# decadenza/SimpleStereo

Measured on AMD Instinct MI355X. Metric: disparity MPixels/s (H*W*nDisp per second), higher is better.
Workload: dtype f32

## Files before the change

simplestereo_amd/csrc/asw_instances.inc:

```
#ifdef SSAMD_PIPE_INSTANCE
SSAMD_PIPE_INSTANCE(true, 0, 0, 0)
SSAMD_PIPE_INSTANCE(false, 0, 0, 0)
SSAMD_PIPE_INSTANCE(false, 120, 316, 208)
SSAMD_PIPE_INSTANCE(false, 88, 348, 272)
SSAMD_PIPE_INSTANCE(false, 216, 284, 80)
SSAMD_PIPE_INSTANCE(true, 120, 316, 208)
SSAMD_PIPE_INSTANCE(true, 88, 348, 272)
SSAMD_PIPE_INSTANCE(true, 216, 284, 80)
#endif
#ifdef SSAMD_PIPE_INSTANCE_CG
SSAMD_PIPE_INSTANCE_CG(false, 120, 316, 208)
SSAMD_PIPE_INSTANCE_CG(false, 88, 348, 272)
SSAMD_PIPE_INSTANCE_CG(false, 216, 284, 80)
#endif
#ifdef SSAMD_WAVE6_INSTANCE
SSAMD_WAVE6_INSTANCE(true, 0, false)
SSAMD_WAVE6_INSTANCE(false, 0, false)
SSAMD_WAVE6_INSTANCE(false, 2, false)
SSAMD_WAVE6_INSTANCE(false, 2, true)
SSAMD_WAVE6_INSTANCE(false, 3, false)
SSAMD_WAVE6_INSTANCE(false, 3, true)
#endif
```

simplestereo_amd/csrc/asw_kernels.hip.h:

```cpp
#pragma once
#include "common.hip.h"

namespace ssamd {

static constexpr int ASW_RX = 8;
static constexpr int ASW_RD = 4;
static constexpr int ASW_WB = 4;
static constexpr int ASW_MAX_THREADS = 768;
__host__ __device__ constexpr int asw_nwr(int rx) { return (rx + ASW_RD - 1 + 3) / 4 * 4; }
static_assert(ASW_RD == 4 && asw_nwr(8) == 12 && asw_nwr(4) == 8, "the main loop is unrolled for 8x4 and 4x4 register tiles");

struct AswGeom {
    int Tx, XG, DG, Dc, nchunks, threads;
    int Rx;
    int nL, nR, nRc, SR, Se, emask;
    int SL, hL, hR;
    int wseg, wlen;
    int JC;
    int e2;
    int e_bytes;
    int pipe;
    int NC, JCmax;
    int dephase;
    int wave_rx;
    int off_wL, off_wR, off_e, off_labL, off_labR, off_bgrL, off_bgrR, off_bestL, off_bestR, off_cen, off_prox;
    int lds_bytes;
    int lds_bytes_evol;
};

struct AswExactQueue {
    u64 *entries;
    uint32_t *ekeys;
    unsigned int *counter;
    unsigned char *flagL, *flagR;
    unsigned char *zeroL, *zeroR;
    unsigned char *zrow;
    unsigned int W;
    unsigned int cap;
    uint32_t tol;
    float sat_abs;
    uint32_t deep;
};

struct AswArgs {
    const PixRec *recL, *recR;
    const float *prox;
    u64 *keyL;
    u64 *keyR;
    int16_t *disp;
    const unsigned char *evol;
    int erow0, erows, evolW;
    float *costs;
    int cost_keys;
    int H, W, win, pad, minD, maxD, row0, rows;
    int ystep;
    int yb0;
    int yskip_at, yskip;
    float kC;
    AswExactQueue xq;
    AswGeom g;
};

struct AswPipeTileId { int win, XG, DG, JC; };
__host__ __device__ constexpr int asw_cx_round_up(int v, int m) { return (v + m - 1) / m * m; }
__host__ __device__ constexpr int asw_cx_max(int a, int b) { return a > b ? a : b; }
__host__ __device__ constexpr AswGeom asw_pipe_geom_constexpr(AswPipeTileId t)
{
    AswGeom g{};
    const int win = t.win, p = win / 2;
    g.Rx = 8; g.JC = t.JC; g.pipe = 1; g.wave_rx = 0; g.e2 = 1; g.nchunks = 1;
    g.NC = (win + t.JC / 2) / t.JC;
    g.JCmax = asw_cx_max(t.JC, win - (g.NC - 1) * t.JC);
    g.XG = t.XG; g.DG = t.DG;
    g.Tx = 8 * t.XG; g.Dc = ASW_RD * t.DG;
    g.threads = asw_cx_round_up(t.XG * t.DG, 64);
    g.dephase = g.threads / 64 >= 12 ? 1 : 0;
    g.nL = g.Tx + 2 * p;
    g.nRc = g.Tx + g.Dc - 1;
    g.nR = g.nRc + 2 * p;
    g.hL = 0; g.hR = 0;
    g.SL = asw_cx_round_up(g.Tx, 4);
    g.SR = asw_cx_round_up(g.nRc + 1, 4);
    g.Se = 16 * ((t.DG + 3) / 4);
    g.emask = 0;
    const int wrows = 2 * g.JCmax;
    int off = 0;
    g.off_wL = off; off = (off + wrows * g.SL * 4 + 15) & ~15;
    g.off_wR = off; off = (off + wrows * g.SR * 4 + 15) & ~15;
    g.e_bytes = (g.nL * g.Se + 15) & ~15;
    g.off_e = off; off = (off + g.e_bytes * 2 + 15) & ~15;
    g.off_labL = off; off = (off + g.nL * 16 * 2 + 15) & ~15;
    g.off_labR = off; off = (off + g.nR * 16 * 2 + 15) & ~15;
    g.off_bestL = off; off = (off + g.Tx * 8 + 15) & ~15;
    g.off_bestR = off; off = (off + (g.nRc + 1) * 8 + 15) & ~15;
    g.off_cen = off; off = (off + (g.Tx + g.nRc) * 16 + 15) & ~15;
    g.off_prox = off; off = (off + win * 4 * 2 + 15) & ~15;
    g.lds_bytes_evol = off;
    g.off_bgrL = off; off = (off + g.nL * 4 * 2 + 15) & ~15;
    g.off_bgrR = off; off = (off + g.nR * 4 * 2 + 15) & ~15;
    g.lds_bytes = off;
    return g;
}
template <int SLC, int SRC, int SEC> struct AswPipeTile { static constexpr AswPipeTileId id{35, 1, 1, 16}; };
template <> struct AswPipeTile<120, 316, 208> { static constexpr AswPipeTileId id{35, 15, 49, 16}; };
template <> struct AswPipeTile<88, 348, 272> { static constexpr AswPipeTileId id{35, 11, 65, 16}; };
template <> struct AswPipeTile<216, 284, 80> { static constexpr AswPipeTileId id{35, 27, 17, 16}; };
inline bool asw_pipe_geom_matches(const AswGeom &a, const AswGeom &b)
{
    return a.pipe == b.pipe && a.Rx == b.Rx && a.JC == b.JC && a.NC == b.NC && a.JCmax == b.JCmax && a.XG == b.XG && a.DG == b.DG && a.Tx == b.Tx &&
           a.Dc == b.Dc && a.threads == b.threads && a.dephase == b.dephase && a.nL == b.nL && a.nRc == b.nRc && a.nR == b.nR && a.SL == b.SL &&
           a.SR == b.SR && a.Se == b.Se && a.e_bytes == b.e_bytes && a.off_wL == b.off_wL && a.off_wR == b.off_wR && a.off_e == b.off_e &&
           a.off_labL == b.off_labL && a.off_labR == b.off_labR && a.off_bestL == b.off_bestL && a.off_bestR == b.off_bestR &&
           a.off_cen == b.off_cen && a.off_prox == b.off_prox && a.off_bgrL == b.off_bgrL && a.off_bgrR == b.off_bgrR &&
           a.lds_bytes == b.lds_bytes && a.lds_bytes_evol == b.lds_bytes_evol && a.e2 == b.e2;
}

typedef float v2f __attribute__((ext_vector_type(2)));

template <typename Args>
__device__ __forceinline__ int asw_out_row(const Args &A, int b)
{
    b += A.yb0;
    return A.row0 + b * A.ystep + (b >= A.yskip_at ? A.yskip : 0);
}

static constexpr float ASW_TAD_CAP = 40.0f;

struct AswRow {
    float e[ASW_RD], c[ASW_RD];
};

__device__ __forceinline__ void asw_row_unpack(AswRow &row, const uint32_t packed)
{
#pragma unroll
    for (int di = 0; di < ASW_RD; ++di) {
        const float e = (float)((packed >> (8 * di)) & 0xffu);
        row.e[di] = e;
        row.c[di] = ASW_TAD_CAP - e;
    }
}

template <int RX, int ROT>
__device__ __forceinline__ void asw_taps(float (&accN)[RX][ASW_RD], float (&accS)[RX][ASW_RD],
                                         const float (&wl)[RX], const float (&wr)[asw_nwr(RX)],
                                         const AswRow (&win)[RX])
{
#pragma unroll
    for (int xi = 0; xi < RX; ++xi) {
        const AswRow &row = win[(ROT + xi) % RX];
#pragma unroll
        for (int di = 0; di < ASW_RD; ++di) {
            const float w = wl[xi] * wr[xi - di + ASW_RD - 1];
            accN[xi][di] = fmaf(w, row.e[di], accN[xi][di]);
            accS[xi][di] = fmaf(w, row.c[di], accS[xi][di]);
        }
    }
}

__device__ __forceinline__ uint32_t asw_cost_key(const float n, const float s, float &cost)
{
    const float t40 = n + s;
    if (n <= s) {
        cost = ASW_TAD_CAP * n / t40;
        return __float_as_uint(cost);
    }
    const float inv = ASW_TAD_CAP * s / t40;
    cost = ASW_TAD_CAP - inv;
    return 0xC0000000u - __float_as_uint(inv);
}

static constexpr unsigned EXACT_SIDE_L = 1u, EXACT_SIDE_R = 2u;
__device__ __forceinline__ uint32_t exact_zkey(int win)
{
    return __float_as_uint((float)(win * win) * 9.4039548065783e-37f);
}
static constexpr unsigned EXACT_HINT_ZERO = 4u;
static constexpr uint32_t EXACT_KEY_HIGH = 0xC0000000u - 0x41A00000u;

__device__ __forceinline__ bool exact_near(uint32_t key, uint32_t kb, uint32_t tol, float sat_abs, uint32_t zkey)
{
    if (key - kb <= tol || key <= zkey) return true;
    if (key >= EXACT_KEY_HIGH) {
        const float inv = __uint_as_float(0xC0000000u - key);
        if (kb >= EXACT_KEY_HIGH) return __uint_as_float(0xC0000000u - kb) - inv <= sat_abs;
        return (40.0f - inv) - __uint_as_float(kb) <= 20.0f * 1.1920929e-7f * (float)tol;
    }
    return false;
}

__device__ __forceinline__ bool exact_near_local(uint32_t key, uint32_t kb, uint32_t tol, float sat_abs, uint32_t zkey)
{
    if (key - kb <= tol || key <= zkey) return true;
    if (key < EXACT_KEY_HIGH || kb < 0x418C0000u) return false;
    if (exact_near(key, kb, tol, sat_abs, zkey)) return true;
    return kb >= EXACT_KEY_HIGH && __uint_as_float(0xC0000000u - key) >= 20.0f - 20.0f * 1.1920929e-7f * (float)tol;
}

__device__ __forceinline__ u64 exact_entry(uint32_t pix, int d, unsigned sides)
{
    return (u64)pix | ((u64)(uint32_t)d << 32) | ((u64)sides << 48);
}

__device__ __forceinline__ void asw_exact_push_wave(const AswExactQueue &q, bool want, uint32_t pix, int d, unsigned sides, uint32_t key = 0xffffffffu)
{
    if (key == 0u) sides |= EXACT_HINT_ZERO;
    const u64 mask = __builtin_amdgcn_ballot_w64(want);
    if (mask == 0) return;
    const int leader = (int)__builtin_ctzll(mask);
    const unsigned lane = __builtin_amdgcn_mbcnt_hi(~0u, __builtin_amdgcn_mbcnt_lo(~0u, 0u));
    unsigned base = 0;
    if ((int)lane == leader) base = atomicAdd(q.counter, (unsigned)__builtin_popcountll(mask));
    base = (unsigned)__builtin_amdgcn_readlane((int)base, leader);
    if (want) {
        const unsigned slot = base + (unsigned)__builtin_popcountll(mask & (((u64)1 << lane) - 1));
        if (slot < q.cap) {
            q.entries[slot] = exact_entry(pix, d, sides);
            if (q.ekeys) q.ekeys[slot] = key;
        }
        if ((sides & EXACT_SIDE_L) && q.flagL) q.flagL[pix] = 1;
        if ((sides & EXACT_SIDE_R) && q.flagR) q.flagR[pix - (uint32_t)d] = 1;
    }
}

template <int RX, int RD> struct AswKeyTile { uint32_t v[RX][RD]; };
template <int RX, int RD>
__device__ __forceinline__ void asw_exact_select(const AswExactQueue &q, bool live, const AswKeyTile<RX, RD> &kt,
                                                 const u64 *bL, const u64 *bR, int xb, int db, uint32_t rowpix, uint32_t zkey)
{
    const uint32_t (&kk)[RX][RD] = kt.v;
    static_assert(RX * RD <= 32, "one bit per candidate of the register tile");
    uint32_t mL = 0, mR = 0;
    if (live) {
        uint32_t zl = 0, zr = 0;
        const uint32_t tol = q.tol, deep = q.deep;
        const float ctol = 20.0f * 1.1920929e-7f * (float)tol, sat_abs = q.sat_abs;
        auto slow = [&](uint32_t key, uint32_t kh) -> uint32_t {
            const float inv = __uint_as_float(0xC0000000u - key);
            const uint32_t khigh = kh >= EXACT_KEY_HIGH ? 1u : 0u;
            const uint32_t b_ = khigh & (__uint_as_float(0xC0000000u - kh) - inv <= sat_abs ? 1u : 0u);
            const uint32_t c_ = (khigh ^ 1u) & ((40.0f - inv) - __uint_as_float(kh) <= ctol ? 1u : 0u);
            const uint32_t band = khigh & (inv >= 20.0f - ctol ? 1u : 0u);
            return (key >= EXACT_KEY_HIGH ? 1u : 0u) & (b_ | c_ | band);
        };
#pragma unroll
        for (int xi = 0; xi < RX; ++xi) {
            const u64 kl = bL[xi];
            const uint32_t kh = (uint32_t)(kl >> 32);
            const uint32_t wd = (uint32_t)kl - (uint32_t)db;
            const uint32_t tk = kh <= zkey ? max(tol, zkey - kh) : tol;
            uint32_t okm = 0;
#pragma unroll
            for (int di = 0; di < RD; ++di) {
                const uint32_t key = kk[xi][di];
                const uint32_t ok = (key < deep ? 1u : 0u) & (key != 0u ? 1u : 0u) & (wd != (uint32_t)di ? 1u : 0u);
                okm |= ok << di;
                mL |= (ok & (key - kh <= tk ? 1u : 0u)) << (xi * RD + di);
                zl |= ((key == 0u ? 1u : 0u) & (wd != (uint32_t)di ? 1u : 0u)) << xi;
            }
            if (kh >= 0x418C0000u && kh != 0xffffffffu) {
#pragma unroll
                for (int di = 0; di < RD; ++di) mL |= (((okm >> di) & 1u) & slow(kk[xi][di], kh)) << (xi * RD + di);
            }
        }
        if (bR) {
#pragma unroll
            for (int k = 0; k < RX + RD - 1; ++k) {
                const u64 kr = bR[k];
                const uint32_t kh = (uint32_t)(kr >> 32);
                const uint32_t wx = (uint32_t)kr - (uint32_t)xb;
                const bool high = kh >= 0x418C0000u && kh != 0xffffffffu;
                const uint32_t tk = kh <= zkey ? max(tol, zkey - kh) : tol;
#pragma unroll
                for (int xi = 0; xi < RX; ++xi) {
                    const int di = xi + RD - 1 - k;
                    if (di >= 0 && di < RD) {
                        const uint32_t key = kk[xi][di];
                        const uint32_t ok = (key < deep ? 1u : 0u) & (key != 0u ? 1u : 0u) & (wx != (uint32_t)xi ? 1u : 0u);
                        uint32_t near = key - kh <= tk ? 1u : 0u;
                        if (high) near |= slow(key, kh);
                        mR |= (ok & near) << (xi * RD + di);
                        zr |= ((key == 0u ? 1u : 0u) & (wx != (uint32_t)xi ? 1u : 0u)) << k;
                    }
                }
            }
        }
        if (zl | zr) {
            q.zrow[rowpix / q.W] = 1;
            for (uint32_t z = zl; z; z &= z - 1) q.zeroL[rowpix + (uint32_t)(xb + __builtin_ctz(z))] = 1;
            for (uint32_t z = zr; z; z &= z - 1) q.zeroR[rowpix + (uint32_t)(xb - db - RD + 1 + __builtin_ctz(z))] = 1;
        }
    }
    const uint32_t m = mL | mR;
    const uint32_t n = (uint32_t)__builtin_popcount(m);
    if (__builtin_amdgcn_ballot_w64(n != 0) == 0) return;
    uint32_t before = 0, total = 0;
#pragma unroll
    for (int bit = 0; bit < 6; ++bit) {
        const u64 pl = __builtin_amdgcn_ballot_w64((n >> bit) & 1u);
        before += __builtin_amdgcn_mbcnt_hi((uint32_t)(pl >> 32), __builtin_amdgcn_mbcnt_lo((uint32_t)pl, 0u)) << bit;
        total += (uint32_t)__builtin_popcountll(pl) << bit;
    }
    const u64 active = __builtin_amdgcn_ballot_w64(true);
    const int leader = (int)__builtin_ctzll(active);
    const unsigned lane = __builtin_amdgcn_mbcnt_hi(~0u, __builtin_amdgcn_mbcnt_lo(~0u, 0u));
    unsigned base = 0;
    if ((int)lane == leader) base = atomicAdd(q.counter, total);
    base = (unsigned)__builtin_amdgcn_readlane((int)base, leader);
    unsigned slot = base + before;
    uint32_t mm = m;
    while (mm) {
        const int b = __builtin_ctz(mm);
        mm &= mm - 1;
        const int xi = b / RD, di = b - xi * RD;
        const unsigned sides = ((mL >> b) & 1u ? EXACT_SIDE_L : 0u) | ((mR >> b) & 1u ? EXACT_SIDE_R : 0u);
        const uint32_t pix = rowpix + (uint32_t)(xb + xi);
        const int d = db + di;
        if (slot < q.cap) {
            uint32_t key = 0;
#pragma unroll
            for (int a = 0; a < RX; ++a)
#pragma unroll
                for (int c2 = 0; c2 < RD; ++c2)
                    if (a * RD + c2 == b) key = kk[a][c2];
            q.entries[slot] = exact_entry(pix, d, sides | (key == 0u ? EXACT_HINT_ZERO : 0u));
            if (q.ekeys) q.ekeys[slot] = key;
        }
        if ((sides & EXACT_SIDE_L) && q.flagL) q.flagL[pix] = 1;
        if ((sides & EXACT_SIDE_R) && q.flagR) q.flagR[pix - (uint32_t)d] = 1;
        ++slot;
    }
}

template <bool RIGHT>
__device__ __forceinline__ void asw_exact_merge(const AswExactQueue &q, bool have, u64 mine, u64 old, uint32_t rowpix, int xcol, uint32_t zkey)
{
    bool want = false;
    uint32_t pix = 0, key = 0;
    int d = 0;
    if (have && old != KEY_NONE) {
        const u64 lo = mine < old ? mine : old, hi = mine < old ? old : mine;
        if ((uint32_t)(hi >> 32) < q.deep && (uint32_t)(hi >> 32) != 0u && exact_near_local((uint32_t)(hi >> 32), (uint32_t)(lo >> 32), q.tol, q.sat_abs, zkey)) {
            want = true;
            key = (uint32_t)(hi >> 32);
            if (RIGHT) { const int xl = (int)(uint32_t)hi; pix = rowpix + (uint32_t)xl; d = xl - xcol; }
            else { pix = rowpix + (uint32_t)xcol; d = (int)(uint32_t)hi; }
        }
    }
    if (have && old != KEY_NONE && (uint32_t)(old >> 32) == 0u && (uint32_t)(mine >> 32) == 0u) {
        (RIGHT ? q.zeroR : q.zeroL)[rowpix + (uint32_t)xcol] = 1;
        q.zrow[rowpix / q.W] = 1;
    }
    asw_exact_push_wave(q, want, pix, d, RIGHT ? EXACT_SIDE_R : EXACT_SIDE_L, key);
}

__device__ __forceinline__ int asw_split_pos(int c, int half)
{
    return ((c >> 2) & 1) * half + ((c >> 3) << 2) + (c & 3);
}

template <int RX>
__device__ __forceinline__ int asw_e_offset(int ul, int slot, int Se, int emask)
{
    return ul * Se + ((slot ^ ((ul / RX) & emask)) << 2);
}

template <bool WITH_COSTS, bool CHUNKED, int RX = ASW_RX>
__global__ __launch_bounds__(ASW_MAX_THREADS, RX == 8 ? 3 : 4) void asw_aggregate_kernel(const AswArgs A)
{
    constexpr int NWR = asw_nwr(RX);
    extern __shared__ __attribute__((aligned(16))) char smem[];
    const AswGeom &g = A.g;
    float *const wL = reinterpret_cast<float *>(smem + g.off_wL);
    float *const wR = reinterpret_cast<float *>(smem + g.off_wR);
    unsigned char *const eT0 = reinterpret_cast<unsigned char *>(smem + g.off_e);
    float4 *const labL = reinterpret_cast<float4 *>(smem + g.off_labL);
    float4 *const labR = reinterpret_cast<float4 *>(smem + g.off_labR);
    uint32_t *const bgrL = reinterpret_cast<uint32_t *>(smem + g.off_bgrL);
    uint32_t *const bgrR = reinterpret_cast<uint32_t *>(smem + g.off_bgrR);
    u64 *const bestL = reinterpret_cast<u64 *>(smem + g.off_bestL);
    u64 *const bestR = reinterpret_cast<u64 *>(smem + g.off_bestR);
    float4 *const cenLab = reinterpret_cast<float4 *>(smem + g.off_cen);
    float *const proxS = reinterpret_cast<float *>(smem + g.off_prox);

    const int tid = threadIdx.x, nthr = blockDim.x;
    const int W = A.W, win = A.win, p = A.pad;
    const int Tx = g.Tx, Dc = g.Dc, nL = g.nL, nR = g.nR, nRc = g.nRc, SR = g.SR, Se = g.Se, emask = g.emask;
    int bx = blockIdx.x;
    if ((gridDim.x & 7) == 0) bx = (bx & 7) * (gridDim.x >> 3) + (bx >> 3);
    const int x0 = bx * Tx;
    const int y = asw_out_row(A, blockIdx.y);
    const int dlo = A.minD + blockIdx.z * Dc;
    const int dhi = dlo + Dc - 1;
    if (min(x0 + Tx - 1, W - 1) - dlo < 0) {
        if (A.disp)
            for (int k = threadIdx.x; k < Tx && x0 + k < W; k += blockDim.x)
                A.disp[(size_t)(y - A.row0) * W + x0 + k] = (int16_t)(x0 + k);
        return;
    }

    const int segL_lo = x0 - p;
    const int xrc_lo = x0 - dhi;
    const int segR_lo = xrc_lo - p;


    float accN[RX][ASW_RD], accS[RX][ASW_RD];
#pragma unroll
    for (int a = 0; a < RX; ++a)
#pragma unroll
        for (int b = 0; b < ASW_RD; ++b) { accN[a][b] = 0.f; accS[a][b] = 0.f; }

    for (int k = tid; k < Tx; k += nthr) bestL[k] = KEY_NONE;
    for (int k = tid; k <= nRc; k += nthr) bestR[k] = KEY_NONE;

    for (int c = tid; c < Tx + nRc; c += nthr) {
        const bool isL = c < Tx;
        const int ccol = isL ? x0 + c : xrc_lo + (c - Tx);
        float4 v = make_float4(0.f, 0.f, 0.f, 0.f);
// ... 338 lines not shown
```

simplestereo_amd/csrc/asw_pipe_kernel.hip.h:

```cpp
#pragma once
#include "asw_kernels.hip.h"
#ifndef SSAMD_KERNEL_TU
#include "lab_kernels.hip.h"
#endif

#ifndef SSAMD_PIPE_SENTINEL
#define SSAMD_PIPE_SENTINEL 1
#endif

namespace ssamd {

#ifndef SSAMD_KERNEL_TU
static constexpr int TADV_COLS = 64;
template <bool BYTES>
__device__ __forceinline__ void asw_tad_tile(const void *__restrict__ srcL, const void *__restrict__ srcR, unsigned char *__restrict__ evol,
                                             int W, int pad, int minD, int Dc, int Se, int erow0, int erows, int evolW, int rd, long long npix_total,
                                             int bx, int by, int bz, char *smem)
{
    uint32_t *const sL = reinterpret_cast<uint32_t *>(smem);
    uint32_t *const sR = sL + TADV_COLS;
    const int r = erow0 + by, z = bz, uc0 = bx * TADV_COLS;
    const int P = Se >> 2, dlo = minD + z * Dc, dhi = dlo + Dc - 1;
    const int u0 = uc0 - pad, xr0 = u0 - dhi;
    auto pixel = [&](const void *src, int col) -> uint32_t {
        const size_t q = (size_t)r * W + col;
        if constexpr (BYTES) {
            typedef uint32_t __attribute__((aligned(1))) u32_unaligned;
            const uint8_t *const b = reinterpret_cast<const uint8_t *>(src) + 3 * q;
            return (long long)q + 1 < npix_total ? (*reinterpret_cast<const u32_unaligned *>(b) & 0xffffffu)
                                                 : ((uint32_t)b[0] | ((uint32_t)b[1] << 8) | ((uint32_t)b[2] << 16));
        } else {
            return reinterpret_cast<const PixRec *>(src)[q].bgrx;
        }
    };
    for (int k = threadIdx.x; k < 2 * TADV_COLS + Dc; k += blockDim.x) {
        const bool isL = k < TADV_COLS;
        const int col = isL ? u0 + k : xr0 + (k - TADV_COLS);
        const uint32_t v = (unsigned)col < (unsigned)W ? pixel(isL ? srcL : srcR, col) : 0x80000000u;
        (isL ? sL : sR)[isL ? k : k - TADV_COLS] = v;
    }
    __syncthreads();
    const int ncols = min(TADV_COLS, evolW - uc0);
    uint32_t *const out = reinterpret_cast<uint32_t *>(evol + (((size_t)z * erows + by) * (size_t)evolW + uc0) * Se);
    auto dword = [&](int c, int slot, uint32_t lp) {
        uint32_t v = 0;
        const int d0 = rd == 6 ? 6 * (slot >> 1) + 4 * (slot & 1) : 4 * slot, nv = rd == 6 && (slot & 1) ? 2 : 4;
        if (!(lp >> 31) && d0 < Dc) {
            const uint32_t *const rp = sR + c + (Dc - 1) - d0;
#pragma unroll
            for (int q = 0; q < 4; ++q) {
                const uint32_t rv = q < nv && d0 + q < Dc ? rp[-q] : 0x80000000u;
                if (!(rv >> 31)) v |= min(__builtin_amdgcn_sad_u8(lp, rv, 0u), 40u) << (8 * q);
            }
        }
        return v;
    };
    if ((P & 3) == 0) {
        const int P4 = P >> 2;
        uint4 *const out4 = reinterpret_cast<uint4 *>(out);
        for (int k = threadIdx.x; k < ncols * P4; k += blockDim.x) {
            const int c = k / P4, s4 = 4 * (k - c * P4);
            const uint32_t lp = sL[c];
            out4[k] = make_uint4(dword(c, s4, lp), dword(c, s4 + 1, lp), dword(c, s4 + 2, lp), dword(c, s4 + 3, lp));
        }
        return;
    }
    for (int k = threadIdx.x; k < ncols * P; k += blockDim.x) {
        const int c = k / P, slot = k - c * P;
        out[k] = dword(c, slot, sL[c]);
    }
}

__global__ __launch_bounds__(256) void asw_tad_volume_kernel(const PixRec *__restrict__ recL, const PixRec *__restrict__ recR,
                                                             unsigned char *__restrict__ evol, int W, int pad, int minD, int Dc,
                                                             int Se, int erow0, int erows, int evolW, int rd = 4)
{
    extern __shared__ __attribute__((aligned(16))) char smem[];
    asw_tad_tile<false>(recL, recR, evol, W, pad, minD, Dc, Se, erow0, erows, evolW, rd, 0, blockIdx.x, blockIdx.y, blockIdx.z, smem);
}

struct AswPrepassArgs {
    const uint8_t *bgrL, *bgrR;
    PixRec *recL, *recR;
    unsigned char *evol;
    long long npix_total;
    int W, pad, minD, Dc, Se, erow0, erows, evolW, rd;
    int lab_blocks, ex, ey;
};
__global__ __launch_bounds__(256) void asw_prepass_kernel(const AswPrepassArgs P)
{
    extern __shared__ __attribute__((aligned(16))) char smem[];
    if ((int)blockIdx.x < P.lab_blocks) {
        SSAMD_LAB_TABLES_IN_LDS(T)
        const long long np = (long long)P.erows * P.W, first = (long long)P.erow0 * P.W;
        const uint8_t *const bl = P.bgrL + 3 * first, *const br = P.bgrR + 3 * first;
        PixRec *const rl = P.recL + first, *const rr = P.recR + first;
        typedef uint32_t __attribute__((aligned(1))) u32_unaligned;
        for (long long q = (long long)blockIdx.x * blockDim.x + threadIdx.x; q < 2 * np; q += (long long)P.lab_blocks * blockDim.x) {
            const bool right = q >= np;
            const long long p = right ? q - np : q;
            const uint8_t *const bgr = right ? br : bl;
            uint32_t B, G, R;
            if (p + 1 < np) {
                const uint32_t v = *reinterpret_cast<const u32_unaligned *>(bgr + 3 * p);
                B = v & 0xff; G = (v >> 8) & 0xff; R = (v >> 16) & 0xff;
            } else {
                B = bgr[3 * p]; G = bgr[3 * p + 1]; R = bgr[3 * p + 2];
            }
            PixRec o;
            bgr_to_lab(B, G, R, o.L, o.a, o.b, T);
            o.bgrx = B | (G << 8) | (R << 16);
            (right ? rr : rl)[p] = o;
        }
        return;
    }
    const int b = (int)blockIdx.x - P.lab_blocks, bx = b % P.ex, by = (b / P.ex) % P.ey, bz = b / (P.ex * P.ey);
    asw_tad_tile<true>(P.bgrL, P.bgrR, P.evol, P.W, P.pad, P.minD, P.Dc, P.Se, P.erow0, P.erows, P.evolW, P.rd, P.npix_total, bx, by, bz, smem);
}

#endif

template <bool WITH_COSTS, int SLC = 0, int SRC = 0, int SEC = 0, bool CG = false>
__global__ __launch_bounds__(ASW_MAX_THREADS, 3) void asw_aggregate_pipe_kernel(const AswArgs A)
{
    constexpr bool STATIC = SLC > 0;
    static_assert(!CG || STATIC, "compile-time geometry belongs to a static tile");
    constexpr int RX = ASW_RX;
    constexpr int NWR = asw_nwr(RX);
    extern __shared__ __attribute__((aligned(16))) char smem[];
    constexpr AswGeom SG = asw_pipe_geom_constexpr(AswPipeTile<SLC, SRC, SEC>::id);
    static_assert(!STATIC || (SG.SL == SLC && SG.SR == SRC && SG.Se == SEC), "the strides name the tile");
    const AswGeom &g = CG ? SG : A.g;
    float *const wL = reinterpret_cast<float *>(smem + g.off_wL);
    float *const wR = reinterpret_cast<float *>(smem + g.off_wR);
    unsigned char *const eT0 = reinterpret_cast<unsigned char *>(smem + g.off_e);
    float4 *const labL = reinterpret_cast<float4 *>(smem + g.off_labL);
    float4 *const labR = reinterpret_cast<float4 *>(smem + g.off_labR);
    uint32_t *const bgrL = reinterpret_cast<uint32_t *>(smem + g.off_bgrL);
    uint32_t *const bgrR = reinterpret_cast<uint32_t *>(smem + g.off_bgrR);
    u64 *const bestL = reinterpret_cast<u64 *>(smem + g.off_bestL);
    u64 *const bestR = reinterpret_cast<u64 *>(smem + g.off_bestR);
    float4 *const cenLab = reinterpret_cast<float4 *>(smem + g.off_cen);
    float *const proxS = reinterpret_cast<float *>(smem + g.off_prox);

    const int tid = threadIdx.x, nthr = blockDim.x;
    const int W = A.W, win = CG ? AswPipeTile<SLC, SRC, SEC>::id.win : A.win, p = CG ? AswPipeTile<SLC, SRC, SEC>::id.win / 2 : A.pad;
    const int Tx = g.Tx, Dc = g.Dc, nL = g.nL, nR = g.nR, nRc = g.nRc, SR = g.SR, Se = g.Se;
    const int JC = g.JC, NC = g.NC;
    int bx = blockIdx.x;
    if ((gridDim.x & 7) == 0) bx = (bx & 7) * (gridDim.x >> 3) + (bx >> 3);
    const int x0 = bx * Tx;
    const int y = asw_out_row(A, blockIdx.y);
    const int dlo = A.minD + blockIdx.z * Dc;
    const int dhi = dlo + Dc - 1;
    if (min(x0 + Tx - 1, W - 1) - dlo < 0) {
        if (A.disp)
            for (int k = threadIdx.x; k < Tx && x0 + k < W; k += blockDim.x)
                A.disp[(size_t)(y - A.row0) * W + x0 + k] = (int16_t)(x0 + k);
        return;
    }
    const int segL_lo = x0 - p, xrc_lo = x0 - dhi, segR_lo = xrc_lo - p;
    const int phase = g.dephase ? __builtin_amdgcn_readfirstlane((int)(threadIdx.x >> 8)) : 1;

    float accN[RX][ASW_RD], accS[RX][ASW_RD];
#pragma unroll
    for (int a = 0; a < RX; ++a)
#pragma unroll
        for (int b = 0; b < ASW_RD; ++b) { accN[a][b] = 0.f; accS[a][b] = 0.f; }

    for (int k = tid; k < Tx; k += nthr) bestL[k] = KEY_NONE;
    for (int k = tid; k <= nRc; k += nthr) bestR[k] = KEY_NONE;
    for (int c = tid; c < Tx + nRc; c += nthr) {
        const bool isL = c < Tx;
        const int ccol = isL ? x0 + c : xrc_lo + (c - Tx);
        float4 v = make_float4(0.f, 0.f, 0.f, 0.f);
        if ((unsigned)ccol < (unsigned)W) {
            const PixRec q = (isL ? A.recL : A.recR)[(size_t)y * W + ccol];
            v = make_float4(q.L, q.a, q.b, 1.f);
        }
        cenLab[c] = v;
    }

    const int i_lo = max(0, p - y), i_hi = min(win, A.H + p - y);

    auto stage_row = [&](int i) {
        int tids = threadIdx.x;
        asm volatile("" : "+v"(tids));
        const int buf = i & 1, r = y - p + i;
        for (int k = tids; k < win; k += nthr) proxS[buf * win + k] = A.prox[i * win + k];
        const PixRec *const rowL = A.recL + (size_t)r * W;
        const PixRec *const rowR = A.recR + (size_t)r * W;
        for (int k = tids; k < nL + nR; k += nthr) {
            const bool isL = k < nL;
            const int idx = isL ? k : k - nL;
            const int col = (isL ? segL_lo : segR_lo) + idx;
            PixRec v;
            v.L = SSAMD_PIPE_SENTINEL ? __builtin_inff() : 0.f;
            v.a = v.b = 0.f;
            v.bgrx = 0u;
            if ((unsigned)col < (unsigned)W) v = (isL ? rowL : rowR)[col];
            (isL ? labL + buf * nL : labR + buf * nR)[idx] = make_float4(v.L, v.a, v.b, 0.f);
            if (!A.evol) (isL ? bgrL + buf * nL : bgrR + buf * nR)[idx] = v.bgrx;
        }
    };
    auto build_e = [&](int i, int t_lo, int t_hi) {
        int tidb = threadIdx.x;
        asm volatile("" : "+v"(tidb));
        unsigned char *const eT = eT0 + (i & 1) * g.e_bytes;
        const uint32_t *const bgrLc = bgrL + (i & 1) * nL, *const bgrRc = bgrR + (i & 1) * nR;
        const int e_q = nthr / nL, e_r = nthr - e_q * nL;
        int t = t_lo + tidb;
        int sp = t / nL, ul = t - sp * nL;
        while (t < t_hi) {
            const uint32_t lp = bgrLc[ul];
            const uint32_t *const rp = bgrRc + (ul + (Dc - 1) - 8 * sp);
            uint32_t lo = 0, hi = 0;
#pragma unroll
            for (int k = 0; k < 4; ++k) {
                lo |= min(__builtin_amdgcn_sad_u8(lp, rp[-k], 0u), 40u) << (8 * k);
                hi |= min(__builtin_amdgcn_sad_u8(lp, rp[-4 - k], 0u), 40u) << (8 * k);
            }
            uint32_t *const dst = reinterpret_cast<uint32_t *>(eT + ul * Se) + 2 * sp;
            dst[0] = lo;
            if (2 * sp + 1 < g.DG) dst[1] = hi;
            t += nthr; ul += e_r; sp += e_q;
            if (ul >= nL) { ul -= nL; ++sp; }
        }
    };
    auto load_e = [&](int i) {
        int tidd = threadIdx.x;
        asm volatile("" : "+v"(tidd));
        const int r = y - p + i;
        const unsigned char *const src = A.evol + (((size_t)blockIdx.z * A.erows + (r - A.erow0)) * (size_t)A.evolW + x0) * Se;
        unsigned char *const dst = eT0 + (i & 1) * g.e_bytes;
        const int bytes = nL * Se, lane16 = (tidd & 63) * 16;
        for (int k = __builtin_amdgcn_readfirstlane(tidd >> 6) * 1024; k < bytes; k += (nthr >> 6) * 1024)
            if (k + lane16 < bytes)
                __builtin_amdgcn_global_load_lds((const void *)(src + k + lane16),
                                                 (__attribute__((address_space(3))) void *)(dst + k), 16, 0, 0);
    };
    auto build_weights = [&](int i, int jb, int je, int rb) {
        int tidw = threadIdx.x;
        asm volatile("" : "+v"(tidw));
        const float4 *const labLc = labL + (i & 1) * nL, *const labRc = labR + (i & 1) * nR;
        const float *const prow = proxS + (i & 1) * win;
        const int ncen = Tx + nRc;
        const int full = ncen / nthr * nthr, rest = ncen - full;
        int slen = je - jb, nseg = 1;
        if (rest > 0 && full > 0) {
            slen = max(ASW_WB, (je - jb + nthr / rest - 1) / (nthr / rest));
            slen = (slen + ASW_WB - 1) / ASW_WB * ASW_WB;
            nseg = (je - jb + slen - 1) / slen;
        }
        const int ntasks = full + rest * nseg;
        for (int t = tidw; t < ntasks; t += nthr) {
            int c = t, jb_t = jb, je_t = je;
            if (t >= full && nseg > 1) {
                const int q = t - full, sgm = q / rest;
                c = full + q - sgm * rest;
                jb_t = jb + sgm * slen;
                je_t = min(je, jb_t + slen);
            }
            const bool isL = c < Tx;
            const int cc = isL ? c : c - Tx;
            const float4 cen = cenLab[c];
            const float4 *const seg = (isL ? labLc : labRc) + cc;
            const int stride = isL ? g.SL : SR;
            float *const wout = (isL ? wL : wR) + cc + (rb - jb) * stride;
            const int col0 = (isL ? x0 : xrc_lo) + cc - p;
            const uint32_t cmask = cen.w != 0.f ? 0xffffffffu : 0u;
            int j = jb_t;
            const float4 *sp = seg + j;
            const float *pp = prow + j;
            float *wp = wout + j * stride;
            int col = col0 + j;
            const int stride4 = ASW_WB * stride;
            for (; j + ASW_WB <= je_t; j += ASW_WB, sp += ASW_WB, pp += ASW_WB, wp += stride4, col += ASW_WB) {
                float4 tp[ASW_WB];
                float pr[ASW_WB], wv[ASW_WB];
#pragma unroll
                for (int u = 0; u < ASW_WB; ++u) { tp[u] = sp[u]; pr[u] = pp[u]; }
#pragma unroll
                for (int u = 0; u < ASW_WB; ++u) {
                    asm volatile("" ::"v"(tp[u].w));
                    const float dL = tp[u].x - cen.x, da = tp[u].y - cen.y, db = tp[u].z - cen.z;
                    wv[u] = fmaf(db, db, fmaf(da, da, dL * dL));
                }
#pragma unroll
                for (int u = 0; u < ASW_WB; ++u) wv[u] = __builtin_amdgcn_sqrtf(wv[u]);
#pragma unroll
                for (int u = 0; u < ASW_WB; ++u) wv[u] = asw_weight_finish(wv[u], A.kC, pr[u]);
#pragma unroll
                for (int u = 0; u < ASW_WB; ++u) {
                    if constexpr (SSAMD_PIPE_SENTINEL) {
                        wp[u * stride] = wv[u];
                    } else {
                        const uint32_t m = (unsigned)(col + u) < (unsigned)W ? cmask : 0u;
                        wp[u * stride] = __uint_as_float(__float_as_uint(wv[u]) & m);
                    }
                }
            }
            if (j < je_t) {
                float4 tp[ASW_WB];
                float pr[ASW_WB], wv[ASW_WB];
#pragma unroll
                for (int u = 0; u < ASW_WB; ++u) {
                    const int jj = min(j + u, je_t - 1);
                    tp[u] = seg[jj];
                    pr[u] = prow[jj];
                }
#pragma unroll
                for (int u = 0; u < ASW_WB; ++u) {
                    asm volatile("" ::"v"(tp[u].w));
                    const float dL = tp[u].x - cen.x, da = tp[u].y - cen.y, db = tp[u].z - cen.z;
                    wv[u] = fmaf(db, db, fmaf(da, da, dL * dL));
                }
#pragma unroll
                for (int u = 0; u < ASW_WB; ++u) wv[u] = __builtin_amdgcn_sqrtf(wv[u]);
#pragma unroll
                for (int u = 0; u < ASW_WB; ++u) wv[u] = asw_weight_finish(wv[u], A.kC, pr[u]);
#pragma unroll
                for (int u = 0; u < ASW_WB; ++u) {
                    const int jj = min(j + u, je_t - 1);
                    if constexpr (SSAMD_PIPE_SENTINEL) {
                        wout[jj * stride] = wv[u];
                    } else {
                        const uint32_t m = (unsigned)(col0 + jj) < (unsigned)W ? cmask : 0u;
                        wout[jj * stride] = __uint_as_float(__float_as_uint(wv[u]) & m);
                    }
                }
            }
        }
    };
    auto chunk_end = [&](int c) { return c == NC - 1 ? win : (c + 1) * JC; };
    const int nE = nL * ((g.DG + 1) >> 1);
    auto build_next = [&](int i, int c, int cb) {
        const bool more_rows = i + 1 < i_hi;
#ifdef SSAMD_PIPE_BUILD_PRIO
        __builtin_amdgcn_s_setprio(SSAMD_PIPE_BUILD_PRIO);
#endif
#ifndef SSAMD_ABLATE_STAGE
        if (c == 0 && more_rows) stage_row(i + 1);
#endif
        if (c == 0 && more_rows && A.evol) load_e(i + 1);
#ifndef SSAMD_ABLATE_WEIGHTS
        if (c + 1 < NC) build_weights(i, (c + 1) * JC, chunk_end(c + 1), (cb ^ 1) * g.JCmax);
        else if (more_rows) build_weights(i + 1, 0, chunk_end(0), (cb ^ 1) * g.JCmax);
#endif
#ifndef SSAMD_ABLATE_E
        if (c >= 1 && more_rows && !A.evol) build_e(i + 1, (int)((long long)nE * (c - 1) / (NC - 1)), (int)((long long)nE * c / (NC - 1)));
#endif
#ifdef SSAMD_PIPE_BUILD_PRIO
        __builtin_amdgcn_s_setprio(0);
#endif
    };

    stage_row(i_lo);
    if (A.evol) load_e(i_lo);
    __syncthreads();
    if (!A.evol) build_e(i_lo, 0, nE);
    build_weights(i_lo, 0, chunk_end(0), 0);

    const int DGe = max(1, min(g.DG, (min(min(x0 + Tx, W) - 1, x0 + Tx - 1) - dlo) / ASW_RD + 1));
    const int nact = g.XG * DGe;
    int pk_xd;
    bool run;
    {
        const int tidm = threadIdx.x;
        int xg, dg;
#ifdef SSAMD_PIPE_PLAIN_LANES
        xg = tidm / DGe; dg = tidm - xg * DGe;
#else
        const int F = DGe >> 4, Lo = DGe & 15, nfull = g.XG * F;
        const int grp16 = tidm >> 4, r16 = tidm & 15;
        if (grp16 < nfull) {
            xg = grp16 / F;
            int gi = grp16 - xg * F;
            if (xg & 1) gi = F - 1 - gi;
            dg = 16 * gi + r16;
        } else {
            const int q = tidm - 16 * nfull;
            xg = Lo ? q / Lo : g.XG;
            dg = 16 * F + (Lo ? q - xg * Lo : 0);
        }
#endif
        pk_xd = xg | (dg << 16);
        const bool tile_live = tidm < nact && x0 + RX * xg < W && dlo + ASW_RD * dg <= A.maxD &&
                               x0 + RX * xg + RX - 1 - (dlo + ASW_RD * dg) >= 0;
        run = __builtin_amdgcn_ballot_w64(tile_live) != 0 && tidm < nact;
    }

    int cb = 0;
#pragma nounroll
    for (int i = i_lo; i < i_hi; ++i) {
        const unsigned char *const eT = eT0 + (i & 1) * g.e_bytes;
        AswRow ew[RX];

#pragma nounroll
        for (int c = 0; c < NC; ++c) {
#ifndef SSAMD_ABLATE_BARRIER
            __syncthreads();
#endif
            const int jc = c * JC, jend = chunk_end(c);
            const int rb = cb * g.JCmax;
            if (phase == 0) build_next(i, c, cb);
#ifndef SSAMD_ABLATE_AGG
            if (run) {
                const int xg = pk_xd & 0xffff, dg = pk_xd >> 16;
                const unsigned char *erow = eT + (RX * xg + (jc == 0 ? 0 : RX - 1 + jc)) * Se + 4 * dg;
                if (jc == 0) {
#pragma unroll
                    for (int n = 0; n < RX - 1; ++n) {
                        asw_row_unpack(ew[n], *reinterpret_cast<const uint32_t *>(erow));
                        erow += Se;
                    }
                }
                const float *wlp = wL + rb * g.SL + 8 * xg;
                const float *wrp = wR + rb * SR + (RX * xg - ASW_RD * dg + Dc - ASW_RD);
                for (int j0 = jc; j0 < jend; j0 += RX) {
#define SSAMD_PSTEP(JJ)                                                                             \
    if (j0 + (JJ) < jend) {                                                                         \
        const uint32_t epk = *reinterpret_cast<const uint32_t *>(erow + (STATIC ? (JJ) * SEC : 0)); \
        if constexpr (!STATIC) erow += Se;                                                          \
        float wl[RX], wr[NWR];                                                                      \
        {                                                                                           \
            const float *const wl_ = wlp + (STATIC ? (JJ) * SLC : 0);                              \
            const float *const wr_ = wrp + (STATIC ? (JJ) * SRC : 0);                              \
            const float4 v0 = *reinterpret_cast<const float4 *>(wl_);                              \
            wl[0] = v0.x; wl[1] = v0.y; wl[2] = v0.z; wl[3] = v0.w;                                 \
            const float4 v1 = *reinterpret_cast<const float4 *>(wl_ + 4);                          \
            wl[4] = v1.x; wl[5] = v1.y; wl[6] = v1.z; wl[7] = v1.w;                                 \
            const float4 r0 = *reinterpret_cast<const float4 *>(wr_);                              \
            const float4 r1 = *reinterpret_cast<const float4 *>(wr_ + 4);                          \
            const float4 r2 = *reinterpret_cast<const float4 *>(wr_ + 8);                          \
            asm volatile("" ::"v"(r2.w));       \
            wr[0] = r0.x; wr[1] = r0.y; wr[2] = r0.z; wr[3] = r0.w;                                 \
            wr[4] = r1.x; wr[5] = r1.y; wr[6] = r1.z; wr[7] = r1.w;                                 \
            wr[8] = r2.x; wr[9] = r2.y; wr[10] = r2.z; wr[11] = r2.w;                               \
        }                                                                                           \
        if constexpr (!STATIC) { wlp += g.SL; wrp += SR; }                                         \
               \
        _Pragma("unroll") for (int xi = 0; xi < RX; ++xi) {                                         \
            if (xi == RX - 1) asw_row_unpack(ew[((JJ) + RX - 1) % RX], epk);                        \
            const AswRow &row_ = ew[((JJ) + xi) % RX];                                              \
            _Pragma("unroll") for (int di = 0; di < ASW_RD; ++di) {                                 \
                const float w_ = wl[xi] * wr[xi - di + ASW_RD - 1];                                 \
                accN[xi][di] = fmaf(w_, row_.e[di], accN[xi][di]);                                  \
                accS[xi][di] = fmaf(w_, row_.c[di], accS[xi][di]);                                  \
            }                                                                                       \
        }                                                                                           \
    }
                    SSAMD_PSTEP(0) SSAMD_PSTEP(1) SSAMD_PSTEP(2) SSAMD_PSTEP(3)
                    SSAMD_PSTEP(4) SSAMD_PSTEP(5) SSAMD_PSTEP(6) SSAMD_PSTEP(7)
#undef SSAMD_PSTEP
                    if constexpr (STATIC) { erow += RX * SEC; wlp += RX * SLC; wrp += RX * SRC; }
                }
            }
#endif
            if (phase != 0) build_next(i, c, cb);
            cb ^= 1;
        }
    }

    int tidf = threadIdx.x;
    asm volatile("" : "+v"(tidf));
    AswKeyTile<RX, ASW_RD> kt;
    if (tidf < nact) {
        const int xg = pk_xd & 0xffff, dg = pk_xd >> 16;
        u64 diag[RX + ASW_RD - 1];
#pragma unroll
        for (int k = 0; k < RX + ASW_RD - 1; ++k) diag[k] = KEY_NONE;
#pragma unroll
        for (int xi = 0; xi < RX; ++xi) {
            const int x = x0 + RX * xg + xi;
            u64 bl = KEY_NONE;
#pragma unroll
            for (int di = 0; di < ASW_RD; ++di) {
                const int d = dlo + ASW_RD * dg + di;
                const bool valid = (x < W) && (d <= A.maxD) && (x - d >= 0);
                kt.v[xi][di] = 0xffffffffu;
                if (valid) {
                    float c;
                    const u64 hi = (u64)asw_cost_key(accN[xi][di], accS[xi][di], c) << 32;
                    kt.v[xi][di] = (uint32_t)(hi >> 32);
                    bl = min(bl, hi | (u64)(uint32_t)d);
                    diag[xi - di + ASW_RD - 1] = min(diag[xi - di + ASW_RD - 1], hi | (u64)(uint32_t)x);
                    if (WITH_COSTS)
                        A.costs[((size_t)(y - A.row0) * W + x) * (A.maxD - A.minD + 1) + (d - A.minD)] = A.cost_keys ? __uint_as_float((uint32_t)(hi >> 32)) : c;
                }
            }
            if (bl != KEY_NONE) atomicMin(&bestL[RX * xg + xi], bl);
        }
        if (A.keyR) {
            const int base = RX * xg - ASW_RD * dg + Dc - ASW_RD;
#pragma unroll
            for (int k = 0; k < RX + ASW_RD - 1; ++k)
                if (diag[k] != KEY_NONE) atomicMin(&bestR[base + k], diag[k]);
        }
    }
    __syncthreads();
    const size_t orow = (size_t)(y - A.row0) * W;
    const bool xq = !WITH_COSTS && A.xq.entries != nullptr;
    if (xq) {
        const int xg = pk_xd & 0xffff, dg = pk_xd >> 16;
        asw_exact_select<RX, ASW_RD>(A.xq, tidf < nact, kt, bestL + RX * xg, A.keyR ? bestR + (RX * xg - ASW_RD * dg + Dc - ASW_RD) : nullptr,
                                     x0 + RX * xg, dlo + ASW_RD * dg, (uint32_t)orow, exact_zkey(win));
    }
    if (A.disp) {
        for (int k = tid; k < Tx; k += nthr) {
            const int x = x0 + k;
            if (x < W) A.disp[orow + x] = bestL[k] == KEY_NONE ? (int16_t)x : (int16_t)(uint32_t)bestL[k];
        }
        return;
    }
    if (xq) {
        for (int k0 = 0; k0 < Tx; k0 += nthr) {
            const int k = k0 + tid, x = x0 + k;
            const bool have = k < Tx && x < W && bestL[k < Tx ? k : 0] != KEY_NONE;
            const u64 mine = have ? bestL[k] : KEY_NONE;
            const u64 old = have ? atomicMin(&A.keyL[orow + x], mine) : KEY_NONE;
            asw_exact_merge<false>(A.xq, have, mine, old, (uint32_t)orow, x, exact_zkey(win));
        }
        if (A.keyR)
            for (int k0 = 0; k0 < nRc; k0 += nthr) {
                const int k = k0 + tid, xr = xrc_lo + k;
                const bool have = k < nRc && (unsigned)xr < (unsigned)W && bestR[k < nRc ? k : 0] != KEY_NONE;
                const u64 mine = have ? bestR[k] : KEY_NONE;
                const u64 old = have ? atomicMin(&A.keyR[orow + xr], mine) : KEY_NONE;
                asw_exact_merge<true>(A.xq, have, mine, old, (uint32_t)orow, xr, exact_zkey(win));
            }
        return;
    }
    for (int k = tid; k < Tx; k += nthr) {
        const int x = x0 + k;
        if (x < W && bestL[k] != KEY_NONE) atomicMin(&A.keyL[orow + x], bestL[k]);
    }
    if (A.keyR) {
        for (int k = tid; k < nRc; k += nthr) {
            const int xr = xrc_lo + k;
            if ((unsigned)xr < (unsigned)W && bestR[k] != KEY_NONE) atomicMin(&A.keyR[orow + xr], bestR[k]);
        }
    }
}

}
```

simplestereo_amd/csrc/asw_pipe_tu.hip:

```cpp
#define SSAMD_KERNEL_TU 1
#include <hip/hip_runtime.h>
#include "asw_pipe_kernel.hip.h"

namespace ssamd {
#define SSAMD_PIPE_INSTANCE(C, SL, SR, SE) template __global__ void asw_aggregate_pipe_kernel<C, SL, SR, SE>(const AswArgs);
#define SSAMD_PIPE_INSTANCE_CG(C, SL, SR, SE) template __global__ void asw_aggregate_pipe_kernel<C, SL, SR, SE, true>(const AswArgs);
#include "asw_instances.inc"
#undef SSAMD_PIPE_INSTANCE_CG
#undef SSAMD_PIPE_INSTANCE
}
```

simplestereo_amd/csrc/ssamd_api.hip:

```cpp
#include <hip/hip_runtime.h>

#include <algorithm>
#include <array>
#include <atomic>
#include <list>
#include <map>
#include <thread>
#include <cmath>
#include <cstdarg>
#include <cstdio>
#include <cstdlib>
#include <cstring>
#include <mutex>
#include <string>
#include <vector>

#include "../../include/ssamd.h"
#include "asw_kernels.hip.h"
#include "asw_pipe_kernel.hip.h"
#include "asw_wave_kernel.hip.h"
#include "asw_wave6_kernel.hip.h"
#include "asw_alt_kernels.hip.h"
#ifndef SSAMD_SINGLE_TU
namespace ssamd {
#define SSAMD_PIPE_INSTANCE(C, SL, SR, SE) extern template __global__ void asw_aggregate_pipe_kernel<C, SL, SR, SE>(const AswArgs);
#define SSAMD_PIPE_INSTANCE_CG(C, SL, SR, SE) extern template __global__ void asw_aggregate_pipe_kernel<C, SL, SR, SE, true>(const AswArgs);
#define SSAMD_WAVE6_INSTANCE(C, K, CREG) extern template __global__ void asw_aggregate_wave6_kernel<C, K, CREG>(const AswWaveArgs);
#include "asw_instances.inc"
#undef SSAMD_PIPE_INSTANCE
#undef SSAMD_PIPE_INSTANCE_CG
#undef SSAMD_WAVE6_INSTANCE
}
#endif
#include "gsw_kernels.hip.h"
#include "lab_kernels.hip.h"
#include "asw_exact_kernels.hip.h"
#include "rig_kernels.hip.h"
#include "unwrap_kernels.hip.h"

using namespace ssamd;

namespace {

thread_local std::string g_err;
std::mutex g_geom_mutex;

int fail(int code, const char *fmt, ...)
{
    char buf[512];
    va_list ap;
    va_start(ap, fmt);
    vsnprintf(buf, sizeof(buf), fmt, ap);
    va_end(ap);
    g_err = buf;
    return code;
}

struct Tuning {
    std::string asw_geom, gsw_geom;
    int asw_pipe = -1;
    int asw_dephase = -1;
    int asw_evol = 1;
    int asw_wave = -1;
    int wave_rx = 0;
    int wave_wg = 0;
    int wave_unroll = 1;
    int wave_merge = 1;
    int asw_static = 1;
    int evol_max_mb = 0;
    int wave_rd = 0;
    bool no_e2 = false, xor_only = false, multi_allow_repeat = false;
    int alt_queue_cap = 0;
    int autotune_env = -2;
    int evol_fail = 0;
    int lds_relax = 1;
    int wave_creg = 1;
    int asw_tail = -1;
    int prepass_fuse = 1;
    int exact_tol = 128;
    int exact_cap = 0;
    int exact_rawcap = 0;
    int unwrap_rows = 0;
};
std::mutex g_tune_mutex;
std::atomic<unsigned> g_tune_version{1};

bool tuning_assign(Tuning &t, const std::string &name, const char *v)
{
    auto num = [&](int unset) { return v ? atoi(v) : unset; };
    if (name == "SSAMD_ASW_GEOM") t.asw_geom = v ? v : "";
    else if (name == "SSAMD_GSW_GEOM") t.gsw_geom = v ? v : "";
    else if (name == "SSAMD_ASW_PIPE") t.asw_pipe = num(-1);
    else if (name == "SSAMD_ASW_DEPHASE") t.asw_dephase = num(-1);
    else if (name == "SSAMD_ASW_EVOL") t.asw_evol = num(1);
    else if (name == "SSAMD_ASW_WAVE") t.asw_wave = v ? (atoi(v) != 0 ? 1 : 0) : -1;
    else if (name == "SSAMD_ASW_WAVE_RX") t.wave_rx = num(0);
    else if (name == "SSAMD_ASW_WAVE_WG") t.wave_wg = v ? std::max(1, std::min(4, atoi(v))) : 0;
    else if (name == "SSAMD_ASW_WAVE_UNROLL") t.wave_unroll = num(1);
    else if (name == "SSAMD_ASW_WAVE_MERGE") t.wave_merge = num(1);
    else if (name == "SSAMD_ASW_STATIC") t.asw_static = num(1);
    else if (name == "SSAMD_ASW_EVOL_MAX_MB") t.evol_max_mb = v ? std::max(0, atoi(v)) : 0;
    else if (name == "SSAMD_ASW_WAVE_RD") t.wave_rd = num(0);
    else if (name == "SSAMD_ASW_NO_E2") t.no_e2 = v != nullptr;
    else if (name == "SSAMD_ASW_XOR_ONLY") t.xor_only = v != nullptr;
    else if (name == "SSAMD_MULTI_ALLOW_REPEAT") t.multi_allow_repeat = v != nullptr;
    else if (name == "SSAMD_ALT_QUEUE_CAP") t.alt_queue_cap = v ? std::max(1, atoi(v)) : 0;
    else if (name == "SSAMD_AUTOTUNE") t.autotune_env = v ? (atoi(v) > 0 ? 1 : (atoi(v) < 0 ? -1 : 0)) : -2;
    else if (name == "SSAMD_ASW_EVOL_FAIL") t.evol_fail = num(0);
    else if (name == "SSAMD_ASW_TAIL") t.asw_tail = num(-1);
    else if (name == "SSAMD_ASW_WAVE_CREG") t.wave_creg = num(1);
    else if (name == "SSAMD_ASW_LDS_RELAX") t.lds_relax = num(1);
    else if (name == "SSAMD_ASW_PREPASS_FUSE") t.prepass_fuse = num(1);
    else if (name == "SSAMD_EXACT_TOL") t.exact_tol = v ? std::max(0, atoi(v)) : 128;
    else if (name == "SSAMD_EXACT_CAP") t.exact_cap = v ? std::max(1, atoi(v)) : 0;
    else if (name == "SSAMD_EXACT_RAWCAP") t.exact_rawcap = v ? std::max(1, atoi(v)) : 0;
    else if (name == "SSAMD_UNWRAP_ROWS") t.unwrap_rows = v ? std::max(0, std::min(UNWRAP_MAX_ROWS, atoi(v))) : 0;
    else return false;
    return true;
}

const char *const kTuningNames[] = {"SSAMD_ASW_GEOM", "SSAMD_GSW_GEOM", "SSAMD_ASW_PIPE", "SSAMD_ASW_DEPHASE", "SSAMD_ASW_EVOL",
                                    "SSAMD_ASW_WAVE", "SSAMD_ASW_WAVE_RX", "SSAMD_ASW_WAVE_WG", "SSAMD_ASW_WAVE_UNROLL",
                                    "SSAMD_ASW_WAVE_MERGE", "SSAMD_ASW_STATIC", "SSAMD_ASW_EVOL_MAX_MB", "SSAMD_ASW_WAVE_RD", "SSAMD_ASW_NO_E2", "SSAMD_ASW_XOR_ONLY", "SSAMD_MULTI_ALLOW_REPEAT",
                                    "SSAMD_ALT_QUEUE_CAP", "SSAMD_AUTOTUNE", "SSAMD_ASW_EVOL_FAIL", "SSAMD_ASW_TAIL", "SSAMD_ASW_WAVE_CREG", "SSAMD_ASW_LDS_RELAX",
                                    "SSAMD_EXACT_TOL", "SSAMD_EXACT_CAP", "SSAMD_EXACT_RAWCAP", "SSAMD_ASW_PREPASS_FUSE", "SSAMD_UNWRAP_ROWS"};

std::map<std::string, std::string> g_tuning_env;
Tuning tuning_from_env()
{
    Tuning t;
    for (const char *n : kTuningNames)
        if (const char *v = getenv(n)) {
            g_tuning_env[n] = v;
            (void)tuning_assign(t, n, v);
        }
    return t;
}
Tuning g_tuning = tuning_from_env();

const Tuning &tune()
{
    thread_local Tuning snap;
    thread_local unsigned seen = 0;
    const unsigned v = g_tune_version.load(std::memory_order_acquire);
    if (v != seen) {
        std::lock_guard<std::mutex> lk(g_tune_mutex);
        snap = g_tuning;
        seen = v;
    }
    return snap;
}

#define HIP_TRY(expr)                                                                              \
    do {                                                                                           \
        hipError_t e_ = (expr);                                                                    \
        if (e_ != hipSuccess)                                                                      \
            return fail(e_ == hipErrorOutOfMemory ? SSAMD_ENOMEM : SSAMD_EHIP, "%s failed: %s",    \
                        #expr, hipGetErrorString(e_));                                             \
    } while (0)

struct DevBuf {
    void *ptr = nullptr;
    size_t cap = 0;
    int reserve(size_t bytes)
    {
        if (bytes <= cap) return SSAMD_OK;
        if (ptr) { (void)hipFree(ptr); ptr = nullptr; cap = 0; }
        size_t want = bytes + bytes / 8 + 256;
        hipError_t e = hipMalloc(&ptr, want);
        if (e != hipSuccess) {
            ptr = nullptr;
            (void)hipGetLastError();
            return fail(SSAMD_ENOMEM, "hipMalloc(%zu) failed: %s", want, hipGetErrorString(e));
        }
        cap = want;
        return SSAMD_OK;
    }
    void release()
    {
        if (ptr) (void)hipFree(ptr);
        ptr = nullptr; cap = 0;
    }
};

struct Profile {
    bool on = false;
    struct Pair { hipEvent_t a, b; int slot; };
    std::vector<Pair> pending;
    std::vector<hipEvent_t> pool;
    double ms[SSAMD_K_COUNT] = {0};
    long long n[SSAMD_K_COUNT] = {0};
    hipEvent_t get()
    {
        if (!pool.empty()) { hipEvent_t e = pool.back(); pool.pop_back(); return e; }
        hipEvent_t e = nullptr;
        (void)hipEventCreate(&e);
        return e;
    }
    void drain()
    {
        for (auto &p : pending) {
            float t = 0.f;
            if (hipEventSynchronize(p.b) == hipSuccess && hipEventElapsedTime(&t, p.a, p.b) == hipSuccess) {
                ms[p.slot] += t;
                n[p.slot] += 1;
            }
            pool.push_back(p.a);
            pool.push_back(p.b);
        }
        pending.clear();
    }
};

struct TableEntry {
    int k0 = 0; double k1 = 0;
    DevBuf dev;
    std::vector<float> host;
    std::vector<double> host64;
};
struct TableCache {
    std::list<TableEntry> entries;
    size_t max_entries;
    explicit TableCache(size_t n) : max_entries(n) {}
    TableEntry *find(int k0, double k1)
    {
        for (auto it = entries.begin(); it != entries.end(); ++it)
            if (it->k0 == k0 && it->k1 == k1) {
                entries.splice(entries.begin(), entries, it);
                return &entries.front();
            }
        return nullptr;
    }
};

struct Ctx {
    std::mutex mu;
    int dev = -1;
    int cus = 256;
    bool lut_ready = false;
    hipStream_t stream = nullptr;
    DevBuf imgL, imgR, recL, recR, keyL, keyR, disp, costs, lab, altq, evol, altdisp;
    DevBuf xlabL, xlabR, xflags, xqueue, xcost, xslots, xctr, xraw, xwtab;
    DevBuf uwIn, uwOut;
    unsigned int xcap = 0, xrawcap = 0;
    TableCache proxTabs{8}, gswTabs{4}, proxTabs64{8};
    std::map<const void *, int> max_dyn_lds;
    hipEvent_t scratch_free = nullptr;
    int evol_small_calls = 0;
    long long evol_fallbacks = 0;
    long long tail_splits = 0;
    long long exact_calls = 0;
    long long static_tile_mismatch = 0;
    Profile prof;
};

Ctx g_ctx[16];

struct DeviceGuard {
    int saved = -1;
    DeviceGuard() { if (hipGetDevice(&saved) != hipSuccess) saved = -1; }
    ~DeviceGuard() { if (saved >= 0) (void)hipSetDevice(saved); }
    DeviceGuard(const DeviceGuard &) = delete;
    DeviceGuard &operator=(const DeviceGuard &) = delete;
};

int grant_dyn_lds(Ctx &c, const void *kernel, int bytes);

struct Timed {
    Ctx &c; hipStream_t s; int slot; hipEvent_t a = nullptr, b = nullptr;
    Timed(Ctx &c_, hipStream_t s_, int slot_) : c(c_), s(s_), slot(slot_)
    {
        if (c.prof.on) { a = c.prof.get(); b = c.prof.get(); (void)hipEventRecord(a, s); }
    }
    ~Timed()
    {
        if (a) { (void)hipEventRecord(b, s); c.prof.pending.push_back({a, b, slot}); }
    }
};

struct CtxLock {
    DeviceGuard guard;
    std::unique_lock<std::mutex> lk;
    Ctx *c = nullptr;
    Ctx *operator->() { return c; }
    Ctx &operator*() { return *c; }
};

int get_ctx(int device, CtxLock &out)
{
    int n = 0;
    if (hipGetDeviceCount(&n) != hipSuccess || n <= 0)
        return fail(SSAMD_ENODEVICE, "no HIP device visible: libssamd has no CPU fallback");
    if (device < 0) device = out.guard.saved >= 0 ? out.guard.saved : 0;
    if (device >= n || device >= 16) return fail(SSAMD_EINVAL, "device ordinal %d out of range (%d visible)", device, n);
    HIP_TRY(hipSetDevice(device));
    Ctx &c = g_ctx[device];
    out.lk = std::unique_lock<std::mutex>(c.mu);
    out.c = &c;
    if (c.dev < 0) {
        c.dev = device;
        int cus = 0;
        if (hipDeviceGetAttribute(&cus, hipDeviceAttributeMultiprocessorCount, device) == hipSuccess && cus > 0) c.cus = cus;
        else (void)hipGetLastError();
        HIP_TRY(hipStreamCreateWithFlags(&c.stream, hipStreamNonBlocking));
        HIP_TRY(hipEventCreateWithFlags(&c.scratch_free, hipEventDisableTiming));
    }
    if (!c.lut_ready) {
        float lut[256];
        for (int v = 0; v < 256; ++v) {
            float x = v / 255.0;
            if (x > 0.04045) x = glibc_powf_pos((float)((x + 0.055) / 1.055), (float)2.4);
            else x /= 12.92;
            x *= 100;
            lut[v] = x;
        }
        HIP_TRY(hipMemcpyToSymbol(HIP_SYMBOL(c_lin100), lut, sizeof(lut)));
        c.lut_ready = true;
    }
    return SSAMD_OK;
}

int grant_dyn_lds(Ctx &c, const void *kernel, int bytes)
{
    int &granted = c.max_dyn_lds[kernel];
    if (bytes <= granted || bytes <= 48 * 1024) return SSAMD_OK;
    HIP_TRY(hipFuncSetAttribute(kernel, hipFuncAttributeMaxDynamicSharedMemorySize, bytes));
    granted = bytes;
    return SSAMD_OK;
}

struct ScratchOrder {
    Ctx &c; hipStream_t s;
    ScratchOrder(Ctx &c_, hipStream_t s_) : c(c_), s(s_) { (void)hipStreamWaitEvent(s, c.scratch_free, 0); }
    ~ScratchOrder() { (void)hipEventRecord(c.scratch_free, s); }
};

int check_common(int H, int W, int win, int minD, int maxD, int row0, int rows)
{
    if (H <= 0 || W <= 0) return fail(SSAMD_EINVAL, "Wrong image dimensions!");
    if (!(win > 0 && win % 2 == 1)) return fail(SSAMD_EINVAL, "winSize must be a positive odd number!");
    if (minD < 0) return fail(SSAMD_EINVAL, "minDisparity must be >= 0 (negative values are undefined behaviour in the reference)");
    if (W > 32767 || maxD > 32767) return fail(SSAMD_ELIMIT, "width / maxDisparity exceed the int16 disparity range");
    if (row0 < 0 || rows < 0 || row0 + rows > H) return fail(SSAMD_EINVAL, "output row range [%d,%d) outside the image (height %d)", row0, row0 + rows, H);
    if (win > 255) return fail(SSAMD_ELIMIT, "winSize %d > 255 not supported", win);
    if (rows > 65535) return fail(SSAMD_ELIMIT, "more than 65535 output rows per call: split the image into row strips");
    return SSAMD_OK;
}

inline int round_up(int v, int m) { return (v + m - 1) / m * m; }

thread_local bool t_pipe_full_lds = false;

bool asw_layout_e(AswGeom &g, int win, int XG, int DG, size_t limit, int JC, int Rx, bool e2, bool odd_pitch = false,
                  bool pipe = false)
{
    g.Rx = Rx;
    g.JC = JC >= win ? win : JC;
    g.pipe = 0; g.NC = 1; g.JCmax = g.JC; g.dephase = 0; g.wave_rx = 0;
    if (pipe) {
        if (Rx != 8 || JC % Rx || !e2) return false;
        g.NC = (win + JC / 2) / JC;
        if (g.NC < 2 || (g.NC - 1) * JC >= win) return false;
        g.pipe = 1;
        g.dephase = tune().asw_dephase >= 0 ? tune().asw_dephase : (round_up(XG * DG, 64) / 64 >= 12 ? 1 : 0);
        g.JCmax = std::max(JC, win - (g.NC - 1) * JC);
    }
    const int wrows = g.pipe ? 2 * g.JCmax : (g.JC < win ? 2 * g.JC : win);
    const int wcols = g.JC;

    const int p = win / 2;
    g.XG = XG; g.DG = DG;
    g.Tx = Rx * XG; g.Dc = ASW_RD * DG;
    g.threads = round_up(XG * DG, 64);
    g.nL = g.Tx + 2 * p;
    g.nRc = g.Tx + g.Dc - 1;
    g.nR = g.nRc + 2 * p;
    g.hL = ((g.Tx + 7) / 8) * 4 + 4;
    g.SL = 2 * g.hL;
    g.hR = ((g.nRc + 4 + 7) / 8) * 4 + 4;
    g.SR = 2 * g.hR;
    int P = 8;
    while (P < DG && P < 32) P <<= 1;
    if (P < DG) P = round_up(DG, 32);
    g.Se = 4 * P;
    g.emask = std::min(P, 32) - 1;
    if (odd_pitch) {
        g.Se = 4 * (DG | 1);
        g.emask = 0;
    }
    if (g.pipe) {
        g.hL = g.hR = 0;
        g.SL = round_up(g.Tx, 4);
        g.SR = round_up(g.nRc + 1, 4);
        g.Se = 16 * ((DG + 3) / 4);
        g.emask = 0;
    }
    {
        const int ncen = g.Tx + g.nRc;
        int best_cost = 1 << 30;
        for (int ns = 1; ns <= wcols && ns <= 8; ++ns) {
            const int len = (wcols + ns - 1) / ns, rounds = (ncen * ns + g.threads - 1) / g.threads;
            const int cost = rounds * (round_up(len, ASW_WB) + 2);
            if (cost < best_cost) { best_cost = cost; g.wseg = ns; g.wlen = len; }
        }
    }
    size_t off = 0;
    auto take = [&](size_t bytes) { size_t o = off; off = (off + bytes + 15) & ~(size_t)15; return (int)o; };
    g.off_wL = take((size_t)wrows * g.SL * 4);
    g.off_wR = take((size_t)wrows * g.SR * 4);
    g.e_bytes = (int)(((size_t)g.nL * g.Se + 15) & ~(size_t)15);
    g.e2 = (e2 && g.JC < win && (win + g.JC - 1) / g.JC >= 2) ? 1 : 0;
    if (g.pipe && !g.e2) return false;
    g.off_e = take((size_t)g.e_bytes * (g.e2 ? 2 : 1));
    g.off_labL = take((size_t)g.nL * 16 * 2);
    g.off_labR = take((size_t)g.nR * 16 * 2);
    if (!g.pipe) {
        g.off_bgrL = take((size_t)g.nL * 4 * 2);
        g.off_bgrR = take((size_t)g.nR * 4 * 2);
    }
    g.off_bestL = take((size_t)g.Tx * 8);
    g.off_bestR = take((size_t)(g.nRc + 1) * 8);
    g.off_cen = take((size_t)(g.Tx + g.nRc) * 16);
    g.off_prox = take((size_t)win * 4 * 2);
    g.lds_bytes_evol = (int)off;
    if (g.pipe) {
        g.off_bgrL = take((size_t)g.nL * 4 * 2);
        g.off_bgrR = take((size_t)g.nR * 4 * 2);
    }
    g.lds_bytes = (int)off;
    if (g.pipe && tune().asw_evol != 0 && tune().lds_relax != 0 && !t_pipe_full_lds) return (size_t)g.lds_bytes_evol <= limit;
    return off <= limit;
}

bool asw_layout(AswGeom &g, int win, int XG, int DG, size_t limit, int JC = 1 << 20, int Rx = ASW_RX, bool odd_pitch = false)
{
    if (!tune().no_e2 && asw_layout_e(g, win, XG, DG, limit, JC, Rx, true, odd_pitch) && g.e2) return true;
    return asw_layout_e(g, win, XG, DG, limit, JC, Rx, false, odd_pitch);
}

double asw_e_read_passes(const AswGeom &g)
{
    const int P = g.Se / 4, T = g.XG * g.DG;
    long long tot = 0, cnt = 0;
    for (int n = 0; n < g.Rx; ++n)
        for (int base = 0; base < T; base += 32) {
            int hits[64] = {0}, worst = 0;
            for (int l = 0; l < 32 && base + l < T; ++l) {
                const int tid = base + l, xg = tid % g.XG, dg = tid / g.XG, ul = g.Rx * xg + n;
                worst = std::max(worst, ++hits[(ul * P + (dg ^ ((ul / g.Rx) & g.emask))) & 63]);
            }
            tot += worst; ++cnt;
        }
    return cnt ? (double)tot / cnt : 1.0;
}

void asw_pick_e_scheme(AswGeom &g, int win)
{
    if (tune().xor_only) return;
    AswGeom alt;
    if (!asw_layout(alt, win, g.XG, g.DG, 160 * 1024, g.JC >= win ? (1 << 20) : g.JC, g.Rx, true)) return;
    const bool take = alt.e2 != g.e2 ? alt.e2 > g.e2 : asw_e_read_passes(alt) <= asw_e_read_passes(g) + 1e-9;
    if (take) {
        alt.nchunks = g.nchunks;
        g = alt;
    }
}

void asw_try_pipe(AswGeom &g, int win)
{
    const int want = tune().asw_pipe;
    if (want == 0 || g.Rx != 8) return;
    for (int JC : {16, 8}) {
        if (want > 0 && JC != want) continue;
        if (want < 0 && JC == 8 && round_up(g.XG * g.DG, 64) / 64 < 12) continue;
        AswGeom alt;
        if (!asw_layout_e(alt, win, g.XG, g.DG, 160 * 1024, JC, 8, true, false, true)) continue;
        alt.nchunks = g.nchunks;
        g = alt;
        return;
    }
}

static constexpr int ASW_WAVE_MAX_DG = 16;
bool asw_wave_layout_one(AswWaveGeom &g, int win, int DG, int rx, int nxg, bool merged, int rd = ASW_RD, bool creg = false)
{
    g.RX = rx;
    g.RD = rd;
    g.creg = 0;
    const int p = win / 2;
    g.DG = DG;
    g.NXG = nxg;
    g.Txw = rx * g.NXG;
    g.Dc = rd * g.DG;
    g.lanes = g.NXG * g.DG;
    g.nLw = g.Txw + 2 * p;
    g.nRcw = g.Txw + g.Dc - 1;
    g.nRw = g.nRcw + 2 * p;
    g.merged = merged ? 1 : 0;
    if (merged) {
        g.K = (g.Txw + g.nRcw + 63) / 64;
        g.SLw = g.Txw;
        g.SRw = round_up(g.Txw + g.nRcw + 1, 64) - g.Txw;
    } else {
        g.K = (g.Txw + 63) / 64 + (g.nRcw + 63) / 64;
        g.SLw = round_up(g.Txw, 64);
        g.SRw = round_up(g.nRcw + 1, 64);
    }
    g.Se = rd == 6 ? 8 * ((g.DG + 1) | 1) : 4 * (g.DG | 1);
    g.waves = tune().wave_wg ? tune().wave_wg : 1;
    size_t off = 0;
    auto take = [&](size_t bytes) { size_t o = off; off = (off + bytes + 15) & ~(size_t)15; return (int)o; };
    g.off_w = take((size_t)(g.SLw + g.SRw) * 4 * 2);
    g.creg = creg && merged && rx == 4 && g.K >= 2 && (rd == 6 ? g.K <= 3 : g.K <= 4) ? 1 : 0;
    g.off_cen = take(g.creg ? 0 : (size_t)(g.Txw + g.nRcw) * 16);
    g.off_pixL = take((size_t)g.nLw * 16);
    g.off_pixR = take((size_t)g.nRw * 16);
    g.off_e = take(std::max((size_t)g.nLw * g.Se, (size_t)(129 + 2 * p) * 16) + (rd == 6 ? 0 : (size_t)rx * g.Se));
    g.off_bestL = g.off_pixL;
    g.off_bestR = g.off_pixL + (int)(((size_t)g.Txw * 8 + 15) & ~(size_t)15);
    if ((size_t)g.off_bestR + (size_t)(g.nRcw + 1) * 8 > off) off = (size_t)g.off_bestR + (size_t)(g.nRcw + 1) * 8;
    g.wave_lds = (int)((off + 15) & ~(size_t)15);
    return g.off_pixR == g.off_pixL + g.nLw * 16 && (size_t)g.wave_lds * g.waves <= 160 * 1024;
}

bool asw_wave_layout(AswWaveGeom &g, int win, int nD, int rx, bool creg = false)
{
    const bool never6 = (rx & 16) != 0;
    rx &= 15;
    creg = creg && tune().wave_creg != 0;
    const int DG = (nD + ASW_RD - 1) / ASW_RD;
    if (DG < 1 || DG > ASW_WAVE_MAX_DG) return false;
    const int nxg_max = 64 / DG;
    if (tune().wave_merge == 0) return asw_wave_layout_one(g, win, DG, rx, nxg_max, false);
    const double c_round = 17.0, c_taps = rx == 8 ? 110.0 : 59.0;
    double best = 1e30;
    bool found = false;
    for (int nxg = nxg_max; nxg >= std::max(1, nxg_max - 4); --nxg)
        for (int merged = 0; merged <= 1; ++merged) {
            AswWaveGeom c;
            if (merged && nxg != nxg_max && tune().wave_merge == 2) continue;
            if (!asw_wave_layout_one(c, win, DG, rx, nxg, merged != 0, ASW_RD, creg)) continue;
            if (merged && c.K > 4) continue;
            if (!merged && nxg != nxg_max) continue;
            const double cost = (c.K * c_round + c_taps) / (double)c.Txw;
            if (cost < best - 1e-9) { best = cost; g = c; found = true; }
        }
    if (found && rx == 4 && !never6 && tune().wave_rd != 4 && tune().wave_merge != 0) {
        const int DG6 = (nD + 5) / 6;
        if (DG6 >= 1 && DG6 <= 10) {
            const int nxg6 = 64 / DG6;
            for (int nxg = nxg6; nxg >= std::max(1, nxg6 - 4); --nxg) {
                AswWaveGeom c;
                if (!asw_wave_layout_one(c, win, DG6, 4, nxg, true, 6, creg) || c.K > 4) continue;
                const double cost = (c.K * c_round + 87.0) / (double)c.Txw;
                if (cost < 0.95 * best) { best = cost / 0.95; g = c; }
            }
        }
    }
    return found;
}

static constexpr int ASW_WAVE_MAX_ND = 64;
int asw_wave_pick(int win, int nD)
{
    if (tune().asw_wave == 0 || tune().asw_evol == 0) return 0;
    if (nD < 1 || nD > ASW_WAVE_MAX_ND || win > 63) return 0;
    AswWaveGeom wg;
    if (const int rx = tune().wave_rx) {
        return (rx == 8 || rx == 4) && asw_wave_layout(wg, win, nD, rx) ? rx : 0;
    }
    const int first = nD <= 20 ? 4 : 8, second = 12 - first;
    if (asw_wave_layout(wg, win, nD, first)) return first;
    return asw_wave_layout(wg, win, nD, second) ? second : 0;
}

int asw_search_geometry(AswGeom &best, int W, int rows, int win, int nD, std::vector<AswGeom> *shortlist = nullptr);

std::map<std::array<int, 4>, AswGeom> g_asw_geom_cache;
std::map<std::array<int, 4>, bool> g_asw_geom_tuned;
std::atomic<int> g_autotune{g_tuning.autotune_env != -2 ? g_tuning.autotune_env : -1};
constexpr double ASW_AUTOTUNE_SMALL_TAPS = 6.0e10;

bool asw_geometry_forced()
{
    const Tuning &t = tune();
    return !t.asw_geom.empty() || t.asw_wave >= 0 || t.wave_rx != 0 || t.wave_merge != 1 || t.asw_pipe >= 0 || t.asw_dephase >= 0 ||
           t.asw_evol != 1 || t.wave_wg != 0 || t.no_e2 || t.xor_only || t.asw_static != 1 || t.evol_max_mb != 0 || t.wave_rd != 0 ||
           t.wave_creg != 1 || t.lds_relax != 1;
}

int asw_choose_geometry(AswGeom &best, int W, int rows, int win, int nD)
{
    if (asw_geometry_forced()) return asw_search_geometry(best, W, rows, win, nD);
    std::lock_guard<std::mutex> glk(g_geom_mutex);
    const std::array<int, 4> key{W, rows, win, nD};
    auto it = g_asw_geom_cache.find(key);
    if (it != g_asw_geom_cache.end()) { best = it->second; return SSAMD_OK; }
    const int rc = asw_search_geometry(best, W, rows, win, nD);
    if (rc == SSAMD_OK) {
        if (g_asw_geom_cache.size() > 256) { g_asw_geom_cache.clear(); g_asw_geom_tuned.clear(); }
        g_asw_geom_cache[key] = best;
    }
    return rc;
}

int asw_search_geometry(AswGeom &best, int W, int rows, int win, int nD, std::vector<AswGeom> *shortlist)
{
    std::map<std::array<int, 4>, std::pair<double, AswGeom>> classes;
    if (!tune().asw_geom.empty()) {
        int XG = 0, DG = 0, JCe = 1 << 20, Rx = ASW_RX;
        if (sscanf(tune().asw_geom.c_str(), "%d,%d,%d,%d", &XG, &DG, &JCe, &Rx) >= 2 && XG > 0 && DG > 0 && XG * DG <= ASW_MAX_THREADS &&
            (Rx == 8 || Rx == 4)) {
            if (JCe <= 0 || JCe % Rx) JCe = 1 << 20;
            if (!asw_layout(best, win, XG, DG, 160 * 1024, JCe, Rx)) return fail(SSAMD_ELIMIT, "SSAMD_ASW_GEOM does not fit LDS");
            best.nchunks = (nD + best.Dc - 1) / best.Dc;
            asw_pick_e_scheme(best, win);
            asw_try_pipe(best, win);
            return SSAMD_OK;
        }
    }
    const double c_tap = 10.9, c_w = 70.0, c_e = 60.0, c_stage = 40.0;
    double best_score = -1.0;
    bool found = false;
    for (int nch = 1; nch <= nD; ++nch) {
        const int per = (nD + nch - 1) / nch;
        const int DG = round_up(per, ASW_RD) / ASW_RD;
        if (DG > 128) continue;
        if ((nD + DG * ASW_RD - 1) / (DG * ASW_RD) != nch) continue;
        for (int Rx : {8, 4}) {
        if (Rx == 4 && nD > 56) continue;
        const int max_wps = Rx == 8 ? 3 : 4;
        const int xg_cap = std::min(ASW_MAX_THREADS / DG, (W + Rx - 1) / Rx);
        const int pipe_env = tune().asw_pipe;
        for (int XG = xg_cap; XG >= 1; --XG)
        for (int cand = 0; cand < 6; ++cand) {
            static const int jcs[6] = {1 << 20, 16, 8, 4, 16, 8};
            const int JC = jcs[cand];
            const bool piped = cand >= 4;
            AswGeom g;
            if (piped) {
                if (Rx != 8 || pipe_env == 0 || (pipe_env > 0 && pipe_env != JC)) continue;
                if (pipe_env < 0 && JC == 8 && round_up(XG * DG, 64) / 64 < 12) continue;
                if (!asw_layout_e(g, win, XG, DG, 160 * 1024, JC, 8, true, false, true)) continue;
            } else {
                if (JC < (1 << 20) && (JC >= win || JC % Rx)) continue;
                if (!asw_layout(g, win, XG, DG, 160 * 1024, JC, Rx)) continue;
            }
            g.nchunks = nch;
            const int waves = g.threads / 64, per_simd = (waves + 3) / 4;
            const int k = std::min(max_wps / per_simd, (160 * 1024) / (piped && tune().asw_evol != 0 ? g.lds_bytes_evol : g.lds_bytes));
            if (k < 1) continue;
            const double M = (double)win * Rx * ASW_RD * (Rx == 8 ? (piped ? 0.93 * c_tap : c_tap) : c_tap * 1.15);
            const int ncen = g.Tx + g.nRc;
            const int njc = piped ? g.NC : (win + g.JC - 1) / g.JC;
            double B;
            if (piped)
                B = (double)ncen * win / g.threads * 28.0 + njc * 350.0 + c_stage;
            else
                B = (double)njc * ((ncen * g.wseg + g.threads - 1) / g.threads) * (round_up(g.wlen, ASW_WB) + 2) * c_w +
                    (njc > 1 ? njc * 400.0 : 0.0) +
                    (double)((g.nL * (g.Dc / 4) + g.threads - 1) / g.threads) * c_e +
                    (double)((g.nL + g.nR + g.threads - 1) / g.threads) * c_stage;
            const double d_util = (double)nD / ((double)nch * g.Dc);
            const int xt = (W + g.Tx - 1) / g.Tx;
            const double x_util = (double)W / ((double)xt * g.Tx);
            const double nwg = (double)xt * std::max(rows, 1) * nch, slots = 256.0 * k;
            const double tail = nwg / (std::ceil(nwg / slots) * slots);
            const double overlap = k > 1 ? 1.05 : 1.0;
            const int wps = k * per_simd;
            const double occ = wps >= 3 ? 1.0 : (wps == 2 ? 0.85 : 0.6);
            const double useful = (double)win * Rx * ASW_RD * c_tap;
            const double score = (double)XG * DG / per_simd * occ * (useful / (M + B)) * d_util * x_util * tail * overlap;
            if (score > best_score) { best_score = score; best = g; found = true; }
            if (shortlist) {
                auto &slot = classes[{piped ? 80 : Rx, std::min(g.JC, 64), nch, waves}];
                if (score > slot.first) slot = {score, g};
            }
        }
        }
        if (DG <= 2) break;
    }
    if (found && !best.pipe && best.Rx == 8 && best.JC >= win && best.DG >= 33 && win > 16) {
        AswGeom g;
        if (asw_layout(g, win, best.XG, best.DG, 160 * 1024, 16, 8)) {
            g.nchunks = best.nchunks;
            best = g;
        }
    }
    if (found && !best.pipe) asw_pick_e_scheme(best, win);
    const int wave_rx = found ? asw_wave_pick(win, nD) : 0;
    if (wave_rx) best.wave_rx = wave_rx;
    if (shortlist && found) {
        std::vector<std::pair<double, AswGeom>> v;
        for (auto &kv : classes) v.push_back(kv.second);
        std::sort(v.begin(), v.end(), [](const auto &a, const auto &b) { return a.first > b.first; });
        shortlist->clear();
        if (wave_rx) {
            shortlist->push_back(best);
            AswWaveGeom wg;
            if (!tune().wave_rx && asw_wave_layout(wg, win, nD, 12 - wave_rx)) {
                AswGeom other = best;
                other.wave_rx = 12 - wave_rx;
                shortlist->push_back(other);
            }
            if (wave_rx == 4 && asw_wave_layout(wg, win, nD, 4) && wg.RD == 6) {
                AswGeom other = best;
                other.wave_rx = 4 | 16;
                shortlist->push_back(other);
            }
        }
        for (size_t i = 0; i < v.size() && i < (wave_rx ? 3u : 12u) && v[i].first > 0.6 * best_score; ++i) {
            if (!v[i].second.pipe) asw_pick_e_scheme(v[i].second, win);
            v[i].second.wave_rx = 0;
            shortlist->push_back(v[i].second);
        }
    }
    return found ? SSAMD_OK : fail(SSAMD_ELIMIT, "no ASW launch geometry fits LDS for winSize=%d nD=%d", win, nD);
}

int get_prox(Ctx &c, int win, double gammaP, hipStream_t s, const float **out)
{
    if (TableEntry *e = c.proxTabs.find(win, gammaP)) { *out = (const float *)e->dev.ptr; return SSAMD_OK; }
    if (c.proxTabs.entries.size() >= c.proxTabs.max_entries) {
        HIP_TRY(hipDeviceSynchronize());
        (void)hipFree(c.proxTabs.entries.back().dev.ptr);
        c.proxTabs.entries.pop_back();
    }
    c.proxTabs.entries.emplace_front();
    TableEntry &e = c.proxTabs.entries.front();
    e.k0 = win; e.k1 = gammaP;
    const int p = win / 2;
    e.host.resize((size_t)win * win);
    for (int i = 0; i < win; ++i)
        for (int j = 0; j < win; ++j) {
            const double di = i - p, dj = j - p;
#if SSAMD_W_FOLD
            e.host[(size_t)i * win + j] = (float)(-std::sqrt(di * di + dj * dj) / gammaP * 1.4426950408889634);
#else
            e.host[(size_t)i * win + j] = (float)glibc_exp(-std::sqrt(di * di + dj * dj) / gammaP);
#endif
        }
    int rc = e.dev.reserve(e.host.size() * 4);
    if (rc) { c.proxTabs.entries.pop_front(); return rc; }
    hipError_t he = hipMemcpyAsync(e.dev.ptr, e.host.data(), e.host.size() * 4, hipMemcpyHostToDevice, s);
    if (he != hipSuccess) {
        (void)hipFree(e.dev.ptr);
        c.proxTabs.entries.pop_front();
        return fail(SSAMD_EHIP, "hipMemcpyAsync(proximity table) failed: %s", hipGetErrorString(he));
    }
    *out = (const float *)e.dev.ptr;
    return SSAMD_OK;
}

int get_prox64(Ctx &c, int win, double gammaP, hipStream_t s, const double **out)
{
    if (TableEntry *e = c.proxTabs64.find(win, gammaP)) { *out = (const double *)e->dev.ptr; return SSAMD_OK; }
    if (c.proxTabs64.entries.size() >= c.proxTabs64.max_entries) {
        HIP_TRY(hipDeviceSynchronize());
        (void)hipFree(c.proxTabs64.entries.back().dev.ptr);
        c.proxTabs64.entries.pop_back();
    }
    c.proxTabs64.entries.emplace_front();
    TableEntry &e = c.proxTabs64.entries.front();
    e.k0 = win; e.k1 = gammaP;
    const int p = win / 2;
    e.host64.resize((size_t)win * win);
    for (int i = 0; i < win; ++i)
        for (int j = 0; j < win; ++j)
            {
                const double di = i - p, dj = j - p;
                e.host64[(size_t)i * win + j] = glibc_exp(-std::sqrt(di * di + dj * dj) / gammaP);
            }
    int rc = e.dev.reserve(e.host64.size() * 8);
    if (rc) { c.proxTabs64.entries.pop_front(); return rc; }
    hipError_t he = hipMemcpyAsync(e.dev.ptr, e.host64.data(), e.host64.size() * 8, hipMemcpyHostToDevice, s);
    if (he != hipSuccess) {
        (void)hipFree(e.dev.ptr);
        c.proxTabs64.entries.pop_front();
        return fail(SSAMD_EHIP, "hipMemcpyAsync(fp64 proximity table) failed: %s", hipGetErrorString(he));
    }
    *out = (const double *)e.dev.ptr;
    return SSAMD_OK;
}

int asw_exact_prepare(Ctx &c, int W, int rows, int win, int nD, double gammaC, bool consistent, bool direct, hipStream_t s,
                      AswExactQueue &q, AswExactQueue &raw, AswExactQueue &kernel_q)
{
    const size_t nout = (size_t)rows * W;
    if (nout >= ((size_t)1 << 32)) return fail(SSAMD_ELIMIT, "exact mode: more than 2^32 output pixels per call");
    const size_t all_cands = 2 * (nout * (size_t)nD + nout);
    size_t cap = std::min<size_t>(std::max<size_t>(4 * nout, std::min<size_t>(all_cands, (size_t)1 << 23)), (size_t)1 << 26);
    if (tune().exact_cap) cap = (size_t)tune().exact_cap;
    size_t rawcap = direct ? 0 : std::min<size_t>(std::max<size_t>(2 * nout, std::min<size_t>(all_cands, (size_t)1 << 23)), (size_t)1 << 26);
    if (!direct && tune().exact_cap) rawcap = std::max<size_t>(rawcap, cap);
    if (!direct && tune().exact_rawcap) rawcap = (size_t)tune().exact_rawcap;
    int rc;
    if ((rc = c.xqueue.reserve(cap * 8)) || (rc = c.xcost.reserve(cap * 8)) || (rc = c.xflags.reserve(64 + 4 * nout + (size_t)rows)) ||
        (rc = c.xslots.reserve(nout * 32)) || (rawcap && (rc = c.xraw.reserve(rawcap * 12))))
        return rc;
    c.xcap = (unsigned int)cap;
    c.xrawcap = (unsigned int)rawcap;
    HIP_TRY(hipMemsetAsync(c.xflags.ptr, 0, 64 + 4 * nout + (size_t)rows, s));
    q.entries = (u64 *)c.xqueue.ptr;
    q.ekeys = nullptr;
    q.counter = (unsigned int *)c.xflags.ptr;
    q.flagL = (unsigned char *)c.xflags.ptr + 64;
    q.flagR = consistent ? q.flagL + nout : nullptr;
    q.zeroL = q.flagL + 2 * nout;
    q.zeroR = consistent ? q.flagL + 3 * nout : nullptr;
    q.zrow = q.flagL + 4 * nout;
    q.W = (unsigned int)W;
    q.cap = (unsigned int)cap;
    q.tol = (uint32_t)std::min(1.0e6, (double)tune().exact_tol * std::max(1.0, 5.0 / gammaC) * std::max(1.0, win / 35.0));
    q.sat_abs = (float)(1.5 * 2.0 * 2.0 * ((double)win * win + 3.0) * 1.1102230246251565e-16 * 40.0);
    q.deep = 0xffffffffu;
    raw = AswExactQueue{};
    if (!direct) {
        raw = q;
        union { float f; uint32_t u; } sa; sa.f = q.sat_abs;
        raw.deep = 0xC0000000u - sa.u;
        raw.entries = (u64 *)c.xraw.ptr;
        raw.ekeys = (uint32_t *)((u64 *)c.xraw.ptr + rawcap);
        raw.counter = q.counter + 4;
        raw.flagL = raw.flagR = nullptr;
        raw.cap = (unsigned int)rawcap;
    }
    kernel_q = direct ? q : raw;
    return SSAMD_OK;
}

int asw_exact_pass(Ctx &c, const AswExactQueue &q, const AswExactQueue &raw, int H, int W, int row0, int rows, int win, int maxD, int minD, double gammaC, double gammaP,
                   bool consistent, bool direct, int16_t *d_disp, hipStream_t s)
{
    const int p = win / 2;
    const size_t nout = (size_t)rows * W, npix = (size_t)H * W;
    int rc;
    const double *d_prox = nullptr;
    if ((rc = get_prox64(c, win, gammaP, s, &d_prox))) return rc;
    if ((rc = c.xlabL.reserve(npix * 24)) || (rc = c.xlabR.reserve(npix * 24))) return rc;
    AswExactArgs x;
    x.recL = (const PixRec *)c.recL.ptr; x.recR = (const PixRec *)c.recR.ptr;
    x.labL = (const double *)c.xlabL.ptr; x.labR = (const double *)c.xlabR.ptr;
    x.prox = d_prox;
    x.keyL = direct ? nullptr : (u64 *)c.keyL.ptr; x.keyR = consistent ? (u64 *)c.keyR.ptr : nullptr;
    x.disp = d_disp;
    x.q = q;
    x.raw = raw;
    x.ecost = (double *)c.xcost.ptr;
    x.costL = (u64 *)c.xslots.ptr; x.costR = x.costL + nout;
    x.idxL = (uint32_t *)(x.costR + nout); x.idxR = x.idxL + nout;
    x.wslotL = x.idxR + nout; x.wslotR = x.wslotL + nout;
    {
        const size_t per = (size_t)win * win * 8;
        size_t wcap = std::min<size_t>(65536, ((size_t)64 << 20) / per);
        if (nout >= ((size_t)1 << 31)) wcap = 0;
        if (wcap && (rc = c.xwtab.reserve(wcap * 8 + wcap * per))) return rc;
        x.wcap = (unsigned int)wcap;
        x.wpix = (uint32_t *)c.xwtab.ptr;
        x.wtab = (double *)((char *)c.xwtab.ptr + wcap * 8);
    }
    x.H = H; x.W = W; x.win = win; x.pad = p; x.minD = minD; x.maxD = maxD; x.row0 = row0; x.rows = rows;
    x.gammaC = gammaC;
    Timed t(c, s, SSAMD_K_ASW_EXACT);
    {
        const int r0 = std::max(0, row0 - p), r1 = std::min(H, row0 + rows + p);
        const long long np2 = (long long)(r1 - r0) * W;
        const int blocks = (int)std::min<long long>((2 * np2 + 255) / 256, 256 * 8);
        hipLaunchKernelGGL(bgr2lab_f64_pair_kernel, dim3(blocks), dim3(256), 0, s, x.recL + (size_t)r0 * W, x.recR + (size_t)r0 * W,
                           (double *)c.xlabL.ptr + 3 * (size_t)r0 * W, (double *)c.xlabR.ptr + 3 * (size_t)r0 * W, np2);
    }
    const int pb = (int)std::min<long long>(((long long)nout + 255) / 256, 256 * 8);
    if (raw.entries) {
        hipLaunchKernelGGL(asw_exact_filter_kernel, dim3(256 * 8), dim3(256), 0, s, x);
        hipLaunchKernelGGL(asw_exact_escalate_kernel, dim3(pb), dim3(256), 0, s, x);
    }
    {
        const int zwin = std::min(win, EXACT_ZWIN_MAX - 1);
        const size_t zlds = (size_t)2 * zwin * (EXACT_ZSEG + 2 * (zwin / 2)) * 4;
        if ((rc = grant_dyn_lds(c, (const void *)asw_exact_zero_kernel, (int)zlds))) return rc;
        const long long segs = (long long)rows * ((W + EXACT_ZSEG - 1) / EXACT_ZSEG);
        hipLaunchKernelGGL(asw_exact_zero_kernel, dim3((unsigned)std::min<long long>(segs, 256 * 64)), dim3(256), zlds, s, x);
    }
    hipLaunchKernelGGL(asw_exact_winners_kernel, dim3(pb), dim3(256), 0, s, x);
    if (x.wcap) hipLaunchKernelGGL(asw_exact_wtab_kernel, dim3(256 * 4), dim3(256), 0, s, x);
    hipLaunchKernelGGL(asw_exact_eval_kernel, dim3((unsigned)(c.cus * 5)), dim3(64 * EXACT_WAVES), 0, s, x);
    hipLaunchKernelGGL(asw_exact_resolve_kernel, dim3(256 * 4), dim3(256), 0, s, x);
    hipLaunchKernelGGL(asw_exact_patch_kernel, dim3(pb), dim3(256), 0, s, x);
    HIP_TRY(hipGetLastError());
    ++c.exact_calls;
    return SSAMD_OK;
}

int launch_finalize(Ctx &c, int slot, bool lrcheck, int rows, int W, int16_t *d_disp, hipStream_t s,
                    int16_t *d_raw_right = nullptr)
{
    if (rows <= 0) return SSAMD_OK;
    Timed t(c, s, slot);
    if (d_raw_right) {
        const long long n = (long long)rows * W;
        const int blocks = (int)std::min<long long>((n + 255) / 256, 256 * 8);
        hipLaunchKernelGGL(wta_decode_kernel, dim3(blocks), dim3(256), 0, s, (const u64 *)c.keyL.ptr, d_disp, rows, W, 0);
        hipLaunchKernelGGL(wta_decode_kernel, dim3(blocks), dim3(256), 0, s, (const u64 *)c.keyR.ptr, d_raw_right, rows, W, 1);
    } else if (lrcheck) {
        const size_t lds = (((size_t)W * 2 + 15) & ~(size_t)15) + W;
        int rc = grant_dyn_lds(c, (const void *)lr_check_fill_kernel, (int)lds);
        if (rc) return rc;
        hipLaunchKernelGGL(lr_check_fill_kernel, dim3(rows), dim3(256), lds, s, (const u64 *)c.keyL.ptr,
                           (const u64 *)c.keyR.ptr, d_disp, rows, W);
    } else {
        const long long n = (long long)rows * W;
        const int blocks = (int)std::min<long long>((n + 255) / 256, 256 * 8);
        hipLaunchKernelGGL(wta_decode_kernel, dim3(blocks), dim3(256), 0, s, (const u64 *)c.keyL.ptr, d_disp, rows, W, 0);
    }
    HIP_TRY(hipGetLastError());
    return SSAMD_OK;
}

int asw_device_impl(Ctx &c, const uint8_t *dL, const uint8_t *dR, int H, int W, int row0, int rows, int win,
                    int maxD, int minD, double gammaC, double gammaP, int consistent, int16_t *d_disp,
                    float *d_costs, hipStream_t s, bool alternate = false, int16_t *d_raw_right = nullptr, const RemapSrc *rm = nullptr,
                    bool exact = false, int skip_at = 0, int skip = 0)
{
    int rc = check_common(H, W, win, minD, maxD, row0, rows);
    if (rc) return rc;
    if (skip < 0 || skip_at < 0 || skip_at + skip > rows) return fail(SSAMD_EINVAL, "bad row gap [%d,%d) in a range of %d rows", skip_at, skip_at + skip, rows);
    if (skip > 0 && (alternate || d_costs || d_raw_right)) return fail(SSAMD_EINVAL, "two row ranges: plain, consistent and exact matching only");
    if (skip == rows) return SSAMD_OK;
    if (!(gammaC > 0) || !(gammaP > 0)) return fail(SSAMD_EINVAL, "gammaC and gammaP must be positive");
    if (exact && (alternate || d_costs)) return fail(SSAMD_EINVAL, "the exact (fp64 tie-break) mode has no alternate-rows form and no cost dump");
    if (maxD < minD) exact = false;
    if (alternate && d_costs) return fail(SSAMD_EINVAL, "the alternate-rows mode has no cost dump");
    if (rows == 0) return SSAMD_OK;
    ScratchOrder order(c, s);
    const int p = win / 2, nD = maxD - minD + 1;
    const size_t npix = (size_t)H * W, nout = (size_t)rows * W;

    AswArgs a{};
    AswExactQueue xq_final{}, xq_raw{};
    const int grows = alternate ? (rows + 1) / 2 : rows - skip;
    if (nD >= 1 && (rc = asw_choose_geometry(a.g, W, grows, win, nD))) return rc;
    const std::array<int, 4> shape{W, grows, win, nD};
    std::vector<AswGeom> trial;
    const double call_taps = (double)W * grows * nD * win * win;
    const int tune_mode = g_autotune.load();
    const bool tune_now = (tune_mode > 0 || (tune_mode < 0 && call_taps <= ASW_AUTOTUNE_SMALL_TAPS));
    bool tuned_already;
    { std::lock_guard<std::mutex> glk(g_geom_mutex); tuned_already = g_asw_geom_tuned.count(shape) != 0; }
    if (tune_now && nD >= 1 && !asw_geometry_forced() && !tuned_already) {
        AswGeom tmp;
        if (asw_search_geometry(tmp, W, grows, win, nD, &trial) != SSAMD_OK || trial.size() < 2) trial.clear();
    }
    const size_t evol_cap_max = tune().evol_max_mb ? std::min((size_t)24 << 30, (size_t)tune().evol_max_mb << 20) : (size_t)24 << 30;
    size_t evol_limit_cached = 0;
    bool evol_limit_known = false;
    auto evol_fits = [&](size_t bytes) {
        if (bytes > evol_cap_max) return false;
        if (bytes <= c.evol.cap) return true;
        if (!evol_limit_known) {
            size_t free_b = 0, total_b = 0;
            evol_limit_cached = evol_cap_max;
            if (hipMemGetInfo(&free_b, &total_b) == hipSuccess) evol_limit_cached = std::min(evol_cap_max, c.evol.cap + free_b / 2);
            else (void)hipGetLastError();
            evol_limit_known = true;
        }
        return bytes <= evol_limit_cached;
    };
    auto wave_volume_fits = [&](const AswGeom &g) {
        AswWaveGeom wg;
        if (!g.wave_rx || !asw_wave_layout(wg, win, nD, g.wave_rx)) return !g.wave_rx;
        const int xt = (W + wg.Txw - 1) / wg.Txw, erows = std::min(H, row0 + rows + win / 2) - std::max(0, row0 - win / 2);
        return evol_fits((size_t)erows * (size_t)round_up(xt * wg.Txw + 2 * (win / 2), 4) * (size_t)wg.Se + 4096);
    };
    if (nD >= 1 && a.g.wave_rx && !wave_volume_fits(a.g)) ++c.evol_fallbacks;
    if (nD >= 1 && !wave_volume_fits(a.g)) a.g.wave_rx = 0;
    trial.erase(std::remove_if(trial.begin(), trial.end(), [&](const AswGeom &g) { return !wave_volume_fits(g); }), trial.end());
    if (trial.size() < 2) trial.clear();
    auto is_direct = [&](const AswGeom &g) { return nD >= 1 && (g.nchunks == 1 || g.wave_rx) && !consistent; };
    bool need_keys = !is_direct(a.g) || alternate;
    for (const AswGeom &g : trial) need_keys = need_keys || !is_direct(g);
    if (need_keys) {
        if ((rc = c.keyL.reserve(nout * 8))) return rc;
        HIP_TRY(hipMemsetAsync(c.keyL.ptr, 0xFF, nout * 8, s));
    }
    if (consistent) {
        if ((rc = c.keyR.reserve(nout * 8))) return rc;
        HIP_TRY(hipMemsetAsync(c.keyR.ptr, 0xFF, nout * 8, s));
    }

    if (nD >= 1) {
        if ((rc = c.recL.reserve(npix * sizeof(PixRec)))) return rc;
        if ((rc = c.recR.reserve(npix * sizeof(PixRec)))) return rc;
        const float *d_prox = nullptr;
        if ((rc = get_prox(c, win, gammaP, s, &d_prox))) return rc;
        const int r0 = std::max(0, row0 - p), r1 = std::min(H, row0 + rows + p);
        const long long np2 = (long long)(r1 - r0) * W;
        const int lab_blocks = (int)std::min<long long>((2 * np2 + 255) / 256, 256 * 8);
        auto launch_lab = [&]() -> int {
            Timed t(c, s, SSAMD_K_LAB);
            if (rm)
                hipLaunchKernelGGL(remap_lab_records_pair_kernel, dim3(lab_blocks), dim3(256), 0, s, *rm, (PixRec *)c.recL.ptr, (PixRec *)c.recR.ptr,
                                   (long long)r0 * W, np2);
            else
                hipLaunchKernelGGL(bgr2lab_records_pair_kernel, dim3(lab_blocks), dim3(256), 0, s, dL + (size_t)r0 * W * 3, dR + (size_t)r0 * W * 3,
                                   (PixRec *)c.recL.ptr + (size_t)r0 * W, (PixRec *)c.recR.ptr + (size_t)r0 * W, np2);
            HIP_TRY(hipGetLastError());
            return SSAMD_OK;
        };
        bool lab_pending = trial.empty() && !rm && tune().prepass_fuse != 0;
        if (!lab_pending && (rc = launch_lab())) return rc;

        a.recL = (const PixRec *)c.recL.ptr; a.recR = (const PixRec *)c.recR.ptr;
        a.prox = d_prox;
        a.keyR = consistent ? (u64 *)c.keyR.ptr : nullptr;
        a.costs = d_costs;
        a.cost_keys = 0;
        a.xq = AswExactQueue{};
        a.H = H; a.W = W; a.win = win; a.pad = p; a.minD = minD; a.maxD = maxD; a.row0 = row0; a.rows = rows;
        a.kC = (float)(-1.4426950408889634 / gammaC);
        a.ystep = alternate ? 2 : 1;
        a.yskip_at = skip > 0 ? skip_at : 0x7fffffff; a.yskip = skip;
        a.evol = nullptr; a.erow0 = r0; a.erows = r1 - r0; a.evolW = 0;
        AswWaveArgs wa;
        auto prepare_evol = [&](const AswGeom &g) -> int {
            a.evol = nullptr;
            int chunks = g.nchunks, Tx = g.Tx, Dc = g.Dc, Se = g.Se;
            if (g.wave_rx) {
                if (!asw_wave_layout(wa.g, win, nD, g.wave_rx, !d_costs && tune().wave_unroll != 0))
                    return fail(SSAMD_ELIMIT, "wave kernel geometry does not fit LDS");
                chunks = 1; Tx = wa.g.Txw; Dc = wa.g.Dc; Se = wa.g.Se;
            } else if (!g.pipe || tune().asw_evol == 0) {
                return SSAMD_OK;
            }
            const int xt = (W + Tx - 1) / Tx;
            const int evolW = round_up(xt * Tx + 2 * p + (g.wave_rx ? 0 : Tx / 2 + 8), 4);
            const size_t bytes = (size_t)chunks * (size_t)(r1 - r0) * (size_t)evolW * (size_t)Se;
            if (c.evol.cap > ((size_t)256 << 20) && (bytes + 4096) * 4 < c.evol.cap) {
                if (trial.empty() && ++c.evol_small_calls >= 8) {
                    (void)hipStreamSynchronize(s);
                    c.evol.release();
                    c.evol_small_calls = 0;
                }
            } else {
                c.evol_small_calls = 0;
            }
            int erc = SSAMD_ENOMEM;
            if (tune().evol_fail) {
                void *none = nullptr;
                size_t free_b = 0, total_b = (size_t)512 << 30;
                (void)hipMemGetInfo(&free_b, &total_b);
                if (hipMalloc(&none, 2 * total_b) == hipSuccess) (void)hipFree(none);
            } else if (evol_fits(bytes + 4096)) {
                erc = c.evol.reserve(bytes + 4096);
            }
            if (erc) {
                (void)hipGetLastError();
                if (g.wave_rx) return fail(erc == SSAMD_ENOMEM ? SSAMD_ENOMEM : erc, "TAD volume of %zu bytes does not fit the device memory left", bytes);
                ++c.evol_fallbacks;
                g_err.clear();
                return SSAMD_OK;
            }
            a.evol = (const unsigned char *)c.evol.ptr;
            a.evolW = evolW;
            Timed t(c, s, SSAMD_K_LAB);
            const dim3 egrid((unsigned)((evolW + TADV_COLS - 1) / TADV_COLS), (unsigned)(r1 - r0), (unsigned)chunks);
            const size_t elds = (size_t)(2 * TADV_COLS + Dc) * 4;
            const long long tiles = (long long)egrid.x * egrid.y * egrid.z;
            if (lab_pending && tiles + lab_blocks < (1ll << 31)) {
                AswPrepassArgs pa;
                pa.bgrL = dL; pa.bgrR = dR; pa.recL = (PixRec *)c.recL.ptr; pa.recR = (PixRec *)c.recR.ptr;
                pa.evol = (unsigned char *)c.evol.ptr; pa.npix_total = (long long)H * W;
                pa.W = W; pa.pad = p; pa.minD = minD; pa.Dc = Dc; pa.Se = Se; pa.erow0 = r0; pa.erows = r1 - r0; pa.evolW = evolW;
                pa.rd = g.wave_rx ? wa.g.RD : 4;
                pa.lab_blocks = lab_blocks; pa.ex = (int)egrid.x; pa.ey = (int)egrid.y;
                if (int grc = grant_dyn_lds(c, (const void *)asw_prepass_kernel, (int)elds)) return grc;
                hipLaunchKernelGGL(asw_prepass_kernel, dim3((unsigned)(tiles + lab_blocks)), dim3(256), elds, s, pa);
                HIP_TRY(hipGetLastError());
                lab_pending = false;
                return SSAMD_OK;
            }
            if (lab_pending) {
                lab_pending = false;
                if (int lrc = launch_lab()) return lrc;
            }
            if (int grc = grant_dyn_lds(c, (const void *)asw_tad_volume_kernel, (int)elds)) return grc;
            hipLaunchKernelGGL(asw_tad_volume_kernel, egrid, dim3(256), elds, s, (const PixRec *)c.recL.ptr, (const PixRec *)c.recR.ptr,
                               (unsigned char *)c.evol.ptr, W, p, minD, Dc, Se, r0, r1 - r0, evolW, g.wave_rx ? wa.g.RD : 4);
            HIP_TRY(hipGetLastError());
            return SSAMD_OK;
        };
        auto launch = [&](const AswGeom &g) -> int {
            a.g = g;
            a.keyL = is_direct(g) ? nullptr : (u64 *)c.keyL.ptr;
            a.disp = is_direct(g) ? d_disp : nullptr;
            if (g.wave_rx) {
                wa.recL = a.recL; wa.recR = a.recR; wa.prox = a.prox;
                wa.keyL = a.keyL; wa.keyR = a.keyR; wa.disp = a.disp; wa.costs = a.costs; wa.cost_keys = a.cost_keys; wa.xq = a.xq;
                wa.evol = a.evol; wa.erow0 = a.erow0; wa.erows = a.erows; wa.evolW = a.evolW;
                wa.H = H; wa.W = W; wa.win = win; wa.pad = p; wa.minD = minD; wa.maxD = maxD; wa.row0 = row0; wa.rows = rows;
                wa.ystep = a.ystep; wa.kC = a.kC; wa.yb0 = 0; wa.yskip_at = a.yskip_at; wa.yskip = a.yskip;
                auto wk = wa.g.RX == 8 ? (d_costs ? asw_aggregate_wave_kernel<true, 8> : asw_aggregate_wave_kernel<false, 8>)
                                       : (d_costs ? asw_aggregate_wave_kernel<true, 4> : asw_aggregate_wave_kernel<false, 4>);
                const int kl = (wa.g.Txw + 63) / 64, kr = (wa.g.nRcw + 63) / 64;
                const bool unrolled = tune().wave_unroll != 0;
                if (wa.g.RD == 6) {
                    wk = d_costs ? asw_aggregate_wave6_kernel<true, 0> : asw_aggregate_wave6_kernel<false, 0>;
                    if (unrolled && !d_costs && wa.g.K == 3) wk = wa.g.creg ? asw_aggregate_wave6_kernel<false, 3, true> : asw_aggregate_wave6_kernel<false, 3>;
                    else if (unrolled && !d_costs && wa.g.K == 2) wk = wa.g.creg ? asw_aggregate_wave6_kernel<false, 2, true> : asw_aggregate_wave6_kernel<false, 2>;
                } else if (unrolled && !d_costs && wa.g.merged) {
                    const int key = wa.g.RX * 10 + wa.g.K;
                    if (key == 42) wk = wa.g.creg ? asw_aggregate_wave_kernel<false, 4, 0, 0, 2, true> : asw_aggregate_wave_kernel<false, 4, 0, 0, 2>;
                    else if (key == 43) wk = wa.g.creg ? asw_aggregate_wave_kernel<false, 4, 0, 0, 3, true> : asw_aggregate_wave_kernel<false, 4, 0, 0, 3>;
                    else if (key == 44) wk = wa.g.creg ? asw_aggregate_wave_kernel<false, 4, 0, 0, 4, true> : asw_aggregate_wave_kernel<false, 4, 0, 0, 4>;
                    else if (key == 82) wk = asw_aggregate_wave_kernel<false, 8, 0, 0, 2>;
                    else if (key == 83) wk = asw_aggregate_wave_kernel<false, 8, 0, 0, 3>;
                    else if (key == 84) wk = asw_aggregate_wave_kernel<false, 8, 0, 0, 4>;
                } else if (unrolled && !d_costs) {
                    const int key = wa.g.RX * 100 + kl * 10 + kr;
                    if (key == 822) wk = asw_aggregate_wave_kernel<false, 8, 2, 2>;
                    else if (key == 812) wk = asw_aggregate_wave_kernel<false, 8, 1, 2>;
                    else if (key == 412) wk = asw_aggregate_wave_kernel<false, 4, 1, 2>;
                    else if (key == 422) wk = asw_aggregate_wave_kernel<false, 4, 2, 2>;
                    else if (key == 423) wk = asw_aggregate_wave_kernel<false, 4, 2, 3>;
                }
                const int lds = wa.g.wave_lds * wa.g.waves, xt = (W + wa.g.Txw - 1) / wa.g.Txw;
                if (int grc = grant_dyn_lds(c, (const void *)wk, lds)) return grc;
                hipLaunchKernelGGL(wk, dim3((xt + wa.g.waves - 1) / wa.g.waves, grows, 1), dim3(64 * wa.g.waves), lds, s, wa);
                HIP_TRY(hipGetLastError());
                return SSAMD_OK;
            }
            const dim3 grid((W + g.Tx - 1) / g.Tx, grows, g.nchunks), block(g.threads);
            const bool chunked = g.JC < win;
            if (g.pipe) {
                auto pk = d_costs ? asw_aggregate_pipe_kernel<true> : asw_aggregate_pipe_kernel<false>;
                if (tune().asw_static != 0) {
                    if (g.SL == 120 && g.SR == 316 && g.Se == 208) pk = d_costs ? asw_aggregate_pipe_kernel<true, 120, 316, 208> : asw_aggregate_pipe_kernel<false, 120, 316, 208>;
                    else if (g.SL == 88 && g.SR == 348 && g.Se == 272) pk = d_costs ? asw_aggregate_pipe_kernel<true, 88, 348, 272> : asw_aggregate_pipe_kernel<false, 88, 348, 272>;
                    else if (g.SL == 216 && g.SR == 284 && g.Se == 80) pk = d_costs ? asw_aggregate_pipe_kernel<true, 216, 284, 80> : asw_aggregate_pipe_kernel<false, 216, 284, 80>;
                }
                if (tune().asw_static == 2 && !d_costs) {
                    auto is_tile = [&](AswPipeTileId id) { return win == id.win && asw_pipe_geom_matches(g, asw_pipe_geom_constexpr(id)); };
                    if (is_tile(AswPipeTile<120, 316, 208>::id)) pk = asw_aggregate_pipe_kernel<false, 120, 316, 208, true>;
                    else if (is_tile(AswPipeTile<88, 348, 272>::id)) pk = asw_aggregate_pipe_kernel<false, 88, 348, 272, true>;
                    else if (is_tile(AswPipeTile<216, 284, 80>::id)) pk = asw_aggregate_pipe_kernel<false, 216, 284, 80, true>;
                    else ++c.static_tile_mismatch;
                }
                const int pipe_lds = a.evol ? g.lds_bytes_evol : g.lds_bytes;
                if (pipe_lds > 160 * 1024) return fail(SSAMD_ELIMIT, "this tile needs the TAD volume (LDS %d bytes without it)", pipe_lds);
                if (int grc = grant_dyn_lds(c, (const void *)pk, pipe_lds)) return grc;
                int rows_main = grows;
                AswGeom tail_g;
                if (!alternate && tune().asw_tail != 0 && g.XG >= 4) {
                    const int per_simd = (g.threads / 64 + 3) / 4;
                    const long long resident = std::max(1, std::min(3 / std::max(1, per_simd), (160 * 1024) / std::max(1, pipe_lds)));
                    const long long per_row = (long long)grid.x * g.nchunks, n = per_row * grows, slots = (long long)c.cus * resident;
                    const long long full = n / slots, rem = n - full * slots;
                    if (full >= 1 && rem > 0 && 2 * rem <= slots && (full < 32 || tune().asw_tail > 0)) {
                        const int rm = (int)(full * slots / per_row);
                        if (rm >= 1 && rm < grows &&
                            asw_layout_e(tail_g, win, (g.XG + 1) / 2, g.DG, 160 * 1024, g.JC, 8, true, false, true) && tail_g.pipe &&
                            tail_g.Se == g.Se && tail_g.Dc == g.Dc &&
                            (a.evol == nullptr || round_up(((W + tail_g.Tx - 1) / tail_g.Tx) * tail_g.Tx + 2 * p, 4) <= a.evolW)) {
                            tail_g.nchunks = g.nchunks;
                            rows_main = rm;
                        }
                    }
                }
                hipLaunchKernelGGL(pk, dim3(grid.x, rows_main, grid.z), block, pipe_lds, s, a);
                HIP_TRY(hipGetLastError());
                if (rows_main < grows) {
                    ++c.tail_splits;
                    AswArgs t = a;
                    t.g = tail_g;
                    t.yb0 = rows_main;
                    auto tk = d_costs ? asw_aggregate_pipe_kernel<true> : asw_aggregate_pipe_kernel<false>;
                    const int tail_lds = a.evol ? tail_g.lds_bytes_evol : tail_g.lds_bytes;
                    if (int grc = grant_dyn_lds(c, (const void *)tk, tail_lds)) return grc;
                    hipLaunchKernelGGL(tk, dim3((W + tail_g.Tx - 1) / tail_g.Tx, grows - rows_main, tail_g.nchunks), dim3(tail_g.threads),
                                       tail_lds, s, t);
                    HIP_TRY(hipGetLastError());
                }
                return SSAMD_OK;
            }
            auto kern = chunked ? (d_costs ? asw_aggregate_kernel<true, true> : asw_aggregate_kernel<false, true>)
                                : (d_costs ? asw_aggregate_kernel<true, false> : asw_aggregate_kernel<false, false>);
            if (g.Rx == 4)
                kern = chunked ? (d_costs ? asw_aggregate_kernel<true, true, 4> : asw_aggregate_kernel<false, true, 4>)
                               : (d_costs ? asw_aggregate_kernel<true, false, 4> : asw_aggregate_kernel<false, false, 4>);
            if (int grc = grant_dyn_lds(c, (const void *)kern, g.lds_bytes)) return grc;
            hipLaunchKernelGGL(kern, grid, block, g.lds_bytes, s, a);
            HIP_TRY(hipGetLastError());
            return SSAMD_OK;
        };
        if (!trial.empty()) {
            hipEvent_t e0 = nullptr, e1 = nullptr;
            HIP_TRY(hipEventCreate(&e0));
            HIP_TRY(hipEventCreate(&e1));
            std::vector<float> cand_ms(trial.size(), 3.0e38f);
            bool all_prepared = true;
            const bool want_evol = tune().asw_evol != 0;
            for (const AswGeom &g : trial) {
                if (prepare_evol(g) != SSAMD_OK) { all_prepared = false; continue; }
                if (g.pipe && !g.wave_rx && want_evol && !a.evol) all_prepared = false;
                if (launch(g) != SSAMD_OK) all_prepared = false;
            }
            for (int round = 0; round < 4; ++round)
                for (size_t ci = 0; ci < trial.size(); ++ci) {
                    float ms = 3.0e38f;
                    if (hipEventRecord(e0, s) == hipSuccess && prepare_evol(trial[ci]) == SSAMD_OK && launch(trial[ci]) == SSAMD_OK &&
                        hipEventRecord(e1, s) == hipSuccess && hipEventSynchronize(e1) == hipSuccess)
                        (void)hipEventElapsedTime(&ms, e0, e1);
                    else
                        all_prepared = false;
                    if (trial[ci].pipe && !trial[ci].wave_rx && want_evol && !a.evol) all_prepared = false;
                    if (round > 0) cand_ms[ci] = std::min(cand_ms[ci], ms);
                }
            AswGeom fastest = a.g;
            float best_ms = 3.0e38f;
            for (size_t ci = 0; ci < trial.size(); ++ci)
                if (cand_ms[ci] < best_ms * (ci == 0 ? 1.0f : 0.985f)) { best_ms = cand_ms[ci]; fastest = trial[ci]; }
            (void)hipEventDestroy(e0);
            (void)hipEventDestroy(e1);
            if (all_prepared) {
                std::lock_guard<std::mutex> glk(g_geom_mutex);
                g_asw_geom_cache[shape] = fastest;
                g_asw_geom_tuned[shape] = true;
            } else {
                g_err.clear();
            }
            a.g = fastest;
        }
        {
            AswGeom final_geom = a.g;
            rc = prepare_evol(final_geom);
            if (rc == SSAMD_ENOMEM && final_geom.wave_rx) {
                ++c.evol_fallbacks;
                g_err.clear();
                final_geom.wave_rx = 0;
                a.g = final_geom;
                if (!is_direct(final_geom) && !need_keys) {
                    if ((rc = c.keyL.reserve(nout * 8))) return rc;
                    HIP_TRY(hipMemsetAsync(c.keyL.ptr, 0xFF, nout * 8, s));
                    need_keys = true;
                }
                rc = prepare_evol(final_geom);
            }
            if (rc) return rc;
            if (final_geom.pipe && !final_geom.wave_rx && !a.evol && final_geom.lds_bytes > 160 * 1024) {
                t_pipe_full_lds = true;
                AswGeom g2;
                const int r2 = asw_search_geometry(g2, W, grows, win, nD);
                t_pipe_full_lds = false;
                if (r2) return r2;
                g2.wave_rx = 0;
                if (!is_direct(g2) && !need_keys) {
                    if ((rc = c.keyL.reserve(nout * 8))) return rc;
                    HIP_TRY(hipMemsetAsync(c.keyL.ptr, 0xFF, nout * 8, s));
                }
                final_geom = g2;
                if ((rc = prepare_evol(final_geom))) return rc;
            }
            if (lab_pending) {
                lab_pending = false;
                if ((rc = launch_lab())) return rc;
            }
            if (exact) {
                if (!trial.empty()) {
                    if (need_keys) HIP_TRY(hipMemsetAsync(c.keyL.ptr, 0xFF, nout * 8, s));
                    if (consistent) HIP_TRY(hipMemsetAsync(c.keyR.ptr, 0xFF, nout * 8, s));
                }
                if ((rc = asw_exact_prepare(c, W, rows, win, nD, gammaC, consistent != 0, is_direct(final_geom), s, xq_final, xq_raw, a.xq))) return rc;
            }
            Timed t(c, s, SSAMD_K_ASW_AGG);
            if ((rc = launch(final_geom))) return rc;
        }
    }
    const bool direct = is_direct(a.g);
    if (exact && nD >= 1 &&
        (rc = asw_exact_pass(c, xq_final, xq_raw, H, W, row0, rows, win, maxD, minD, gammaC, gammaP, consistent != 0, direct, d_disp, s)))
        return rc;
    if (!direct && skip > 0) {
        const auto band = [&](int b0, int nb) -> int {
            if (nb <= 0) return SSAMD_OK;
            const size_t off = (size_t)b0 * W;
            Timed t(c, s, SSAMD_K_ASW_FIN);
            if (consistent) {
                const size_t lds = (((size_t)W * 2 + 15) & ~(size_t)15) + W;
                if (int grc = grant_dyn_lds(c, (const void *)lr_check_fill_kernel, (int)lds)) return grc;
                hipLaunchKernelGGL(lr_check_fill_kernel, dim3(nb), dim3(256), lds, s, (const u64 *)c.keyL.ptr + off, (const u64 *)c.keyR.ptr + off,
                                   d_disp + off, nb, W);
            } else {
                const long long n = (long long)nb * W;
                hipLaunchKernelGGL(wta_decode_kernel, dim3((int)std::min<long long>((n + 255) / 256, 256 * 8)), dim3(256), 0, s,
                                   (const u64 *)c.keyL.ptr + off, d_disp + off, nb, W, 0);
            }
            HIP_TRY(hipGetLastError());
            return SSAMD_OK;
        };
        if ((rc = band(0, skip_at)) || (rc = band(skip_at + skip, rows - skip_at - skip))) return rc;
    } else if (!direct && (rc = launch_finalize(c, SSAMD_K_ASW_FIN, consistent != 0, rows, W, d_disp, s, d_raw_right))) return rc;
    if (alternate && rows > 1) {
        AswAltArgs f;
        const size_t nodd = (size_t)(rows / 2) * W;
        if ((double)nodd * ((nD + 7) / 8 + 1) >= 4.0e9)
            return fail(SSAMD_ELIMIT, "alternate-rows mode: image x disparity range too large for the 32-bit job counter");
        f.cap = (unsigned int)std::min<size_t>(std::max<size_t>(nodd, 1 << 16), 1u << 28);
        if (tune().alt_queue_cap)
            f.cap = (unsigned int)tune().alt_queue_cap;
        if ((rc = c.altq.reserve((size_t)f.cap * 8 + 16))) return rc;
        f.ctr = (unsigned int *)c.altq.ptr; f.queue = (u64 *)((char *)c.altq.ptr + 16);
        HIP_TRY(hipMemsetAsync(f.ctr, 0, 16, s));
        f.recL = (const PixRec *)c.recL.ptr; f.recR = (const PixRec *)c.recR.ptr; f.prox = a.prox;
        f.disp = d_disp; f.key = (u64 *)c.keyL.ptr;
        f.H = H; f.W = W; f.win = win; f.pad = p; f.minD = minD; f.maxD = maxD; f.row0 = row0; f.rows = rows;
        f.kC = (float)(-1.4426950408889634 / gammaC);
        const dim3 pix_grid((W + 255) / 256, rows / 2);
        Timed t(c, s, SSAMD_K_ASW_ALT);
        hipLaunchKernelGGL(asw_alt_scan_kernel, pix_grid, dim3(256), 0, s, f);
        hipLaunchKernelGGL(asw_alt_jobs_kernel, dim3(256 * 8), dim3(256), 0, s, f);
        hipLaunchKernelGGL(asw_alt_decode_kernel, pix_grid, dim3(256), 0, s, f);
        HIP_TRY(hipGetLastError());
    }
    return SSAMD_OK;
}


int asw_alternate_rows(Ctx &c, const uint8_t *dL, const uint8_t *dR, int H, int W, int row0, int rows, int row_parity, int win,
                       int maxD, int minD, double gammaC, double gammaP, int consistent, int16_t *d_disp, hipStream_t s)
{
    int rc = check_common(H, W, win, minD, maxD, row0, rows);
    if (rc) return rc;
    if (rows == 0) return SSAMD_OK;
    const bool top_odd = ((row0 + row_parity) & 1) != 0, bottom_odd = ((row0 + rows - 1 + row_parity) & 1) != 0;
    if (top_odd && row0 == 0)
        return fail(SSAMD_EINVAL, "alternate rows: the first output row is an odd row of the image, the sub-image must start at least one row above it");
    const int e0 = top_odd ? row0 - 1 : row0, e1 = bottom_odd ? std::min(H, row0 + rows + 1) : row0 + rows;
    if (e0 == row0 && e1 == row0 + rows)
        return asw_device_impl(c, dL, dR, H, W, row0, rows, win, maxD, minD, gammaC, gammaP, consistent, d_disp, nullptr, s, true);
    ScratchOrder order(c, s);
    if ((rc = c.altdisp.reserve((size_t)(e1 - e0) * W * 2))) return rc;
    rc = asw_device_impl(c, dL, dR, H, W, e0, e1 - e0, win, maxD, minD, gammaC, gammaP, consistent, (int16_t *)c.altdisp.ptr, nullptr, s, true);
    if (rc) return rc;
    HIP_TRY(hipMemcpyAsync(d_disp, (const int16_t *)c.altdisp.ptr + (size_t)(row0 - e0) * W, (size_t)rows * W * 2, hipMemcpyDeviceToDevice, s));
    return SSAMD_OK;
}

bool gsw_layout(GswGeom &g, int win, int XG, int DG, int Ty, size_t limit, int Hy = 1)
{
    const int p = win / 2;
    g.XG = XG; g.DG = DG; g.Ty = Ty; g.Rd = Ty == 2 ? 4 : 8; g.Hy = Hy;
    g.Tx = GSW_RX * XG; g.Dc = g.Rd * DG;
    g.threads = round_up(XG * DG, 64);
    g.nL = g.Tx + 2 * p;
    g.nT = g.nL + g.Dc - 1;
    int P = 1;
    while (8 * P < g.Dc) P <<= 1;
    g.Se = 8 * P;
    g.Ses = 3;
    while ((1 << g.Ses) < g.Se) ++g.Ses;
    g.emask = std::min(P, 32) - 1;
    size_t off = 0;
    auto take = [&](size_t bytes) { size_t o = off; off = (off + bytes + 15) & ~(size_t)15; return (int)o; };
    g.off_w = take((size_t)Ty * Hy * win * g.Tx * 4);
    const int nL4 = round_up(g.nL, 4);
    g.off_e = take((size_t)nL4 * g.Se * 4);
    g.off_ref = take((size_t)nL4 * 16 * 2);
    g.off_tgt = take((size_t)(g.nT + nL4 - g.nL) * 16 * 2);
    g.off_best = take((size_t)Ty * Hy * g.Tx * 8);
    g.off_cen = take((size_t)Ty * Hy * g.Tx * 4);
    g.lds_bytes = (int)off;
    return off <= limit && g.threads * Hy <= GSW_MAX_THREADS;
}

int gsw_search_geometry(GswGeom &best, int W, int rows, int win, int nD);

std::map<std::array<int, 4>, GswGeom> g_gsw_geom_cache;
std::map<std::array<int, 4>, bool> g_gsw_geom_tuned;

int gsw_choose_geometry(GswGeom &best, int W, int rows, int win, int nD)
{
    if (!tune().gsw_geom.empty()) return gsw_search_geometry(best, W, rows, win, nD);
    std::lock_guard<std::mutex> glk(g_geom_mutex);
    const std::array<int, 4> key{W, rows, win, nD};
    auto it = g_gsw_geom_cache.find(key);
    if (it != g_gsw_geom_cache.end()) { best = it->second; return SSAMD_OK; }
    const int rc = gsw_search_geometry(best, W, rows, win, nD);
    if (rc == SSAMD_OK) {
        if (g_gsw_geom_cache.size() > 256) { g_gsw_geom_cache.clear(); g_gsw_geom_tuned.clear(); }
        g_gsw_geom_cache[key] = best;
    }
    return rc;
}

void gsw_candidates(std::vector<GswGeom> &out, const GswGeom &model, int W, int rows, int win, int nD)
{
    out.clear();
    out.push_back(model);
    const int Ty = 2, Rd = 4;
    if (rows < 2) return;
    for (int nch = model.nchunks; nch <= model.nchunks + 1 && nch <= nD; ++nch) {
        const int per = (nD + nch - 1) / nch, DG = round_up(per, Rd) / Rd;
        if (DG > 64 || (nD + DG * Rd - 1) / (DG * Rd) != nch) continue;
        for (int Hy : {1, 2, 4}) {
            if (Ty * Hy > std::max(rows, 2)) break;
            for (int T : {32, 64, 128, 192, 256, 384, 512}) {
                if (T * Hy > GSW_MAX_THREADS) break;
                for (int trim = 0; trim < 2; ++trim) {
                    const int XG = std::min((T / DG) * (6 - trim) / 6, (W + GSW_RX - 1) / GSW_RX);
                    if (XG < 2) continue;
                    GswGeom g;
                    if (!gsw_layout(g, win, XG, DG, Ty, 160 * 1024, Hy)) continue;
                    g.nchunks = nch;
                    bool dup = false;
                    for (const GswGeom &o : out) dup = dup || (o.XG == g.XG && o.DG == g.DG && o.Ty == g.Ty && o.Hy == g.Hy && o.nchunks == g.nchunks);
                    if (!dup && out.size() < 36) out.push_back(g);
                }
            }
        }
    }
}

int gsw_search_geometry(GswGeom &best, int W, int rows, int win, int nD)
{
    if (!tune().gsw_geom.empty()) {
        const char *const env = tune().gsw_geom.c_str();
        int XG = 0, DG = 0, Ty = 1, Hy = 1;
        if (sscanf(env, "%d,%d,%d,%d", &XG, &DG, &Ty, &Hy) >= 2 && XG >= 1 && DG >= 1 && (Ty == 1 || Ty == 2) && Hy >= 1 && Hy <= 8 &&
            XG * DG <= GSW_MAX_THREADS && gsw_layout(best, win, XG, DG, Ty, 160 * 1024, Hy)) {
            best.nchunks = (nD + best.Dc - 1) / best.Dc;
            return SSAMD_OK;
        }
        return fail(SSAMD_EINVAL, "SSAMD_GSW_GEOM=%s is not a usable geometry", env);
    }
    const double c_tap = 5.3, c_w = 60.0, c_e = 70.0;
    double best_score = -1.0;
    bool found = false;
    for (int Ty = 1; Ty <= 2; ++Ty) {
        if (Ty > std::max(rows, 1)) break;
        const int Rd = Ty == 2 ? 4 : 8;
        for (int nch = 1; nch <= nD; ++nch) {
            const int per = (nD + nch - 1) / nch;
            const int DG = round_up(per, Rd) / Rd;
            if (DG > 64) continue;
            if ((nD + DG * Rd - 1) / (DG * Rd) != nch) continue;
            const int xg_cap = std::min(GSW_MAX_THREADS / DG, (W + GSW_RX - 1) / GSW_RX);
            for (int Hy = 1; Hy <= 1; Hy *= 2)
            for (int XG = xg_cap; XG >= 1; --XG) {
                GswGeom g;
                if (!gsw_layout(g, win, XG, DG, Ty, 160 * 1024, Hy)) continue;
                g.nchunks = nch;
                const int tot = g.threads * Hy, TyS = Ty * Hy;
                const int waves = tot / 64, per_simd = (waves + 3) / 4;
                const int k = std::min({4 / per_simd, (160 * 1024) / g.lds_bytes, 8});
                if (k < 1) continue;
                const double M = (double)win * GSW_RX * Rd * c_tap;
                const double Bw = (double)((g.Tx * win + tot - 1) / tot) * c_w;
                const double Be = (double)((g.nL * g.Dc + tot - 1) / tot) * c_e;
                const double strip = (double)(win + TyS - 1) * Be + (double)TyS * win * Bw + (double)Ty * win * M;
                const double eff = (double)Ty * win * M / strip;
                const double d_util = (double)nD / ((double)nch * g.Dc);
                const int xt = (W + g.Tx - 1) / g.Tx, yt = (std::max(rows, 1) + TyS - 1) / TyS;
                const double x_util = (double)W / ((double)xt * g.Tx);
                const double y_util = (double)std::max(rows, 1) / ((double)yt * TyS);
                const double nwg = (double)xt * yt * nch, slots = 256.0 * k;
                const double tail = nwg / (std::ceil(nwg / slots) * slots);
                const double score = (double)k * XG * DG * Hy * eff * d_util * x_util * y_util * tail;
                if (score > best_score) { best_score = score; best = g; found = true; }
            }
            if (DG <= 1) break;
        }
    }
    return found ? SSAMD_OK : fail(SSAMD_ELIMIT, "no GSW launch geometry fits LDS for winSize=%d nD=%d", win, nD);
}

int get_gsw_table(Ctx &c, int gamma, hipStream_t s, const float **out)
{
    if (TableEntry *e = c.gswTabs.find(gamma, 0.0)) { *out = (const float *)e->dev.ptr; return SSAMD_OK; }
    if (c.gswTabs.entries.size() >= c.gswTabs.max_entries) {
// ... 12 lines not shown
    int rc = e.dev.reserve(e.host.size() * 4);
    if (rc) { c.gswTabs.entries.pop_front(); return rc; }
    hipError_t he = hipMemcpyAsync(e.dev.ptr, e.host.data(), e.host.size() * 4, hipMemcpyHostToDevice, s);
    if (he != hipSuccess) {
        (void)hipFree(e.dev.ptr);
        c.gswTabs.entries.pop_front();
        return fail(SSAMD_EHIP, "hipMemcpyAsync(GSW weight table) failed: %s", hipGetErrorString(he));
    }
    *out = (const float *)e.dev.ptr;
    return SSAMD_OK;
}

int gsw_device_impl(Ctx &c, const uint8_t *dL, const uint8_t *dR, int H, int W, int row0, int rows, int win, int maxD,
                    int minD, int gamma, float fMax, int iterations, int16_t *d_disp, hipStream_t s, const RemapSrc *rm = nullptr)
{
    int rc = check_common(H, W, win, minD, maxD, row0, rows);
    if (rc) return rc;
    if (gamma == 0) return fail(SSAMD_EINVAL, "gamma must be non-zero");
    if (rows == 0) return SSAMD_OK;
    ScratchOrder order(c, s);
    const int p = win / 2, nD = maxD - minD + 1;
    const size_t npix = (size_t)H * W, nout = (size_t)rows * W;
    if ((rc = c.keyL.reserve(nout * 8)) || (rc = c.keyR.reserve(nout * 8))) return rc;
    HIP_TRY(hipMemsetAsync(c.keyL.ptr, 0xFF, nout * 8, s));
    HIP_TRY(hipMemsetAsync(c.keyR.ptr, 0xFF, nout * 8, s));
    if (nD >= 1) {
        if ((rc = c.recL.reserve(npix * 4)) || (rc = c.recR.reserve(npix * 4))) return rc;
        const float *d_tab = nullptr;
        if ((rc = get_gsw_table(c, gamma, s, &d_tab))) return rc;
        const int r0 = std::max(0, row0 - p), r1 = std::min(H, row0 + rows + p);
        const long long np = (long long)(r1 - r0) * W;
        const int blocks = (int)std::min<long long>((np + 255) / 256, 256 * 8);
        {
            Timed t(c, s, SSAMD_K_LAB);
            if (rm) {
                hipLaunchKernelGGL(remap_pack_pair_kernel, dim3(blocks), dim3(256), 0, s, *rm, (uint32_t *)c.recL.ptr, (uint32_t *)c.recR.ptr,
                                   (long long)r0 * W, np);
            } else {
                hipLaunchKernelGGL(bgr_pack_kernel, dim3(blocks), dim3(256), 0, s, dL + (size_t)r0 * W * 3,
                                   (uint32_t *)c.recL.ptr + (size_t)r0 * W, np);
                hipLaunchKernelGGL(bgr_pack_kernel, dim3(blocks), dim3(256), 0, s, dR + (size_t)r0 * W * 3,
                                   (uint32_t *)c.recR.ptr + (size_t)r0 * W, np);
            }
            HIP_TRY(hipGetLastError());
        }
        GswArgs a;
        if ((rc = gsw_choose_geometry(a.g, W, rows, win, nD))) return rc;
        a.tab = d_tab;
        a.H = H; a.W = W; a.win = win; a.pad = p; a.minD = minD; a.maxD = maxD; a.row0 = row0; a.rows = rows;
        a.iterations = iterations; a.fMax = fMax;
        auto launch = [&](const GswGeom &g) -> int {
            a.g = g;
            const int TyS = g.Ty * g.Hy;
            const dim3 grid((W + g.Tx - 1) / g.Tx, (rows + TyS - 1) / TyS, g.nchunks), block(g.threads * g.Hy);
            auto kernel = g.Ty == 2 ? gsw_aggregate_kernel<2, 4> : gsw_aggregate_kernel<1, 8>;
            if (int grc = grant_dyn_lds(c, (const void *)kernel, g.lds_bytes)) return grc;
            for (int pass = 0; pass < 2; ++pass) {
                a.right = pass;
                a.ref = (const uint32_t *)(pass ? c.recR.ptr : c.recL.ptr);
                a.tgt = (const uint32_t *)(pass ? c.recL.ptr : c.recR.ptr);
                a.key = (u64 *)(pass ? c.keyR.ptr : c.keyL.ptr);
                hipLaunchKernelGGL(kernel, grid, block, g.lds_bytes, s, a);
                HIP_TRY(hipGetLastError());
            }
            return SSAMD_OK;
        };
        {
            const std::array<int, 4> shape{W, rows, win, nD};
            const double call_taps = 2.0 * (double)W * rows * nD * win * win;
            const int tune_mode = g_autotune.load();
            bool tuned_already;
            { std::lock_guard<std::mutex> glk(g_geom_mutex); tuned_already = g_gsw_geom_tuned.count(shape) != 0; }
            if ((tune_mode > 0 || (tune_mode < 0 && call_taps <= ASW_AUTOTUNE_SMALL_TAPS)) && tune().gsw_geom.empty() && !tuned_already) {
                std::vector<GswGeom> trial;
                gsw_candidates(trial, a.g, W, rows, win, nD);
                if (trial.size() >= 2) {
                    hipEvent_t e0 = nullptr, e1 = nullptr;
                    HIP_TRY(hipEventCreate(&e0));
                    if (hipEventCreate(&e1) != hipSuccess) {
                        (void)hipEventDestroy(e0);
                        return fail(SSAMD_EHIP, "hipEventCreate failed");
                    }
                    std::vector<float> cand_ms(trial.size(), 3.0e38f), warm_ms(trial.size(), 3.0e38f);
                    std::vector<char> alive(trial.size(), 1);
                    for (int round = 0; round < 3; ++round) {
                        for (size_t ci = 0; ci < trial.size(); ++ci) {
                            if (!alive[ci]) continue;
                            float ms = 3.0e38f;
                            if (hipEventRecord(e0, s) == hipSuccess && launch(trial[ci]) == SSAMD_OK && hipEventRecord(e1, s) == hipSuccess &&
                                hipEventSynchronize(e1) == hipSuccess)
                                (void)hipEventElapsedTime(&ms, e0, e1);
                            if (round > 0) cand_ms[ci] = std::min(cand_ms[ci], ms);
                            else warm_ms[ci] = ms;
                        }
                        if (round == 0) {
                            const float wbest = *std::min_element(warm_ms.begin(), warm_ms.end());
                            for (size_t ci = 1; ci < trial.size(); ++ci) alive[ci] = warm_ms[ci] <= 2.0f * wbest;
                        }
                    }
                    (void)hipGetLastError();
                    g_err.clear();
                    GswGeom fastest = trial[0];
                    float best_ms = 3.0e38f;
                    for (size_t ci = 0; ci < trial.size(); ++ci)
                        if (cand_ms[ci] < best_ms * (ci == 0 ? 1.0f : 0.985f)) { best_ms = cand_ms[ci]; fastest = trial[ci]; }
                    (void)hipEventDestroy(e0);
                    (void)hipEventDestroy(e1);
                    std::lock_guard<std::mutex> glk(g_geom_mutex);
                    g_gsw_geom_cache[shape] = fastest;
                    g_gsw_geom_tuned[shape] = true;
                    a.g = fastest;
                }
            }
        }
        {
            const GswGeom final_geom = a.g;
            Timed t(c, s, SSAMD_K_GSW_AGG);
            if ((rc = launch(final_geom))) return rc;
        }
    }
    return launch_finalize(c, SSAMD_K_GSW_FIN, true, rows, W, d_disp, s);
}

}

namespace {

struct HostJob {
    const uint8_t *img1, *img2;
    int H, W, win, maxD, minD;
    int o0, o1;
    int16_t *disparity;
    double gammaC, gammaP; int consistent; float *costs; bool alternate;
    bool exact;
    int16_t *raw_right;
    int gamma; float fMax; int iterations;
};

int asw_host_rows(const HostJob &j, int device)
{
    CtxLock c;
    int rc = get_ctx(device, c);
    if (rc) return rc;
    if ((rc = check_common(j.H, j.W, j.win, j.minD, j.maxD, j.o0, j.o1 - j.o0))) return rc;
    const int p = j.win / 2 + (j.alternate ? 1 : 0);
    const int in0 = std::max(0, j.o0 - p), in1 = std::min(j.H, j.o1 + p), rows = j.o1 - j.o0;
    const size_t nb = (size_t)(in1 - in0) * j.W * 3, nout = (size_t)rows * j.W;
    if ((rc = c->imgL.reserve(nb)) || (rc = c->imgR.reserve(nb)) || (rc = c->disp.reserve(nout * 2))) return rc;
    const size_t ncost = j.costs ? nout * (size_t)std::max(1, j.maxD - j.minD + 1) : 0;
    if (j.costs && (rc = c->costs.reserve(ncost * 4))) return rc;
    if (j.raw_right && (rc = c->lab.reserve(nout * 2))) return rc;
    hipStream_t s = c->stream;
    HIP_TRY(hipMemcpyAsync(c->imgL.ptr, j.img1 + (size_t)in0 * j.W * 3, nb, hipMemcpyHostToDevice, s));
    HIP_TRY(hipMemcpyAsync(c->imgR.ptr, j.img2 + (size_t)in0 * j.W * 3, nb, hipMemcpyHostToDevice, s));
    if (j.costs) HIP_TRY(hipMemsetAsync(c->costs.ptr, 0xFF, ncost * 4, s));
    if (j.alternate)
        rc = asw_alternate_rows(*c, (const uint8_t *)c->imgL.ptr, (const uint8_t *)c->imgR.ptr, in1 - in0, j.W, j.o0 - in0, rows, in0 & 1,
                                j.win, j.maxD, j.minD, j.gammaC, j.gammaP, j.consistent, (int16_t *)c->disp.ptr, s);
    else
        rc = asw_device_impl(*c, (const uint8_t *)c->imgL.ptr, (const uint8_t *)c->imgR.ptr, in1 - in0, j.W, j.o0 - in0, rows,
                             j.win, j.maxD, j.minD, j.gammaC, j.gammaP, j.consistent, (int16_t *)c->disp.ptr,
                             j.costs ? (float *)c->costs.ptr : nullptr, s, false,
                             j.raw_right ? (int16_t *)c->lab.ptr : nullptr, nullptr, j.exact);
    if (rc) return rc;
    if (j.raw_right)
        HIP_TRY(hipMemcpyAsync(j.raw_right + (size_t)j.o0 * j.W, c->lab.ptr, nout * 2, hipMemcpyDeviceToHost, s));
    if (j.disparity)
        HIP_TRY(hipMemcpyAsync(j.disparity + (size_t)j.o0 * j.W, c->disp.ptr, nout * 2, hipMemcpyDeviceToHost, s));
    if (j.costs) HIP_TRY(hipMemcpyAsync(j.costs, c->costs.ptr, ncost * 4, hipMemcpyDeviceToHost, s));
    HIP_TRY(hipStreamSynchronize(s));
    return SSAMD_OK;
}

int gsw_host_rows(const HostJob &j, int device)
{
    CtxLock c;
    int rc = get_ctx(device, c);
    if (rc) return rc;
    if ((rc = check_common(j.H, j.W, j.win, j.minD, j.maxD, j.o0, j.o1 - j.o0))) return rc;
    const int p = j.win / 2, in0 = std::max(0, j.o0 - p), in1 = std::min(j.H, j.o1 + p), rows = j.o1 - j.o0;
    const size_t nb = (size_t)(in1 - in0) * j.W * 3, nout = (size_t)rows * j.W;
    if ((rc = c->imgL.reserve(nb)) || (rc = c->imgR.reserve(nb)) || (rc = c->disp.reserve(nout * 2))) return rc;
    hipStream_t s = c->stream;
    HIP_TRY(hipMemcpyAsync(c->imgL.ptr, j.img1 + (size_t)in0 * j.W * 3, nb, hipMemcpyHostToDevice, s));
    HIP_TRY(hipMemcpyAsync(c->imgR.ptr, j.img2 + (size_t)in0 * j.W * 3, nb, hipMemcpyHostToDevice, s));
    rc = gsw_device_impl(*c, (const uint8_t *)c->imgL.ptr, (const uint8_t *)c->imgR.ptr, in1 - in0, j.W, j.o0 - in0, rows,
                         j.win, j.maxD, j.minD, j.gamma, j.fMax, j.iterations, (int16_t *)c->disp.ptr, s);
    if (rc) return rc;
    HIP_TRY(hipMemcpyAsync(j.disparity + (size_t)j.o0 * j.W, c->disp.ptr, nout * 2, hipMemcpyDeviceToHost, s));
    HIP_TRY(hipStreamSynchronize(s));
    return SSAMD_OK;
}

int run_strips(const HostJob &job, const int *devices, int n_devices, int (*fn)(const HostJob &, int))
{
    if (!devices || n_devices < 1) return fail(SSAMD_EINVAL, "devices must name at least one GPU");
    if (n_devices > 16) return fail(SSAMD_EINVAL, "at most 16 devices");
    for (int a = 0; a < n_devices; ++a) {
        if (devices[a] < 0) return fail(SSAMD_EINVAL, "devices[%d] = %d: explicit non-negative ordinals only", a, devices[a]);
        for (int b = 0; b < a && !tune().multi_allow_repeat; ++b)
            if (devices[a] == devices[b]) return fail(SSAMD_EINVAL, "device %d listed twice", devices[a]);
    }
    int rc = check_common(job.H, job.W, job.win, job.minD, job.maxD, 0, job.H);
    if (rc) return rc;
    const int base = job.H / n_devices, extra = job.H % n_devices;
    std::vector<int> codes(n_devices, SSAMD_OK);
    std::vector<std::string> msgs(n_devices);
    std::vector<std::thread> th;
    for (int k = 0; k < n_devices; ++k) {
        HostJob j = job;
        j.o0 = k * base + std::min(k, extra);
        j.o1 = j.o0 + base + (k < extra ? 1 : 0);
        if (j.o1 <= j.o0) continue;
        const int dev = devices[k];
        try {
            th.emplace_back([j, dev, k, fn, &codes, &msgs]() {
                codes[k] = fn(j, dev);
                if (codes[k]) msgs[k] = g_err;
            });
        } catch (const std::exception &e) {
            codes[k] = SSAMD_ENOMEM;
            msgs[k] = std::string("could not start a host thread: ") + e.what();
            break;
        }
    }
    for (auto &t : th) t.join();
    for (int k = 0; k < n_devices; ++k)
        if (codes[k]) return fail(codes[k], "strip %d on device %d: %s", k, devices[k], msgs[k].c_str());
    return SSAMD_OK;
}

HostJob asw_job(const uint8_t *img1, const uint8_t *img2, int H, int W, int win, int maxD, int minD, double gammaC,
                double gammaP, int consistent, int16_t *disparity, float *costs, bool alternate)
{
    HostJob j{};
    j.img1 = img1; j.img2 = img2; j.H = H; j.W = W; j.win = win; j.maxD = maxD; j.minD = minD; j.o0 = 0; j.o1 = H;
    j.disparity = disparity; j.gammaC = gammaC; j.gammaP = gammaP; j.consistent = consistent; j.costs = costs;
    j.alternate = alternate;
    return j;
}

HostJob gsw_job(const uint8_t *img1, const uint8_t *img2, int H, int W, int win, int maxD, int minD, int gamma, float fMax,
                int iterations, int16_t *disparity)
{
    HostJob j{};
    j.img1 = img1; j.img2 = img2; j.H = H; j.W = W; j.win = win; j.maxD = maxD; j.minD = minD; j.o0 = 0; j.o1 = H;
    j.disparity = disparity; j.gamma = gamma; j.fMax = fMax; j.iterations = iterations;
    return j;
}

}

extern "C" {

int ssamd_abi_version(void) { return SSAMD_ABI_VERSION; }
const char *ssamd_last_error(void) { return g_err.c_str(); }

int ssamd_device_count(void)
{
    int n = 0;
    if (hipGetDeviceCount(&n) != hipSuccess) return 0;
    return n;
}

const char *ssamd_kernel_name(int slot)
{
    static const char *names[SSAMD_K_COUNT] = {"asw pre-pass (asw_prepass_kernel: Lab records + TAD volume; or bgr2lab_records_pair_kernel, asw_tad_volume_kernel)", "asw aggregation kernel (asw_aggregate_pipe / _wave / asw_aggregate_kernel)",
                                               "asw finalize (wta_decode / lr_check_fill)",
                                               "gsw_aggregate_kernel", "gsw finalize (lr_check_fill)", "remap_bgr_kernel", "reproject_kernel",
                                               "asw_alt_fill_kernel", "asw fp64 tie-break pass (bgr2lab_f64_pair + asw_exact_winners / _eval / _resolve / _patch kernels)",
                                               "iir_unwrap_kernel"};
    return (slot >= 0 && slot < SSAMD_K_COUNT) ? names[slot] : "";
}

int ssamd_set_option(const char *name, const char *value)
{
    if (!name) return fail(SSAMD_EINVAL, "option name is NULL");
    std::lock_guard<std::mutex> lk(g_tune_mutex);
    if (value) {
        if (!tuning_assign(g_tuning, name, value)) return fail(SSAMD_EINVAL, "unknown option %s", name);
    } else {
        const auto it = g_tuning_env.find(name);
        if (!tuning_assign(g_tuning, name, it == g_tuning_env.end() ? nullptr : it->second.c_str()))
            return fail(SSAMD_EINVAL, "unknown option %s", name);
    }
    if (std::string(name) == "SSAMD_AUTOTUNE")
        g_autotune.store(g_tuning.autotune_env != -2 ? g_tuning.autotune_env : -1);
    g_tune_version.fetch_add(1, std::memory_order_release);
    return SSAMD_OK;
}

int ssamd_counter(int device, const char *name, long long *value)
{
    if (!name || !value) return fail(SSAMD_EINVAL, "name / value is NULL");
    CtxLock c;
    int rc = get_ctx(device, c);
    if (rc) return rc;
    const std::string n(name);
    if (n == "evol_fallbacks") *value = c->evol_fallbacks;
    else if (n == "evol_bytes") *value = (long long)c->evol.cap;
    else if (n == "tail_splits") *value = c->tail_splits;
    else if (n == "exact_calls") *value = c->exact_calls;
    else if (n == "static_tile_mismatch") *value = c->static_tile_mismatch;
    else if (n == "exact_entries" || n == "exact_flagged_left" || n == "exact_flagged_right" || n == "exact_overflow" || n == "exact_raw_entries") {
        unsigned int ctr[5] = {0, 0, 0, 0, 0};
        if (c->xflags.ptr && c->exact_calls > 0) {
            HIP_TRY(hipDeviceSynchronize());
            HIP_TRY(hipMemcpy(ctr, c->xflags.ptr, sizeof(ctr), hipMemcpyDeviceToHost));
        }
        *value = n == "exact_entries" ? ctr[0] : n == "exact_flagged_left" ? ctr[1] : n == "exact_flagged_right" ? ctr[2] :
                 n == "exact_raw_entries" ? ctr[4] : ((ctr[0] > c->xcap || (c->xrawcap && ctr[4] > c->xrawcap)) ? 1 : 0);
    }
    else return fail(SSAMD_EINVAL, "unknown counter %s", name);
    return SSAMD_OK;
}

int ssamd_autotune(int on)
{
    return g_autotune.exchange(on > 0 ? 1 : (on < 0 ? -1 : 0));
}

int ssamd_asw_geometry(int width, int rows, int winSize, int maxDisparity, int minDisparity, int *out)
{
    if (!out) return fail(SSAMD_EINVAL, "out is NULL");
    int rc = check_common(1 << 14, width, winSize, minDisparity, maxDisparity, 0, 0);
    if (rc) return rc;
    const int nD = maxDisparity - minDisparity + 1;
    if (nD < 1) return fail(SSAMD_EINVAL, "empty disparity range");
    AswGeom g;
    if ((rc = asw_choose_geometry(g, width, rows, winSize, nD))) return rc;
    out[0] = g.Tx; out[1] = g.Dc; out[2] = g.nchunks; out[3] = g.threads; out[4] = g.lds_bytes;
    out[5] = (width + g.Tx - 1) / g.Tx; out[6] = rows; out[7] = g.nchunks;
    AswWaveGeom wg;
    if (g.wave_rx && asw_wave_layout(wg, winSize, nD, g.wave_rx, tune().wave_unroll != 0)) {
        out[0] = wg.Txw * wg.waves; out[1] = wg.Dc; out[2] = 1; out[3] = 64 * wg.waves; out[4] = wg.wave_lds * wg.waves;
        out[5] = (width + out[0] - 1) / out[0]; out[7] = 1;
    }
    return SSAMD_OK;
}

int ssamd_asw_kernel_form(int width, int rows, int winSize, int maxDisparity, int minDisparity, int *out)
{
    if (!out) return fail(SSAMD_EINVAL, "out is NULL");
    int rc = check_common(1 << 14, width, winSize, minDisparity, maxDisparity, 0, 0);
    if (rc) return rc;
    const int nD = maxDisparity - minDisparity + 1;
    if (nD < 1) return fail(SSAMD_EINVAL, "empty disparity range");
    AswGeom g;
    if ((rc = asw_choose_geometry(g, width, rows, winSize, nD))) return rc;
    out[0] = g.pipe; out[1] = g.Rx; out[2] = g.JC >= winSize ? 0 : g.JC; out[3] = g.pipe ? g.dephase : 0;
    out[4] = g.wave_rx & 15;
    if (g.wave_rx) { out[0] = 0; out[1] = g.wave_rx & 15; out[2] = 0; out[3] = 0; }
    return SSAMD_OK;
}

int ssamd_gsw_geometry(int width, int rows, int winSize, int maxDisparity, int minDisparity, int *out)
{
    if (!out) return fail(SSAMD_EINVAL, "out is NULL");
    int rc = check_common(1 << 14, width, winSize, minDisparity, maxDisparity, 0, 0);
    if (rc) return rc;
    const int nD = maxDisparity - minDisparity + 1;
    if (nD < 1) return fail(SSAMD_EINVAL, "empty disparity range");
    GswGeom g;
    if ((rc = gsw_choose_geometry(g, width, rows, winSize, nD))) return rc;
    out[0] = g.Tx; out[1] = g.Dc; out[2] = g.nchunks; out[3] = g.threads * g.Hy; out[4] = g.lds_bytes;
    out[5] = (width + g.Tx - 1) / g.Tx; out[6] = (rows + g.Ty * g.Hy - 1) / (g.Ty * g.Hy); out[7] = g.nchunks; out[8] = g.Ty * g.Hy;
    return SSAMD_OK;
}

int ssamd_asw_device(const uint8_t *d_img1, const uint8_t *d_img2, int height, int width, int out_row0, int out_rows,
                     int winSize, int maxDisparity, int minDisparity, double gammaC, double gammaP, int consistent,
                     int16_t *d_disparity, void *stream)
{
    if (!d_img1 || !d_img2 || !d_disparity) return fail(SSAMD_EINVAL, "NULL buffer");
    CtxLock c;
    int rc = get_ctx(-1, c);
    if (rc) return rc;
    return asw_device_impl(*c, d_img1, d_img2, height, width, out_row0, out_rows, winSize, maxDisparity, minDisparity,
                           gammaC, gammaP, consistent, d_disparity, nullptr, (hipStream_t)stream);
}

int ssamd_asw_device_rows2(const uint8_t *d_img1, const uint8_t *d_img2, int height, int width, int out_row0, int out_rows,
                           int skip_row0, int skip_rows, int winSize, int maxDisparity, int minDisparity, double gammaC, double gammaP,
                           int consistent, int16_t *d_disparity, void *stream)
{
    if (!d_img1 || !d_img2 || !d_disparity) return fail(SSAMD_EINVAL, "NULL buffer");
    CtxLock c;
    int rc = get_ctx(-1, c);
    if (rc) return rc;
    if (skip_rows < 0 || (skip_rows > 0 && (skip_row0 < out_row0 || skip_row0 + skip_rows > out_row0 + out_rows)))
        return fail(SSAMD_EINVAL, "the skipped rows [%d,%d) must lie inside the output rows [%d,%d)", skip_row0, skip_row0 + skip_rows,
                    out_row0, out_row0 + out_rows);
    return asw_device_impl(*c, d_img1, d_img2, height, width, out_row0, out_rows, winSize, maxDisparity, minDisparity, gammaC, gammaP,
                           consistent, d_disparity, nullptr, (hipStream_t)stream, false, nullptr, nullptr, false,
                           skip_rows > 0 ? skip_row0 - out_row0 : 0, skip_rows);
}

int ssamd_asw_exact_device(const uint8_t *d_img1, const uint8_t *d_img2, int height, int width, int out_row0, int out_rows,
                           int winSize, int maxDisparity, int minDisparity, double gammaC, double gammaP, int consistent,
                           int16_t *d_disparity, void *stream)
{
    if (!d_img1 || !d_img2 || !d_disparity) return fail(SSAMD_EINVAL, "NULL buffer");
    CtxLock c;
    int rc = get_ctx(-1, c);
    if (rc) return rc;
    return asw_device_impl(*c, d_img1, d_img2, height, width, out_row0, out_rows, winSize, maxDisparity, minDisparity,
                           gammaC, gammaP, consistent, d_disparity, nullptr, (hipStream_t)stream, false, nullptr, nullptr, true);
}

int ssamd_asw_exact_device_rows2(const uint8_t *d_img1, const uint8_t *d_img2, int height, int width, int out_row0, int out_rows,
                                 int skip_row0, int skip_rows, int winSize, int maxDisparity, int minDisparity, double gammaC, double gammaP,
                                 int consistent, int16_t *d_disparity, void *stream)
{
    if (!d_img1 || !d_img2 || !d_disparity) return fail(SSAMD_EINVAL, "NULL buffer");
    CtxLock c;
    int rc = get_ctx(-1, c);
    if (rc) return rc;
    if (skip_rows < 0 || (skip_rows > 0 && (skip_row0 < out_row0 || skip_row0 + skip_rows > out_row0 + out_rows)))
        return fail(SSAMD_EINVAL, "the skipped rows [%d,%d) must lie inside the output rows [%d,%d)", skip_row0, skip_row0 + skip_rows,
                    out_row0, out_row0 + out_rows);
    return asw_device_impl(*c, d_img1, d_img2, height, width, out_row0, out_rows, winSize, maxDisparity, minDisparity, gammaC, gammaP,
                           consistent, d_disparity, nullptr, (hipStream_t)stream, false, nullptr, nullptr, true,
                           skip_rows > 0 ? skip_row0 - out_row0 : 0, skip_rows);
}

int ssamd_asw_exact_rectified_device(const uint8_t *d_raw1, const uint8_t *d_raw2, int src_height, int src_width,
                                     const float *d_mapx1, const float *d_mapy1, const float *d_mapx2, const float *d_mapy2,
                                     int height, int width, int interpolation, int winSize, int maxDisparity, int minDisparity,
                                     double gammaC, double gammaP, int consistent, int16_t *d_disparity, void *stream)
{
    if (!d_raw1 || !d_raw2 || !d_mapx1 || !d_mapy1 || !d_mapx2 || !d_mapy2 || !d_disparity) return fail(SSAMD_EINVAL, "NULL buffer");
    if (src_height <= 0 || src_width <= 0) return fail(SSAMD_EINVAL, "Wrong image dimensions!");
    if (interpolation != 0 && interpolation != 1) return fail(SSAMD_EINVAL, "only INTER_NEAREST (0) and INTER_LINEAR (1) are supported");
    CtxLock c;
    int rc = get_ctx(-1, c);
    if (rc) return rc;
    RemapSrc rm;
    rm.src1 = d_raw1; rm.src2 = d_raw2; rm.mapx1 = d_mapx1; rm.mapy1 = d_mapy1; rm.mapx2 = d_mapx2; rm.mapy2 = d_mapy2;
    rm.Hs = src_height; rm.Ws = src_width; rm.nearest = interpolation == 0 ? 1 : 0;
    return asw_device_impl(*c, nullptr, nullptr, height, width, 0, height, winSize, maxDisparity, minDisparity, gammaC, gammaP, consistent,
                           d_disparity, nullptr, (hipStream_t)stream, false, nullptr, &rm, true);
}

int ssamd_asw_exact(const uint8_t *img1, const uint8_t *img2, int height, int width, int winSize, int maxDisparity,
                    int minDisparity, double gammaC, double gammaP, int consistent, int16_t *disparity, int device)
{
    if (!img1 || !img2 || !disparity) return fail(SSAMD_EINVAL, "NULL buffer");
    HostJob j = asw_job(img1, img2, height, width, winSize, maxDisparity, minDisparity, gammaC, gammaP, consistent, disparity, nullptr, false);
    j.exact = true;
    return asw_host_rows(j, device);
}

int ssamd_asw_rectified_device(const uint8_t *d_raw1, const uint8_t *d_raw2, int src_height, int src_width,
                               const float *d_mapx1, const float *d_mapy1, const float *d_mapx2, const float *d_mapy2,
                               int height, int width, int interpolation, int winSize, int maxDisparity, int minDisparity,
                               double gammaC, double gammaP, int consistent, int16_t *d_disparity, void *stream)
{
    if (!d_raw1 || !d_raw2 || !d_mapx1 || !d_mapy1 || !d_mapx2 || !d_mapy2 || !d_disparity) return fail(SSAMD_EINVAL, "NULL buffer");
    if (src_height <= 0 || src_width <= 0) return fail(SSAMD_EINVAL, "Wrong image dimensions!");
    if (interpolation != 0 && interpolation != 1) return fail(SSAMD_EINVAL, "only INTER_NEAREST (0) and INTER_LINEAR (1) are supported");
    CtxLock c;
    int rc = get_ctx(-1, c);
    if (rc) return rc;
    RemapSrc rm;
    rm.src1 = d_raw1; rm.src2 = d_raw2; rm.mapx1 = d_mapx1; rm.mapy1 = d_mapy1; rm.mapx2 = d_mapx2; rm.mapy2 = d_mapy2;
    rm.Hs = src_height; rm.Ws = src_width; rm.nearest = interpolation == 0 ? 1 : 0;
    return asw_device_impl(*c, nullptr, nullptr, height, width, 0, height, winSize, maxDisparity, minDisparity, gammaC, gammaP, consistent,
                           d_disparity, nullptr, (hipStream_t)stream, false, nullptr, &rm);
}

int ssamd_asw(const uint8_t *img1, const uint8_t *img2, int height, int width, int winSize, int maxDisparity,
              int minDisparity, double gammaC, double gammaP, int consistent, int16_t *disparity, int device)
{
    if (!img1 || !img2 || !disparity) return fail(SSAMD_EINVAL, "NULL buffer");
    return asw_host_rows(asw_job(img1, img2, height, width, winSize, maxDisparity, minDisparity, gammaC, gammaP, consistent,
                                 disparity, nullptr, false), device);
}

int ssamd_asw_multi(const uint8_t *img1, const uint8_t *img2, int height, int width, int winSize, int maxDisparity,
                    int minDisparity, double gammaC, double gammaP, int consistent, int16_t *disparity,
                    const int *devices, int n_devices)
{
    if (!img1 || !img2 || !disparity) return fail(SSAMD_EINVAL, "NULL buffer");
    return run_strips(asw_job(img1, img2, height, width, winSize, maxDisparity, minDisparity, gammaC, gammaP, consistent,
                              disparity, nullptr, false), devices, n_devices, asw_host_rows);
}

int ssamd_asw_exact_multi(const uint8_t *img1, const uint8_t *img2, int height, int width, int winSize, int maxDisparity,
                          int minDisparity, double gammaC, double gammaP, int consistent, int16_t *disparity,
                          const int *devices, int n_devices)
{
    if (!img1 || !img2 || !disparity) return fail(SSAMD_EINVAL, "NULL buffer");
    HostJob j = asw_job(img1, img2, height, width, winSize, maxDisparity, minDisparity, gammaC, gammaP, consistent, disparity, nullptr, false);
    j.exact = true;
    return run_strips(j, devices, n_devices, asw_host_rows);
}

int ssamd_asw_alternate(const uint8_t *img1, const uint8_t *img2, int height, int width, int winSize, int maxDisparity,
                        int minDisparity, double gammaC, double gammaP, int consistent, int16_t *disparity, int device)
{
    if (!img1 || !img2 || !disparity) return fail(SSAMD_EINVAL, "NULL buffer");
    return asw_host_rows(asw_job(img1, img2, height, width, winSize, maxDisparity, minDisparity, gammaC, gammaP, consistent,
                                 disparity, nullptr, true), device);
}

int ssamd_asw_alternate_device(const uint8_t *d_img1, const uint8_t *d_img2, int height, int width, int winSize,
                               int maxDisparity, int minDisparity, double gammaC, double gammaP, int consistent,
                               int16_t *d_disparity, void *stream)
{
    if (!d_img1 || !d_img2 || !d_disparity) return fail(SSAMD_EINVAL, "NULL buffer");
    CtxLock c;
    int rc = get_ctx(-1, c);
    if (rc) return rc;
    return asw_device_impl(*c, d_img1, d_img2, height, width, 0, height, winSize, maxDisparity, minDisparity, gammaC,
                           gammaP, consistent, d_disparity, nullptr, (hipStream_t)stream, true);
}

int ssamd_asw_alternate_rows_device(const uint8_t *d_img1, const uint8_t *d_img2, int height, int width, int out_row0, int out_rows,
                                    int row_parity, int winSize, int maxDisparity, int minDisparity, double gammaC, double gammaP,
                                    int consistent, int16_t *d_disparity, void *stream)
{
    if (!d_img1 || !d_img2 || !d_disparity) return fail(SSAMD_EINVAL, "NULL buffer");
    if (row_parity != 0 && row_parity != 1) return fail(SSAMD_EINVAL, "row_parity must be 0 or 1");
    CtxLock c;
    int rc = get_ctx(-1, c);
    if (rc) return rc;
    return asw_alternate_rows(*c, d_img1, d_img2, height, width, out_row0, out_rows, row_parity, winSize, maxDisparity, minDisparity,
                              gammaC, gammaP, consistent, d_disparity, (hipStream_t)stream);
}

int ssamd_asw_alternate_multi(const uint8_t *img1, const uint8_t *img2, int height, int width, int winSize, int maxDisparity,
                              int minDisparity, double gammaC, double gammaP, int consistent, int16_t *disparity,
                              const int *devices, int n_devices)
{
    if (!img1 || !img2 || !disparity) return fail(SSAMD_EINVAL, "NULL buffer");
    return run_strips(asw_job(img1, img2, height, width, winSize, maxDisparity, minDisparity, gammaC, gammaP, consistent,
                              disparity, nullptr, true), devices, n_devices, asw_host_rows);
}

int ssamd_asw_costs(const uint8_t *img1, const uint8_t *img2, int height, int width, int winSize, int maxDisparity,
                    int minDisparity, double gammaC, double gammaP, float *costs, int device)
{
    if (!img1 || !img2 || !costs) return fail(SSAMD_EINVAL, "NULL buffer");
    if (maxDisparity < minDisparity) return fail(SSAMD_EINVAL, "empty disparity range");
    return asw_host_rows(asw_job(img1, img2, height, width, winSize, maxDisparity, minDisparity, gammaC, gammaP, 0, nullptr,
                                 costs, false), device);
}

int ssamd_asw_argmins(const uint8_t *img1, const uint8_t *img2, int height, int width, int winSize, int maxDisparity,
                      int minDisparity, double gammaC, double gammaP, int16_t *left_disparity, int16_t *right_match,
                      int device)
{
    if (!img1 || !img2 || !left_disparity || !right_match) return fail(SSAMD_EINVAL, "NULL buffer");
    if (maxDisparity < minDisparity) return fail(SSAMD_EINVAL, "empty disparity range");
    HostJob j = asw_job(img1, img2, height, width, winSize, maxDisparity, minDisparity, gammaC, gammaP, 1, left_disparity,
                        nullptr, false);
    j.raw_right = right_match;
    return asw_host_rows(j, device);
}

int ssamd_bgr2lab(const uint8_t *img, int height, int width, float *lab, int device)
{
    if (!img || !lab || height <= 0 || width <= 0) return fail(SSAMD_EINVAL, "bad argument");
    CtxLock c;
    int rc = get_ctx(device, c);
    if (rc) return rc;
    const size_t npix = (size_t)height * width;
    if ((rc = c->imgL.reserve(npix * 3)) || (rc = c->lab.reserve(npix * 12))) return rc;
    hipStream_t s = c->stream;
    ScratchOrder order(*c, s);
    HIP_TRY(hipMemcpyAsync(c->imgL.ptr, img, npix * 3, hipMemcpyHostToDevice, s));
    const int blocks = (int)std::min<size_t>((npix + 255) / 256, 256 * 8);
    hipLaunchKernelGGL(bgr2lab_f32_kernel, dim3(blocks), dim3(256), 0, s, (const uint8_t *)c->imgL.ptr,
                       (float *)c->lab.ptr, (long long)npix);
    HIP_TRY(hipGetLastError());
    HIP_TRY(hipMemcpyAsync(lab, c->lab.ptr, npix * 12, hipMemcpyDeviceToHost, s));
    HIP_TRY(hipStreamSynchronize(s));
    return SSAMD_OK;
}

int ssamd_debug_exact_costs(const uint8_t *img1, const uint8_t *img2, int height, int width, int winSize, double gammaC, double gammaP,
                            int n, const int *yxd, double *costs, double *lab1, double *lab2)
{
    if (!img1 || !img2 || !yxd || !costs || n < 0) return fail(SSAMD_EINVAL, "NULL buffer");
    int rc = check_common(height, width, winSize, 0, 0, 0, height);
    if (rc) return rc;
    CtxLock c;
    if ((rc = get_ctx(-1, c))) return rc;
    const size_t npix = (size_t)height * width;
    hipStream_t s = c->stream;
    ScratchOrder order(*c, s);
    if ((rc = c->imgL.reserve(npix * 3)) || (rc = c->imgR.reserve(npix * 3)) || (rc = c->recL.reserve(npix * sizeof(PixRec))) ||
        (rc = c->recR.reserve(npix * sizeof(PixRec))) || (rc = c->xlabL.reserve(npix * 24)) || (rc = c->xlabR.reserve(npix * 24)) ||
        (rc = c->xqueue.reserve((size_t)std::max(n, 1) * 8)) || (rc = c->xcost.reserve((size_t)std::max(n, 1) * 8)) || (rc = c->xctr.reserve(64)))
        return rc;
    HIP_TRY(hipMemcpyAsync(c->imgL.ptr, img1, npix * 3, hipMemcpyHostToDevice, s));
    HIP_TRY(hipMemcpyAsync(c->imgR.ptr, img2, npix * 3, hipMemcpyHostToDevice, s));
    const int blocks = (int)std::min<long long>((2 * (long long)npix + 255) / 256, 256 * 8);
    hipLaunchKernelGGL(bgr2lab_records_pair_kernel, dim3(blocks), dim3(256), 0, s, (const uint8_t *)c->imgL.ptr, (const uint8_t *)c->imgR.ptr,
                       (PixRec *)c->recL.ptr, (PixRec *)c->recR.ptr, (long long)npix);
    hipLaunchKernelGGL(bgr2lab_f64_pair_kernel, dim3(blocks), dim3(256), 0, s, (const PixRec *)c->recL.ptr, (const PixRec *)c->recR.ptr,
                       (double *)c->xlabL.ptr, (double *)c->xlabR.ptr, (long long)npix);
    std::vector<u64> ent((size_t)n);
    for (int k = 0; k < n; ++k) {
        const int y = yxd[3 * k], x = yxd[3 * k + 1], d = yxd[3 * k + 2];
        if (y < 0 || y >= height || x < 0 || x >= width || d < 0 || x - d < 0) return fail(SSAMD_EINVAL, "candidate %d outside the image", k);
        ent[k] = (u64)((uint32_t)y * (uint32_t)width + (uint32_t)x) | ((u64)(uint32_t)d << 32);
    }
    const unsigned int ctr[16] = {(unsigned int)n};
    HIP_TRY(hipMemcpyAsync(c->xqueue.ptr, ent.data(), (size_t)n * 8, hipMemcpyHostToDevice, s));
    HIP_TRY(hipMemcpyAsync(c->xctr.ptr, ctr, sizeof(ctr), hipMemcpyHostToDevice, s));
    const double *d_prox = nullptr;
    if ((rc = get_prox64(*c, winSize, gammaP, s, &d_prox))) return rc;
    AswExactArgs x{};
    x.recL = (const PixRec *)c->recL.ptr; x.recR = (const PixRec *)c->recR.ptr;
    x.labL = (const double *)c->xlabL.ptr; x.labR = (const double *)c->xlabR.ptr;
    x.prox = d_prox; x.q.entries = (u64 *)c->xqueue.ptr; x.q.counter = (unsigned int *)c->xctr.ptr; x.q.cap = (unsigned int)std::max(n, 1);
    x.ecost = (double *)c->xcost.ptr;
    x.H = height; x.W = width; x.win = winSize; x.pad = winSize / 2; x.row0 = 0; x.rows = height; x.gammaC = gammaC;
    hipLaunchKernelGGL(asw_exact_eval_kernel, dim3(256), dim3(64 * EXACT_WAVES), 0, s, x);
    HIP_TRY(hipGetLastError());
    HIP_TRY(hipMemcpyAsync(costs, c->xcost.ptr, (size_t)n * 8, hipMemcpyDeviceToHost, s));
    if (lab1) HIP_TRY(hipMemcpyAsync(lab1, c->xlabL.ptr, npix * 24, hipMemcpyDeviceToHost, s));
    if (lab2) HIP_TRY(hipMemcpyAsync(lab2, c->xlabR.ptr, npix * 24, hipMemcpyDeviceToHost, s));
    HIP_TRY(hipStreamSynchronize(s));
    return SSAMD_OK;
}

int ssamd_gsw_device(const uint8_t *d_img1, const uint8_t *d_img2, int height, int width, int out_row0, int out_rows,
                     int winSize, int maxDisparity, int minDisparity, int gamma, float fMax, int iterations, int bins,
                     int16_t *d_disparity, void *stream)
{
    (void)bins;
    if (!d_img1 || !d_img2 || !d_disparity) return fail(SSAMD_EINVAL, "NULL buffer");
// ... 281 lines not shown
```

Measured before the change: 10650.

## Add odd-disparity pipe tile handling the leftover disparity with spare waves

When the disparity count is 4k+1, the pipeline kernel can now use a tile whose main register grid covers 4k disparities. The one leftover disparity is aggregated by a separate scalar loop run on waves picked for load balance, and its cost key is merged into the best-left/right reductions and the exact-select queue. The aim is to avoid padding a whole extra disparity group, or splitting into more chunks, for a single extra disparity. In exchange it adds extra LDS traffic and per-tap work on the chosen waves, reuses the bestL and wL buffers as scratch, and adds new static and generic kernel instances plus a scoring penalty in geometry selection.

```diff
diff --git a/simplestereo_amd/csrc/asw_instances.inc b/simplestereo_amd/csrc/asw_instances.inc
--- a/simplestereo_amd/csrc/asw_instances.inc
+++ b/simplestereo_amd/csrc/asw_instances.inc
@@ -1,14 +1,21 @@
 #ifdef SSAMD_PIPE_INSTANCE
 SSAMD_PIPE_INSTANCE(true, 0, 0, 0)
 SSAMD_PIPE_INSTANCE(false, 0, 0, 0)
+SSAMD_PIPE_INSTANCE(false, 128, 324, 208)
 SSAMD_PIPE_INSTANCE(false, 120, 316, 208)
 SSAMD_PIPE_INSTANCE(false, 88, 348, 272)
 SSAMD_PIPE_INSTANCE(false, 216, 284, 80)
+SSAMD_PIPE_INSTANCE(true, 128, 324, 208)
 SSAMD_PIPE_INSTANCE(true, 120, 316, 208)
 SSAMD_PIPE_INSTANCE(true, 88, 348, 272)
 SSAMD_PIPE_INSTANCE(true, 216, 284, 80)
 #endif
+#ifdef SSAMD_PIPE_INSTANCE_ODD
+SSAMD_PIPE_INSTANCE_ODD(true)
+SSAMD_PIPE_INSTANCE_ODD(false)
+#endif
 #ifdef SSAMD_PIPE_INSTANCE_CG
+SSAMD_PIPE_INSTANCE_CG(false, 128, 324, 208)
 SSAMD_PIPE_INSTANCE_CG(false, 120, 316, 208)
 SSAMD_PIPE_INSTANCE_CG(false, 88, 348, 272)
 SSAMD_PIPE_INSTANCE_CG(false, 216, 284, 80)
diff --git a/simplestereo_amd/csrc/asw_kernels.hip.h b/simplestereo_amd/csrc/asw_kernels.hip.h
--- a/simplestereo_amd/csrc/asw_kernels.hip.h
+++ b/simplestereo_amd/csrc/asw_kernels.hip.h
@@ -23,6 +23,8 @@
     int NC, JCmax;
     int dephase;
     int wave_rx;
+    int odd;
+    int odd_waves;
     int off_wL, off_wR, off_e, off_labL, off_labR, off_bgrL, off_bgrR, off_bestL, off_bestR, off_cen, off_prox;
     int lds_bytes;
     int lds_bytes_evol;
@@ -61,14 +63,29 @@
     AswGeom g;
 };
 
-struct AswPipeTileId { int win, XG, DG, JC; };
+struct AswPipeTileId { int win, XG, DG, JC, odd = 0; };
+__host__ __device__ constexpr int asw_odd_waves(int threads, int ncen, int Tx)
+{
+    const int nw = threads / 64, nb = (ncen + 63) / 64, need = (Tx + 63) / 64;
+    if (nb + need > nw) return (1 << nw) - 1;
+    int load[4] = {0, 0, 0, 0}, mask = 0;
+    for (int w = 0; w < nb; ++w) load[w & 3] += 3;
+    for (int n = 0; n < need; ++n) {
+        int pick = -1;
+        for (int w = nb; w < nw; ++w)
+            if (!((mask >> w) & 1) && (pick < 0 || load[w & 3] < load[pick & 3])) pick = w;
+        mask |= 1 << pick;
+        load[pick & 3] += 1;
+    }
+    return mask;
+}
 __host__ __device__ constexpr int asw_cx_round_up(int v, int m) { return (v + m - 1) / m * m; }
 __host__ __device__ constexpr int asw_cx_max(int a, int b) { return a > b ? a : b; }
 __host__ __device__ constexpr AswGeom asw_pipe_geom_constexpr(AswPipeTileId t)
 {
     AswGeom g{};
     const int win = t.win, p = win / 2;
-    g.Rx = 8; g.JC = t.JC; g.pipe = 1; g.wave_rx = 0; g.e2 = 1; g.nchunks = 1;
+    g.Rx = 8; g.JC = t.JC; g.pipe = 1; g.wave_rx = 0; g.e2 = 1; g.nchunks = 1; g.odd = t.odd;
     g.NC = (win + t.JC / 2) / t.JC;
     g.JCmax = asw_cx_max(t.JC, win - (g.NC - 1) * t.JC);
     g.XG = t.XG; g.DG = t.DG;
@@ -76,13 +93,14 @@
     g.threads = asw_cx_round_up(t.XG * t.DG, 64);
     g.dephase = g.threads / 64 >= 12 ? 1 : 0;
     g.nL = g.Tx + 2 * p;
-    g.nRc = g.Tx + g.Dc - 1;
+    g.nRc = g.Tx + g.Dc - 1 + t.odd;
     g.nR = g.nRc + 2 * p;
     g.hL = 0; g.hR = 0;
     g.SL = asw_cx_round_up(g.Tx, 4);
-    g.SR = asw_cx_round_up(g.nRc + 1, 4);
-    g.Se = 16 * ((t.DG + 3) / 4);
+    g.SR = asw_cx_round_up(g.nRc + 1 + 3 * t.odd, 4);
+    g.Se = 16 * ((t.DG + t.odd + 3) / 4);
     g.emask = 0;
+    g.odd_waves = t.odd ? asw_odd_waves(g.threads, g.Tx + g.nRc, g.Tx) : 0;
     const int wrows = 2 * g.JCmax;
     int off = 0;
     g.off_wL = off; off = (off + wrows * g.SL * 4 + 15) & ~15;
@@ -102,6 +120,7 @@
     return g;
 }
 template <int SLC, int SRC, int SEC> struct AswPipeTile { static constexpr AswPipeTileId id{35, 1, 1, 16}; };
+template <> struct AswPipeTile<128, 324, 208> { static constexpr AswPipeTileId id{35, 16, 48, 16, 1}; };
 template <> struct AswPipeTile<120, 316, 208> { static constexpr AswPipeTileId id{35, 15, 49, 16}; };
 template <> struct AswPipeTile<88, 348, 272> { static constexpr AswPipeTileId id{35, 11, 65, 16}; };
 template <> struct AswPipeTile<216, 284, 80> { static constexpr AswPipeTileId id{35, 27, 17, 16}; };
@@ -112,7 +131,7 @@
            a.SR == b.SR && a.Se == b.Se && a.e_bytes == b.e_bytes && a.off_wL == b.off_wL && a.off_wR == b.off_wR && a.off_e == b.off_e &&
            a.off_labL == b.off_labL && a.off_labR == b.off_labR && a.off_bestL == b.off_bestL && a.off_bestR == b.off_bestR &&
            a.off_cen == b.off_cen && a.off_prox == b.off_prox && a.off_bgrL == b.off_bgrL && a.off_bgrR == b.off_bgrR &&
-           a.lds_bytes == b.lds_bytes && a.lds_bytes_evol == b.lds_bytes_evol && a.e2 == b.e2;
+           a.lds_bytes == b.lds_bytes && a.lds_bytes_evol == b.lds_bytes_evol && a.e2 == b.e2 && a.odd == b.odd && a.odd_waves == b.odd_waves;
 }
 
 typedef float v2f __attribute__((ext_vector_type(2)));
diff --git a/simplestereo_amd/csrc/asw_pipe_kernel.hip.h b/simplestereo_amd/csrc/asw_pipe_kernel.hip.h
--- a/simplestereo_amd/csrc/asw_pipe_kernel.hip.h
+++ b/simplestereo_amd/csrc/asw_pipe_kernel.hip.h
@@ -120,11 +120,12 @@
 
 #endif
 
-template <bool WITH_COSTS, int SLC = 0, int SRC = 0, int SEC = 0, bool CG = false>
+template <bool WITH_COSTS, int SLC = 0, int SRC = 0, int SEC = 0, bool CG = false, bool GODD = false>
 __global__ __launch_bounds__(ASW_MAX_THREADS, 3) void asw_aggregate_pipe_kernel(const AswArgs A)
 {
     constexpr bool STATIC = SLC > 0;
     static_assert(!CG || STATIC, "compile-time geometry belongs to a static tile");
+    static_assert(!GODD || !STATIC, "a static tile knows whether it is odd");
     constexpr int RX = ASW_RX;
     constexpr int NWR = asw_nwr(RX);
     extern __shared__ __attribute__((aligned(16))) char smem[];
@@ -147,12 +148,13 @@
     const int W = A.W, win = CG ? AswPipeTile<SLC, SRC, SEC>::id.win : A.win, p = CG ? AswPipeTile<SLC, SRC, SEC>::id.win / 2 : A.pad;
     const int Tx = g.Tx, Dc = g.Dc, nL = g.nL, nR = g.nR, nRc = g.nRc, SR = g.SR, Se = g.Se;
     const int JC = g.JC, NC = g.NC;
+    constexpr int odd = STATIC ? AswPipeTile<SLC, SRC, SEC>::id.odd : (GODD ? 1 : 0);
     int bx = blockIdx.x;
     if ((gridDim.x & 7) == 0) bx = (bx & 7) * (gridDim.x >> 3) + (bx >> 3);
     const int x0 = bx * Tx;
     const int y = asw_out_row(A, blockIdx.y);
     const int dlo = A.minD + blockIdx.z * Dc;
-    const int dhi = dlo + Dc - 1;
+    const int dhi = dlo + Dc - 1 + odd;
     if (min(x0 + Tx - 1, W - 1) - dlo < 0) {
         if (A.disp)
             for (int k = threadIdx.x; k < Tx && x0 + k < W; k += blockDim.x)
@@ -168,8 +170,10 @@
 #pragma unroll
         for (int b = 0; b < ASW_RD; ++b) { accN[a][b] = 0.f; accS[a][b] = 0.f; }
 
-    for (int k = tid; k < Tx; k += nthr) bestL[k] = KEY_NONE;
-    for (int k = tid; k <= nRc; k += nthr) bestR[k] = KEY_NONE;
+    if (!odd) {
+        for (int k = tid; k < Tx; k += nthr) bestL[k] = KEY_NONE;
+        for (int k = tid; k <= nRc; k += nthr) bestR[k] = KEY_NONE;
+    }
     for (int c = tid; c < Tx + nRc; c += nthr) {
         const bool isL = c < Tx;
         const int ccol = isL ? x0 + c : xrc_lo + (c - Tx);
@@ -213,7 +217,7 @@
         int sp = t / nL, ul = t - sp * nL;
         while (t < t_hi) {
             const uint32_t lp = bgrLc[ul];
-            const uint32_t *const rp = bgrRc + (ul + (Dc - 1) - 8 * sp);
+            const uint32_t *const rp = bgrRc + (ul + (Dc - 1 + odd) - 8 * sp);
             uint32_t lo = 0, hi = 0;
 #pragma unroll
             for (int k = 0; k < 4; ++k) {
@@ -221,8 +225,12 @@
                 hi |= min(__builtin_amdgcn_sad_u8(lp, rp[-4 - k], 0u), 40u) << (8 * k);
             }
             uint32_t *const dst = reinterpret_cast<uint32_t *>(eT + ul * Se) + 2 * sp;
+            if (odd) {
+                if (2 * sp == g.DG) lo &= 0xffu;
+                if (2 * sp + 1 == g.DG) hi &= 0xffu;
+            }
             dst[0] = lo;
-            if (2 * sp + 1 < g.DG) dst[1] = hi;
+            if (2 * sp + 1 < g.DG + odd) dst[1] = hi;
             t += nthr; ul += e_r; sp += e_q;
             if (ul >= nL) { ul -= nL; ++sp; }
         }
@@ -266,7 +274,7 @@
             const float4 cen = cenLab[c];
             const float4 *const seg = (isL ? labLc : labRc) + cc;
             const int stride = isL ? g.SL : SR;
-            float *const wout = (isL ? wL : wR) + cc + (rb - jb) * stride;
+            float *const wout = (isL ? wL : wR + 3 * odd) + cc + (rb - jb) * stride;
             const int col0 = (isL ? x0 : xrc_lo) + cc - p;
             const uint32_t cmask = cen.w != 0.f ? 0xffffffffu : 0u;
             int j = jb_t;
@@ -333,7 +341,58 @@
         }
     };
     auto chunk_end = [&](int c) { return c == NC - 1 ? win : (c + 1) * JC; };
-    const int nE = nL * ((g.DG + 1) >> 1);
+    const int nE = nL * ((g.DG + odd + 1) >> 1);
+    float2 *const oddNS = reinterpret_cast<float2 *>(bestL);
+    const int Txo = STATIC ? SG.Tx : Tx;
+    auto d_last = [&]() { return A.minD + (STATIC ? SG.Dc : Dc); };
+    auto odd_first = [&](int t, int &step) {
+        const int w = __builtin_amdgcn_readfirstlane(t >> 6), om = STATIC ? SG.odd_waves : g.odd_waves;
+        step = 64 * __builtin_popcount(om);
+        return (om >> w) & 1 ? 64 * __builtin_popcount(om & ((1 << w) - 1)) + (t & 63) : Txo;
+    };
+    auto odd_taps = [&](int i, int c, int cb) {
+        int tido = threadIdx.x;
+        asm volatile("" : "+v"(tido));
+        if (min(x0 + Txo, A.W) - 1 - d_last() < 0) return;
+        const int SLs = STATIC ? SLC : g.SL, SRs = STATIC ? SRC : SR, Ses = STATIC ? SEC : Se;
+        const int jc = c * JC, n = chunk_end(c) - jc;
+        const int e_bytes = STATIC ? SG.e_bytes : g.e_bytes, wrows = STATIC ? SG.JCmax : g.JCmax, DGs = STATIC ? SG.DG : g.DG;
+        const unsigned char *const eo = eT0 + (i & 1) * e_bytes + 4 * DGs + jc * Ses;
+        const float *const wlo = wL + cb * wrows * SLs, *const wro = wR + cb * wrows * SRs + 3;
+        int step;
+        for (int k = odd_first(tido, step); k < Txo; k += step) {
+            float2 ns = oddNS[k];
+            const float *wl = wlo + k, *wr = wro + k;
+            const unsigned char *ep = eo + k * Ses;
+            constexpr int ASW_OB = 8;
+            for (int j = 0; j < n; j += ASW_OB, wl += ASW_OB * SLs, wr += ASW_OB * SRs, ep += ASW_OB * Ses) {
+                float a_[ASW_OB], b_[ASW_OB];
+                uint32_t e_[ASW_OB];
+                const int m = n - j;
+#pragma unroll
+                for (int u = 0; u < ASW_OB; ++u) {
+                    const int uu = min(u, m - 1);
+                    a_[u] = wl[uu * SLs];
+                    b_[u] = wr[uu * SRs];
+                    e_[u] = ep[uu * Ses];
+                }
+#pragma unroll
+                for (int u = 0; u < ASW_OB; ++u) asm volatile("" : "+v"(a_[u]), "+v"(b_[u]), "+v"(e_[u]));
+#pragma unroll
+                for (int u = 0; u < ASW_OB; ++u)
+                    if (u < m) {
+                        const float w_ = a_[u] * b_[u], e = (float)e_[u];
+                        ns.x = fmaf(w_, e, ns.x);
+                        ns.y = fmaf(w_, ASW_TAD_CAP - e, ns.y);
+                    }
+            }
+            oddNS[k] = ns;
+        }
+    };
+    if (odd) {
+        int step;
+        for (int k = odd_first(tid, step); k < Txo; k += step) oddNS[k] = make_float2(0.f, 0.f);
+    }
     auto build_next = [&](int i, int c, int cb) {
         const bool more_rows = i + 1 < i_hi;
 #ifdef SSAMD_PIPE_BUILD_PRIO
@@ -349,6 +408,9 @@
 #endif
 #ifndef SSAMD_ABLATE_E
         if (c >= 1 && more_rows && !A.evol) build_e(i + 1, (int)((long long)nE * (c - 1) / (NC - 1)), (int)((long long)nE * c / (NC - 1)));
+#endif
+#if !defined(SSAMD_EXP_ODD_MODE) || SSAMD_EXP_ODD_MODE == 0
+        if (odd) odd_taps(i, c, cb);
 #endif
 #ifdef SSAMD_PIPE_BUILD_PRIO
         __builtin_amdgcn_s_setprio(0);
@@ -404,9 +466,14 @@
             const int jc = c * JC, jend = chunk_end(c);
             const int rb = cb * g.JCmax;
             if (phase == 0) build_next(i, c, cb);
+#if defined(SSAMD_EXP_ODD_MODE) && SSAMD_EXP_ODD_MODE == 1
+            if (odd) odd_taps(i, c, cb);
+#endif
 #ifndef SSAMD_ABLATE_AGG
             if (run) {
-                const int xg = pk_xd & 0xffff, dg = pk_xd >> 16;
+                int pk = pk_xd;
+                if (odd) asm volatile("" : "+v"(pk));
+                const int xg = pk & 0xffff, dg = pk >> 16;
                 const unsigned char *erow = eT + (RX * xg + (jc == 0 ? 0 : RX - 1 + jc)) * Se + 4 * dg;
                 if (jc == 0) {
 #pragma unroll
@@ -416,7 +483,7 @@
                     }
                 }
                 const float *wlp = wL + rb * g.SL + 8 * xg;
-                const float *wrp = wR + rb * SR + (RX * xg - ASW_RD * dg + Dc - ASW_RD);
+                const float *wrp = wR + rb * SR + (RX * xg - ASW_RD * dg + Dc - ASW_RD + 4 * odd);
                 for (int j0 = jc; j0 < jend; j0 += RX) {
 #define SSAMD_PSTEP(JJ)                                                                             \
     if (j0 + (JJ) < jend) {                                                                         \
@@ -464,9 +531,38 @@
 
     int tidf = threadIdx.x;
     asm volatile("" : "+v"(tidf));
+    uint32_t *const oddK = reinterpret_cast<uint32_t *>(wL);
+    if (odd) {
+        int step;
+        const int dhi = d_last();
+        for (int k = odd_first(tidf, step); k < Txo; k += step) {
+            const int x = x0 + k;
+            uint32_t img = 0xffffffffu;
+            if (x < W && dhi <= A.maxD && x - dhi >= 0) {
+                const float2 ns = oddNS[k];
+                float c;
+                img = asw_cost_key(ns.x, ns.y, c);
+                if (WITH_COSTS)
+                    A.costs[((size_t)(y - A.row0) * W + x) * (A.maxD - A.minD + 1) + (dhi - A.minD)] = A.cost_keys ? __uint_as_float(img) : c;
+            }
+            reinterpret_cast<uint32_t *>(bestL)[2 * k] = img;
+        }
+        __syncthreads();
+        for (int k = tidf; k <= nRc; k += nthr) {
+            const uint32_t img = k < Txo ? reinterpret_cast<const uint32_t *>(bestL)[2 * k] : 0xffffffffu;
+            if (k < Txo) {
+                oddK[k] = img;
+                bestL[k] = img != 0xffffffffu ? ((u64)img << 32) | (u64)(uint32_t)dhi : KEY_NONE;
+            }
+            bestR[k] = img != 0xffffffffu ? ((u64)img << 32) | (u64)(uint32_t)(x0 + k) : KEY_NONE;
+        }
+        __syncthreads();
+    }
     AswKeyTile<RX, ASW_RD> kt;
+    int pk_e = pk_xd;
+    if (odd) asm volatile("" : "+v"(pk_e));
     if (tidf < nact) {
-        const int xg = pk_xd & 0xffff, dg = pk_xd >> 16;
+        const int xg = pk_e & 0xffff, dg = pk_e >> 16;
         u64 diag[RX + ASW_RD - 1];
 #pragma unroll
         for (int k = 0; k < RX + ASW_RD - 1; ++k) diag[k] = KEY_NONE;
@@ -492,7 +588,7 @@
             if (bl != KEY_NONE) atomicMin(&bestL[RX * xg + xi], bl);
         }
         if (A.keyR) {
-            const int base = RX * xg - ASW_RD * dg + Dc - ASW_RD;
+            const int base = RX * xg - ASW_RD * dg + Dc - ASW_RD + odd;
 #pragma unroll
             for (int k = 0; k < RX + ASW_RD - 1; ++k)
                 if (diag[k] != KEY_NONE) atomicMin(&bestR[base + k], diag[k]);
@@ -502,9 +598,22 @@
     const size_t orow = (size_t)(y - A.row0) * W;
     const bool xq = !WITH_COSTS && A.xq.entries != nullptr;
     if (xq) {
-        const int xg = pk_xd & 0xffff, dg = pk_xd >> 16;
-        asw_exact_select<RX, ASW_RD>(A.xq, tidf < nact, kt, bestL + RX * xg, A.keyR ? bestR + (RX * xg - ASW_RD * dg + Dc - ASW_RD) : nullptr,
+        const int xg = pk_e & 0xffff, dg = pk_e >> 16;
+        asw_exact_select<RX, ASW_RD>(A.xq, tidf < nact, kt, bestL + RX * xg, A.keyR ? bestR + (RX * xg - ASW_RD * dg + Dc - ASW_RD + odd) : nullptr,
                                      x0 + RX * xg, dlo + ASW_RD * dg, (uint32_t)orow, exact_zkey(win));
+        if (odd) {
+            int step;
+            const int k0 = odd_first(tidf, step);
+            if (__builtin_amdgcn_readfirstlane(k0) < Txo)
+                for (int kb = k0 - (tidf & 63); kb < Txo; kb += step) {
+                    const int k = kb + (tidf & 63);
+                    AswKeyTile<1, 1> ko;
+                    ko.v[0][0] = k < Txo ? oddK[k] : 0xffffffffu;
+                    const bool live = ko.v[0][0] != 0xffffffffu;
+                    const int kk = live ? k : 0;
+                    asw_exact_select<1, 1>(A.xq, live, ko, bestL + kk, A.keyR ? bestR + kk : nullptr, x0 + kk, d_last(), (uint32_t)orow, exact_zkey(win));
+                }
+        }
     }
     if (A.disp) {
         for (int k = tid; k < Tx; k += nthr) {
diff --git a/simplestereo_amd/csrc/asw_pipe_tu.hip b/simplestereo_amd/csrc/asw_pipe_tu.hip
--- a/simplestereo_amd/csrc/asw_pipe_tu.hip
+++ b/simplestereo_amd/csrc/asw_pipe_tu.hip
@@ -4,8 +4,10 @@
 
 namespace ssamd {
 #define SSAMD_PIPE_INSTANCE(C, SL, SR, SE) template __global__ void asw_aggregate_pipe_kernel<C, SL, SR, SE>(const AswArgs);
+#define SSAMD_PIPE_INSTANCE_ODD(C) template __global__ void asw_aggregate_pipe_kernel<C, 0, 0, 0, false, true>(const AswArgs);
 #define SSAMD_PIPE_INSTANCE_CG(C, SL, SR, SE) template __global__ void asw_aggregate_pipe_kernel<C, SL, SR, SE, true>(const AswArgs);
 #include "asw_instances.inc"
 #undef SSAMD_PIPE_INSTANCE_CG
+#undef SSAMD_PIPE_INSTANCE_ODD
 #undef SSAMD_PIPE_INSTANCE
 }
diff --git a/simplestereo_amd/csrc/ssamd_api.hip b/simplestereo_amd/csrc/ssamd_api.hip
--- a/simplestereo_amd/csrc/ssamd_api.hip
+++ b/simplestereo_amd/csrc/ssamd_api.hip
@@ -24,11 +24,13 @@
 #ifndef SSAMD_SINGLE_TU
 namespace ssamd {
 #define SSAMD_PIPE_INSTANCE(C, SL, SR, SE) extern template __global__ void asw_aggregate_pipe_kernel<C, SL, SR, SE>(const AswArgs);
+#define SSAMD_PIPE_INSTANCE_ODD(C) extern template __global__ void asw_aggregate_pipe_kernel<C, 0, 0, 0, false, true>(const AswArgs);
 #define SSAMD_PIPE_INSTANCE_CG(C, SL, SR, SE) extern template __global__ void asw_aggregate_pipe_kernel<C, SL, SR, SE, true>(const AswArgs);
 #define SSAMD_WAVE6_INSTANCE(C, K, CREG) extern template __global__ void asw_aggregate_wave6_kernel<C, K, CREG>(const AswWaveArgs);
 #include "asw_instances.inc"
 #undef SSAMD_PIPE_INSTANCE
 #undef SSAMD_PIPE_INSTANCE_CG
+#undef SSAMD_PIPE_INSTANCE_ODD
 #undef SSAMD_WAVE6_INSTANCE
 }
 #endif
@@ -60,6 +62,7 @@
     std::string asw_geom, gsw_geom;
     int asw_pipe = -1;
     int asw_dephase = -1;
+    int asw_odd = -1;
     int asw_evol = 1;
     int asw_wave = -1;
     int wave_rx = 0;
@@ -92,6 +95,7 @@
     else if (name == "SSAMD_GSW_GEOM") t.gsw_geom = v ? v : "";
     else if (name == "SSAMD_ASW_PIPE") t.asw_pipe = num(-1);
     else if (name == "SSAMD_ASW_DEPHASE") t.asw_dephase = num(-1);
+    else if (name == "SSAMD_ASW_ODD") t.asw_odd = v ? (atoi(v) != 0 ? 1 : 0) : -1;
     else if (name == "SSAMD_ASW_EVOL") t.asw_evol = num(1);
     else if (name == "SSAMD_ASW_WAVE") t.asw_wave = v ? (atoi(v) != 0 ? 1 : 0) : -1;
     else if (name == "SSAMD_ASW_WAVE_RX") t.wave_rx = num(0);
@@ -123,7 +127,7 @@
                                     "SSAMD_ASW_WAVE", "SSAMD_ASW_WAVE_RX", "SSAMD_ASW_WAVE_WG", "SSAMD_ASW_WAVE_UNROLL",
                                     "SSAMD_ASW_WAVE_MERGE", "SSAMD_ASW_STATIC", "SSAMD_ASW_EVOL_MAX_MB", "SSAMD_ASW_WAVE_RD", "SSAMD_ASW_NO_E2", "SSAMD_ASW_XOR_ONLY", "SSAMD_MULTI_ALLOW_REPEAT",
                                     "SSAMD_ALT_QUEUE_CAP", "SSAMD_AUTOTUNE", "SSAMD_ASW_EVOL_FAIL", "SSAMD_ASW_TAIL", "SSAMD_ASW_WAVE_CREG", "SSAMD_ASW_LDS_RELAX",
-                                    "SSAMD_EXACT_TOL", "SSAMD_EXACT_CAP", "SSAMD_EXACT_RAWCAP", "SSAMD_ASW_PREPASS_FUSE", "SSAMD_UNWRAP_ROWS"};
+                                    "SSAMD_EXACT_TOL", "SSAMD_EXACT_CAP", "SSAMD_EXACT_RAWCAP", "SSAMD_ASW_PREPASS_FUSE", "SSAMD_UNWRAP_ROWS", "SSAMD_ASW_ODD"};
 
 std::map<std::string, std::string> g_tuning_env;
 Tuning tuning_from_env()
@@ -250,6 +254,7 @@
     long long evol_fallbacks = 0;
     long long tail_splits = 0;
     long long exact_calls = 0;
+    long long odd_tile_launches = 0;
     long long static_tile_mismatch = 0;
     Profile prof;
 };
@@ -352,8 +357,10 @@
 thread_local bool t_pipe_full_lds = false;
 
 bool asw_layout_e(AswGeom &g, int win, int XG, int DG, size_t limit, int JC, int Rx, bool e2, bool odd_pitch = false,
-                  bool pipe = false)
-{
+                  bool pipe = false, int odd = 0)
+{
+    if (odd && !pipe) return false;
+    g.odd = odd; g.odd_waves = 0;
     g.Rx = Rx;
     g.JC = JC >= win ? win : JC;
     g.pipe = 0; g.NC = 1; g.JCmax = g.JC; g.dephase = 0; g.wave_rx = 0;
@@ -373,7 +380,7 @@
     g.Tx = Rx * XG; g.Dc = ASW_RD * DG;
     g.threads = round_up(XG * DG, 64);
     g.nL = g.Tx + 2 * p;
-    g.nRc = g.Tx + g.Dc - 1;
+    g.nRc = g.Tx + g.Dc - 1 + odd;
     g.nR = g.nRc + 2 * p;
     g.hL = ((g.Tx + 7) / 8) * 4 + 4;
     g.SL = 2 * g.hL;
@@ -392,8 +399,12 @@
         g.hL = g.hR = 0;
         g.SL = round_up(g.Tx, 4);
         g.SR = round_up(g.nRc + 1, 4);
-        g.Se = 16 * ((DG + 3) / 4);
+        g.Se = 16 * ((DG + odd + 3) / 4);
         g.emask = 0;
+        if (odd) {
+            g.SR = round_up(g.nRc + 1 + 3, 4);
+            g.odd_waves = asw_odd_waves(g.threads, g.Tx + g.nRc, g.Tx);
+        }
     }
     {
         const int ncen = g.Tx + g.nRc;
@@ -586,7 +597,7 @@
     const Tuning &t = tune();
     return !t.asw_geom.empty() || t.asw_wave >= 0 || t.wave_rx != 0 || t.wave_merge != 1 || t.asw_pipe >= 0 || t.asw_dephase >= 0 ||
            t.asw_evol != 1 || t.wave_wg != 0 || t.no_e2 || t.xor_only || t.asw_static != 1 || t.evol_max_mb != 0 || t.wave_rd != 0 ||
-           t.wave_creg != 1 || t.lds_relax != 1;
+           t.wave_creg != 1 || t.lds_relax != 1 || t.asw_odd >= 0;
 }
 
 int asw_choose_geometry(AswGeom &best, int W, int rows, int win, int nD)
@@ -612,6 +623,13 @@
         if (sscanf(tune().asw_geom.c_str(), "%d,%d,%d,%d", &XG, &DG, &JCe, &Rx) >= 2 && XG > 0 && DG > 0 && XG * DG <= ASW_MAX_THREADS &&
             (Rx == 8 || Rx == 4)) {
             if (JCe <= 0 || JCe % Rx) JCe = 1 << 20;
+            if (tune().asw_odd == 1 && Rx == 8 && nD == ASW_RD * DG + 1 && tune().asw_pipe != 0)
+                for (int JC : {16, 8}) {
+                    if (tune().asw_pipe > 0 ? JC != tune().asw_pipe : (JC == 8 && round_up(XG * DG, 64) / 64 < 12)) continue;
+                    if (!asw_layout_e(best, win, XG, DG, 160 * 1024, JC, 8, true, false, true, 1)) continue;
+                    best.nchunks = 1;
+                    return SSAMD_OK;
+                }
             if (!asw_layout(best, win, XG, DG, 160 * 1024, JCe, Rx)) return fail(SSAMD_ELIMIT, "SSAMD_ASW_GEOM does not fit LDS");
             best.nchunks = (nD + best.Dc - 1) / best.Dc;
             asw_pick_e_scheme(best, win);
@@ -624,7 +642,7 @@
     bool found = false;
     for (int nch = 1; nch <= nD; ++nch) {
         const int per = (nD + nch - 1) / nch;
-        const int DG = round_up(per, ASW_RD) / ASW_RD;
+        const int DG = round_up(per, ASW_RD) / ASW_RD, DGc = DG;
         if (DG > 128) continue;
         if ((nD + DG * ASW_RD - 1) / (DG * ASW_RD) != nch) continue;
         for (int Rx : {8, 4}) {
@@ -632,8 +650,10 @@
         const int max_wps = Rx == 8 ? 3 : 4;
         const int xg_cap = std::min(ASW_MAX_THREADS / DG, (W + Rx - 1) / Rx);
         const int pipe_env = tune().asw_pipe;
-        for (int XG = xg_cap; XG >= 1; --XG)
-        for (int cand = 0; cand < 6; ++cand) {
+        for (int oddv = 0; oddv <= (nch == 1 && Rx == 8 && nD % ASW_RD == 1 && nD > ASW_RD && tune().asw_odd != 0 ? 1 : 0); ++oddv)
+        for (int XG = oddv ? std::min(ASW_MAX_THREADS / (DG - 1), (W + Rx - 1) / Rx) : xg_cap; XG >= 1; --XG)
+        for (int cand = oddv ? 4 : 0; cand < 6; ++cand) {
+            const int DG = oddv ? (nD - 1) / ASW_RD : DGc;
             static const int jcs[6] = {1 << 20, 16, 8, 4, 16, 8};
             const int JC = jcs[cand];
             const bool piped = cand >= 4;
@@ -641,7 +661,8 @@
             if (piped) {
                 if (Rx != 8 || pipe_env == 0 || (pipe_env > 0 && pipe_env != JC)) continue;
                 if (pipe_env < 0 && JC == 8 && round_up(XG * DG, 64) / 64 < 12) continue;
-                if (!asw_layout_e(g, win, XG, DG, 160 * 1024, JC, 8, true, false, true)) continue;
+                if (!asw_layout_e(g, win, XG, DG, 160 * 1024, JC, 8, true, false, true, oddv)) continue;
+                if (oddv && g.odd_waves == (1 << (g.threads / 64)) - 1) continue;
             } else {
                 if (JC < (1 << 20) && (JC >= win || JC % Rx)) continue;
                 if (!asw_layout(g, win, XG, DG, 160 * 1024, JC, Rx)) continue;
@@ -670,7 +691,7 @@
             const int wps = k * per_simd;
             const double occ = wps >= 3 ? 1.0 : (wps == 2 ? 0.85 : 0.6);
             const double useful = (double)win * Rx * ASW_RD * c_tap;
-            const double score = (double)XG * DG / per_simd * occ * (useful / (M + B)) * d_util * x_util * tail * overlap;
+            const double score = (double)XG * DG / per_simd * occ * (useful / (M + B)) * d_util * x_util * tail * overlap * (g.odd ? 0.97 : 1.0);
             if (score > best_score) { best_score = score; best = g; found = true; }
             if (shortlist) {
                 auto &slot = classes[{piped ? 80 : Rx, std::min(g.JC, 64), nch, waves}];
@@ -1023,7 +1044,7 @@
         AswWaveArgs wa;
         auto prepare_evol = [&](const AswGeom &g) -> int {
             a.evol = nullptr;
-            int chunks = g.nchunks, Tx = g.Tx, Dc = g.Dc, Se = g.Se;
+            int chunks = g.nchunks, Tx = g.Tx, Dc = g.Dc + g.odd, Se = g.Se;
             if (g.wave_rx) {
                 if (!asw_wave_layout(wa.g, win, nD, g.wave_rx, !d_costs && tune().wave_unroll != 0))
                     return fail(SSAMD_ELIMIT, "wave kernel geometry does not fit LDS");
@@ -1132,14 +1153,18 @@
             const bool chunked = g.JC < win;
             if (g.pipe) {
                 auto pk = d_costs ? asw_aggregate_pipe_kernel<true> : asw_aggregate_pipe_kernel<false>;
-                if (tune().asw_static != 0) {
+                if (g.odd) pk = d_costs ? asw_aggregate_pipe_kernel<true, 0, 0, 0, false, true> : asw_aggregate_pipe_kernel<false, 0, 0, 0, false, true>;
+                if (tune().asw_static != 0 && g.odd) {
+                    if (win == AswPipeTile<128, 324, 208>::id.win && asw_pipe_geom_matches(g, asw_pipe_geom_constexpr(AswPipeTile<128, 324, 208>::id))) pk = d_costs ? asw_aggregate_pipe_kernel<true, 128, 324, 208> : asw_aggregate_pipe_kernel<false, 128, 324, 208>;
+                } else if (tune().asw_static != 0) {
                     if (g.SL == 120 && g.SR == 316 && g.Se == 208) pk = d_costs ? asw_aggregate_pipe_kernel<true, 120, 316, 208> : asw_aggregate_pipe_kernel<false, 120, 316, 208>;
                     else if (g.SL == 88 && g.SR == 348 && g.Se == 272) pk = d_costs ? asw_aggregate_pipe_kernel<true, 88, 348, 272> : asw_aggregate_pipe_kernel<false, 88, 348, 272>;
                     else if (g.SL == 216 && g.SR == 284 && g.Se == 80) pk = d_costs ? asw_aggregate_pipe_kernel<true, 216, 284, 80> : asw_aggregate_pipe_kernel<false, 216, 284, 80>;
                 }
                 if (tune().asw_static == 2 && !d_costs) {
                     auto is_tile = [&](AswPipeTileId id) { return win == id.win && asw_pipe_geom_matches(g, asw_pipe_geom_constexpr(id)); };
-                    if (is_tile(AswPipeTile<120, 316, 208>::id)) pk = asw_aggregate_pipe_kernel<false, 120, 316, 208, true>;
+                    if (is_tile(AswPipeTile<128, 324, 208>::id)) pk = asw_aggregate_pipe_kernel<false, 128, 324, 208, true>;
+                    else if (is_tile(AswPipeTile<120, 316, 208>::id)) pk = asw_aggregate_pipe_kernel<false, 120, 316, 208, true>;
                     else if (is_tile(AswPipeTile<88, 348, 272>::id)) pk = asw_aggregate_pipe_kernel<false, 88, 348, 272, true>;
                     else if (is_tile(AswPipeTile<216, 284, 80>::id)) pk = asw_aggregate_pipe_kernel<false, 216, 284, 80, true>;
                     else ++c.static_tile_mismatch;
@@ -1157,7 +1182,7 @@
                     if (full >= 1 && rem > 0 && 2 * rem <= slots && (full < 32 || tune().asw_tail > 0)) {
                         const int rm = (int)(full * slots / per_row);
                         if (rm >= 1 && rm < grows &&
-                            asw_layout_e(tail_g, win, (g.XG + 1) / 2, g.DG, 160 * 1024, g.JC, 8, true, false, true) && tail_g.pipe &&
+                            asw_layout_e(tail_g, win, (g.XG + 1) / 2, g.DG, 160 * 1024, g.JC, 8, true, false, true, g.odd) && tail_g.pipe &&
                             tail_g.Se == g.Se && tail_g.Dc == g.Dc &&
                             (a.evol == nullptr || round_up(((W + tail_g.Tx - 1) / tail_g.Tx) * tail_g.Tx + 2 * p, 4) <= a.evolW)) {
                             tail_g.nchunks = g.nchunks;
@@ -1167,12 +1192,14 @@
                 }
                 hipLaunchKernelGGL(pk, dim3(grid.x, rows_main, grid.z), block, pipe_lds, s, a);
                 HIP_TRY(hipGetLastError());
+                if (g.odd) ++c.odd_tile_launches;
                 if (rows_main < grows) {
                     ++c.tail_splits;
                     AswArgs t = a;
                     t.g = tail_g;
                     t.yb0 = rows_main;
                     auto tk = d_costs ? asw_aggregate_pipe_kernel<true> : asw_aggregate_pipe_kernel<false>;
+                    if (tail_g.odd) tk = d_costs ? asw_aggregate_pipe_kernel<true, 0, 0, 0, false, true> : asw_aggregate_pipe_kernel<false, 0, 0, 0, false, true>;
                     const int tail_lds = a.evol ? tail_g.lds_bytes_evol : tail_g.lds_bytes;
                     if (int grc = grant_dyn_lds(c, (const void *)tk, tail_lds)) return grc;
                     hipLaunchKernelGGL(tk, dim3((W + tail_g.Tx - 1) / tail_g.Tx, grows - rows_main, tail_g.nchunks), dim3(tail_g.threads),
@@ -1791,6 +1818,7 @@
     else if (n == "tail_splits") *value = c->tail_splits;
     else if (n == "exact_calls") *value = c->exact_calls;
     else if (n == "static_tile_mismatch") *value = c->static_tile_mismatch;
+    else if (n == "odd_tile_launches") *value = c->odd_tile_launches;
     else if (n == "exact_entries" || n == "exact_flagged_left" || n == "exact_flagged_right" || n == "exact_overflow" || n == "exact_raw_entries") {
         unsigned int ctr[5] = {0, 0, 0, 0, 0};
         if (c->xflags.ptr && c->exact_calls > 0) {
@@ -1819,6 +1847,7 @@
     AswGeom g;
     if ((rc = asw_choose_geometry(g, width, rows, winSize, nD))) return rc;
     out[0] = g.Tx; out[1] = g.Dc; out[2] = g.nchunks; out[3] = g.threads; out[4] = g.lds_bytes;
+    if (g.pipe && !g.wave_rx && g.lds_bytes > 160 * 1024) out[4] = g.lds_bytes_evol;
     out[5] = (width + g.Tx - 1) / g.Tx; out[6] = rows; out[7] = g.nchunks;
     AswWaveGeom wg;
     if (g.wave_rx && asw_wave_layout(wg, winSize, nD, g.wave_rx, tune().wave_unroll != 0)) {
```

Result: slower. 9577 (-10.1%).
